# RichExplor/VIL_Fusion

Hardware: AMD Instinct MI355X
Metric: sliding-window solve iters/sec (10 KF, ~5.5k factors) @1/2/4/8 GPU vs CPU (higher is better)
Workload: dtype f64

## Files before the change

vil_fusion_amd/csrc/vilf_api.hip:

```cpp
#include <hip/hip_runtime.h>
#include <string>
#include <vector>
#include <cstring>
#include <cstdio>
#include <cmath>
#include <algorithm>
#include <chrono>
#include <cstdlib>
#include <thread>
#include <atomic>
#include <type_traits>
#include "vilf_internal.hpp"
#include "vilf_kernels.hpp"
#include "vilf_sort.hpp"

namespace {

int class_plan(const vilf_window_in &in, int *cls, int *cstart, int *ccount) {
    int pcount[VB_NPAIR] = {0};
    for (int f = 0; f < in.n_features; f++) {
        const int s = in.feature_start_frame[f], n = in.feature_obs_offset[f + 1] - in.feature_obs_offset[f];
        for (int k = 1; k < n; k++) { const int j = s + k; pcount[j * (j - 1) / 2 + s]++; }
    }
    int order[VB_NPAIR], load[4] = {0, 0, 0, 0};
// ... 1075 lines not shown
    if (!h || !counts || !h->resident || !h->marg.info || !h->marg.qlInfo) return VILF_ERR_INVALID_ARGUMENT;
    HIPCHECK(h, hipSetDevice(h->device));
    const size_t sB = h->B;
    std::vector<int> info(sB * MG_INFO), qi(sB * 4);
    HIPCHECK(h, hipMemcpyAsync(info.data(), h->marg.info, info.size() * 4, hipMemcpyDeviceToHost, h->stream));
    HIPCHECK(h, hipMemcpyAsync(qi.data(), h->marg.qlInfo, qi.size() * 4, hipMemcpyDeviceToHost, h->stream));
    HIPCHECK(h, hipStreamSynchronize(h->stream));
    counts[0] = counts[1] = counts[2] = counts[3] = 0;
    for (size_t w = 0; w < sB; w++) {
        if (info[w * MG_INFO] != 0) { counts[3]++; continue; }
        counts[0]++;
        if (info[w * MG_INFO + 7] == 0) counts[1]++;
        if (qi[w * 4 + 3] == 1) counts[2]++;
    }
    return VILF_OK;
}

static int hook_buf(vilf_handle *h, size_t doubles) { return h->d[D_HOOK].ensure(doubles * 8) ? VILF_OK : VILF_ERR_DEVICE; }

extern "C" int vilf_eval_projection(vilf_handle *h, const double *const *p, const double pts_i[3], const double pts_j[3], double *residuals, double **jac) {
    if (!h || !p || !residuals) return VILF_ERR_INVALID_ARGUMENT;
    if (hook_buf(h, 256) != VILF_OK) return VILF_ERR_DEVICE;
    double in[32];
    std::memcpy(in, p[0], 56); std::memcpy(in + 7, p[1], 56); std::memcpy(in + 14, p[2], 56);
    std::memcpy(in + 21, pts_i, 24); std::memcpy(in + 24, pts_j, 24);
    double *d = h->d[D_HOOK].as<double>();
    HIPCHECK(h, hipMemcpyAsync(d, in, sizeof(in), hipMemcpyHostToDevice, h->stream));
    hipLaunchKernelGGL(k_hook_projection, dim3(1), dim3(HOOK_NT), 0, h->stream, d, d + 7, d + 14, p[3][0], d + 21, d + 24, h->opts.focal_length / 1.5, d + 32);
    double out[28];
    HIPCHECK(h, hipMemcpyAsync(out, d + 32, sizeof(out), hipMemcpyDeviceToHost, h->stream));
    HIPCHECK(h, hipStreamSynchronize(h->stream));
    residuals[0] = out[0]; residuals[1] = out[1];
    if (jac) {
        for (int blk = 0; blk < 2; blk++)
            if (jac[blk]) for (int r = 0; r < 2; r++) { for (int c = 0; c < 6; c++) jac[blk][7 * r + c] = out[2 + 12 * blk + 6 * r + c]; jac[blk][7 * r + 6] = 0; }
        if (jac[2]) {
            double in2[40] = {0};
            std::memcpy(in2, in, 27 * 8);
            in2[31] = p[3][0]; in2[37] = 0.0; in2[38] = h->opts.focal_length / 1.5;
            HIPCHECK(h, hipMemcpyAsync(d + 64, in2, sizeof(in2), hipMemcpyHostToDevice, h->stream));
            hipLaunchKernelGGL(k_hook_projection_td, dim3(1), dim3(HOOK_NT), 0, h->stream, d + 64, d + 64 + 40);
            double out2[42];
            HIPCHECK(h, hipMemcpyAsync(out2, d + 64 + 40, sizeof(out2), hipMemcpyDeviceToHost, h->stream));
            HIPCHECK(h, hipStreamSynchronize(h->stream));
            for (int r = 0; r < 2; r++) { for (int c = 0; c < 6; c++) jac[2][7 * r + c] = out2[26 + 6 * r + c]; jac[2][7 * r + 6] = 0; }
        }
        if (jac[3]) { jac[3][0] = out[26]; jac[3][1] = out[27]; }
    }
    return VILF_OK;
}

extern "C" int vilf_eval_projection_td(vilf_handle *h, const double *const *p, const double pts_i[3], const double pts_j[3], const double vel_i[2], const double vel_j[2],
                                       double td_i, double td_j, double row_i, double row_j, double *residuals, double **jac) {
    if (!h || !p || !residuals || !pts_i || !pts_j || !vel_i || !vel_j) return VILF_ERR_INVALID_ARGUMENT;
    if (hook_buf(h, 128) != VILF_OK) return VILF_ERR_DEVICE;
    double in[40];
    std::memcpy(in, p[0], 56); std::memcpy(in + 7, p[1], 56); std::memcpy(in + 14, p[2], 56);
    std::memcpy(in + 21, pts_i, 24); std::memcpy(in + 24, pts_j, 24); std::memcpy(in + 27, vel_i, 16); std::memcpy(in + 29, vel_j, 16);
    const double ROW = h->opts.ROW;
    in[31] = p[3][0]; in[32] = p[4][0]; in[33] = td_i; in[34] = td_j; in[35] = row_i - ROW / 2; in[36] = row_j - ROW / 2;
    in[37] = h->opts.TR / ROW; in[38] = h->opts.focal_length / 1.5;
    double *d = h->d[D_HOOK].as<double>();
    HIPCHECK(h, hipMemcpyAsync(d, in, sizeof(in), hipMemcpyHostToDevice, h->stream));
    hipLaunchKernelGGL(k_hook_projection_td, dim3(1), dim3(HOOK_NT), 0, h->stream, d, d + 40);
    double out[42];
    HIPCHECK(h, hipMemcpyAsync(out, d + 40, sizeof(out), hipMemcpyDeviceToHost, h->stream));
    HIPCHECK(h, hipStreamSynchronize(h->stream));
    residuals[0] = out[0]; residuals[1] = out[1];
    if (jac) {
        const int off[3] = {2, 14, 26};
        for (int blk = 0; blk < 3; blk++)
            if (jac[blk]) for (int r = 0; r < 2; r++) { for (int c = 0; c < 6; c++) jac[blk][7 * r + c] = out[off[blk] + 6 * r + c]; jac[blk][7 * r + 6] = 0; }
        if (jac[3]) { jac[3][0] = out[38]; jac[3][1] = out[39]; }
        if (jac[4]) { jac[4][0] = out[40]; jac[4][1] = out[41]; }
    }
    return VILF_OK;
}

static void pack_imu_rec(const vilf_imu_preint *p, double *rec) {
    std::memset(rec, 0, IMU_REC * 8);
    fill_imu_rec(*p, rec);
    rec[287] = 1.0;
}

static int run_imu_hook(vilf_handle *h, const double *const *p, const vilf_imu_preint *pre, double **d_out) {
    if (hook_buf(h, 4096) != VILF_OK) return VILF_ERR_DEVICE;
    double *d = *d_out = h->d[D_HOOK].as<double>();
    std::vector<double> in(40 + IMU_REC + 225, 0.0);
    std::memcpy(&in[0], p[0], 56); std::memcpy(&in[7], p[1], 72); std::memcpy(&in[16], p[2], 56); std::memcpy(&in[23], p[3], 72);
    for (int i = 0; i < 3; i++) in[32 + i] = h->opts.G[i];
    pack_imu_rec(pre, &in[40]);
    std::memcpy(&in[40 + IMU_REC], pre->covariance, 225 * 8);
    HIPCHECK(h, vilf_copy_sync(h, d, in.data(), in.size() * 8, hipMemcpyHostToDevice));
    hipLaunchKernelGGL(k_imu_prep, dim3(1), dim3(IMU_PREP_NT), 0, h->stream, 1, d + 40 + IMU_REC, d + 1024, d + 40);
    hipLaunchKernelGGL(k_hook_imu, dim3(1), dim3(HOOK_NT), 0, h->stream, d, d + 7, d + 16, d + 23, d + 40, d + 32, d + 2048, d + 3072);
    return VILF_OK;
}
extern "C" int vilf_eval_imu(vilf_handle *h, const double *const *p, const vilf_imu_preint *pre, double *residuals, double **jac) {
    if (!h || !p || !pre || !residuals) return VILF_ERR_INVALID_ARGUMENT;
    double *d;
    { const int rc = run_imu_hook(h, p, pre, &d); if (rc != VILF_OK) return rc; }
    std::vector<double> out(15 + 450);
    HIPCHECK(h, hipMemcpyAsync(out.data(), d + 2048, out.size() * 8, hipMemcpyDeviceToHost, h->stream));
    HIPCHECK(h, hipStreamSynchronize(h->stream));
    for (int i = 0; i < 15; i++) residuals[i] = out[i];
    if (jac) {
        const int off[4] = {0, 6, 15, 21}, loc[4] = {6, 9, 6, 9}, glob[4] = {7, 9, 7, 9};
        for (int blk = 0; blk < 4; blk++)
            if (jac[blk]) for (int r = 0; r < 15; r++) { for (int c = 0; c < glob[blk]; c++) jac[blk][glob[blk] * r + c] = (c < loc[blk]) ? out[15 + 30 * r + off[blk] + c] : 0.0; }
    }
    return VILF_OK;
}

extern "C" int vilf_eval_imu_raw(vilf_handle *h, const double *const *p, const vilf_imu_preint *pre, double *residuals, double **jac, double *sqrt_info_out) {
    if (!h || !p || !pre || !residuals) return VILF_ERR_INVALID_ARGUMENT;
    double *d;
    { const int rc = run_imu_hook(h, p, pre, &d); if (rc != VILF_OK) return rc; }
    std::vector<double> raw(450 + 15), S(225);
    HIPCHECK(h, hipMemcpyAsync(raw.data(), d + 3072, raw.size() * 8, hipMemcpyDeviceToHost, h->stream));
    HIPCHECK(h, hipMemcpyAsync(S.data(), d + 40 + IMU_SQRT, 225 * 8, hipMemcpyDeviceToHost, h->stream));
    HIPCHECK(h, hipStreamSynchronize(h->stream));
    for (int i = 0; i < 15; i++) residuals[i] = raw[450 + i];
    if (jac) {
        const int off[4] = {0, 6, 15, 21}, loc[4] = {6, 9, 6, 9}, glob[4] = {7, 9, 7, 9};
        for (int blk = 0; blk < 4; blk++)
            if (jac[blk]) for (int r = 0; r < 15; r++) { for (int c = 0; c < glob[blk]; c++) jac[blk][glob[blk] * r + c] = (c < loc[blk]) ? raw[30 * r + off[blk] + c] : 0.0; }
    }
    if (sqrt_info_out) std::memcpy(sqrt_info_out, S.data(), 225 * 8);
    return VILF_OK;
}

extern "C" int vilf_eval_lidar_between(vilf_handle *h, const double *const *p, const vilf_lidar_constraint *c, double *residuals, double **jac) {
    if (!h || !p || !c || !residuals) return VILF_ERR_INVALID_ARGUMENT;
    if (hook_buf(h, 256) != VILF_OK) return VILF_ERR_DEVICE;
    if (!h->resident) lidar_extrinsic(h->opts, h->batch);
    double in[32];
    std::memcpy(in, p[0], 56); std::memcpy(in + 7, p[1], 56);
    std::memcpy(in + 14, h->batch.qil, 32); std::memcpy(in + 18, h->batch.til, 24);
    for (int i = 0; i < 4; i++) in[21 + i] = c->q[i];
    for (int i = 0; i < 3; i++) in[25 + i] = c->t[i];
    double *d = h->d[D_HOOK].as<double>();
    HIPCHECK(h, hipMemcpyAsync(d, in, sizeof(in), hipMemcpyHostToDevice, h->stream));
    hipLaunchKernelGGL(k_hook_lidar, dim3(1), dim3(HOOK_NT), 0, h->stream, d, d + 7, d + 14, d + 18, d + 21, d + 32);
    double out[78];
    HIPCHECK(h, hipMemcpyAsync(out, d + 32, sizeof(out), hipMemcpyDeviceToHost, h->stream));
    HIPCHECK(h, hipStreamSynchronize(h->stream));
    for (int i = 0; i < 6; i++) residuals[i] = out[i];
    if (jac)
        for (int blk = 0; blk < 2; blk++)
            if (jac[blk]) for (int r = 0; r < 6; r++) { for (int cc = 0; cc < 6; cc++) jac[blk][7 * r + cc] = out[6 + 36 * blk + 6 * r + cc]; jac[blk][7 * r + 6] = 0; }
    return VILF_OK;
}

extern "C" int vilf_eval_edge(vilf_handle *h, const double pose[7], const double cp[3], const double a[3], const double bb[3], double r[3], double *J) {
    if (!h) return VILF_ERR_INVALID_ARGUMENT;
    if (hook_buf(h, 128) != VILF_OK) return VILF_ERR_DEVICE;
    double in[16];
    std::memcpy(in, pose, 56); std::memcpy(in + 7, cp, 24); std::memcpy(in + 10, a, 24); std::memcpy(in + 13, bb, 24);
    double *d = h->d[D_HOOK].as<double>();
    HIPCHECK(h, hipMemcpyAsync(d, in, sizeof(in), hipMemcpyHostToDevice, h->stream));
    hipLaunchKernelGGL(k_hook_edge, dim3(1), dim3(HOOK_NT), 0, h->stream, d, d + 7, d + 10, d + 13, d + 16);
    double out[21];
    HIPCHECK(h, hipMemcpyAsync(out, d + 16, sizeof(out), hipMemcpyDeviceToHost, h->stream));
    HIPCHECK(h, hipStreamSynchronize(h->stream));
    for (int i = 0; i < 3; i++) r[i] = out[i];
    if (J) for (int i = 0; i < 3; i++) { for (int c = 0; c < 6; c++) J[7 * i + c] = out[3 + 6 * i + c]; J[7 * i + 6] = 0; }
    return VILF_OK;
}

extern "C" int vilf_eval_surf(vilf_handle *h, const double pose[7], const double cp[3], const double n[3], double dd, double r[1], double *J) {
    if (!h) return VILF_ERR_INVALID_ARGUMENT;
    if (hook_buf(h, 128) != VILF_OK) return VILF_ERR_DEVICE;
    double in[16];
    std::memcpy(in, pose, 56); std::memcpy(in + 7, cp, 24); std::memcpy(in + 10, n, 24);
    double *d = h->d[D_HOOK].as<double>();
    HIPCHECK(h, hipMemcpyAsync(d, in, sizeof(in), hipMemcpyHostToDevice, h->stream));
    hipLaunchKernelGGL(k_hook_surf, dim3(1), dim3(HOOK_NT), 0, h->stream, d, d + 7, d + 10, dd, d + 16);
    double out[7];
    HIPCHECK(h, hipMemcpyAsync(out, d + 16, sizeof(out), hipMemcpyDeviceToHost, h->stream));
    HIPCHECK(h, hipStreamSynchronize(h->stream));
    r[0] = out[0];
    if (J) { for (int c = 0; c < 6; c++) J[c] = out[1 + c]; J[6] = 0; }
    return VILF_OK;
}

static int plus_hook(vilf_handle *h, const double x[7], const double dl[6], double xp[7], int kind) {
    if (!h) return VILF_ERR_INVALID_ARGUMENT;
    if (hook_buf(h, 64) != VILF_OK) return VILF_ERR_DEVICE;
    double in[13];
    std::memcpy(in, x, 56); std::memcpy(in + 7, dl, 48);
    double *d = h->d[D_HOOK].as<double>();
    HIPCHECK(h, hipMemcpyAsync(d, in, sizeof(in), hipMemcpyHostToDevice, h->stream));
    hipLaunchKernelGGL(k_hook_plus, dim3(1), dim3(HOOK_NT), 0, h->stream, d, d + 7, kind, d + 16);
    HIPCHECK(h, hipMemcpyAsync(xp, d + 16, 56, hipMemcpyDeviceToHost, h->stream));
    HIPCHECK(h, hipStreamSynchronize(h->stream));
    return VILF_OK;
}
extern "C" int vilf_pose_plus(vilf_handle *h, const double x[7], const double d[6], double xp[7]) { return plus_hook(h, x, d, xp, 0); }
extern "C" int vilf_se3_plus(vilf_handle *h, const double x[7], const double d[6], double xp[7]) { return plus_hook(h, x, d, xp, 1); }

extern "C" int vilf_eval_prior(vilf_handle *h, const vilf_prior *p, const double *const *params, double *residuals, double **jac) {
    if (!h || !p || !params || !residuals || !p->valid || p->n < 1 || p->n > VILF_PRIOR_MAX_DIM || p->n_blocks < 1 || p->n_blocks > VILF_PRIOR_MAX_BLOCKS) return VILF_ERR_INVALID_ARGUMENT;
    const int n = p->n, nb = p->n_blocks;
    const size_t doubles = 32 + 2 * 24 * 9 + (size_t)n * n + 2 * (size_t)n + 16;
    if (hook_buf(h, doubles) != VILF_OK) return VILF_ERR_DEVICE;
    std::vector<double> in(32 + 2 * 24 * 9 + (size_t)n * n + n, 0.0);
    int *hdr = reinterpret_cast<int *>(in.data());
    hdr[0] = n; hdr[1] = nb;
    for (int i = 0; i < nb; i++) {
        hdr[2 + i] = p->block_size[i]; hdr[26 + i] = p->block_idx[i];
        if (!params[i]) return VILF_ERR_INVALID_ARGUMENT;
        for (int k = 0; k < p->block_size[i] && k < 9; k++) { in[32 + 9 * i + k] = p->block_x0[i][k]; in[32 + 216 + 9 * i + k] = params[i][k]; }
    }
    std::memcpy(&in[32 + 432], p->linearized_jacobians, sizeof(double) * n * n);
    std::memcpy(&in[32 + 432 + (size_t)n * n], p->linearized_residuals, sizeof(double) * n);
    double *d = h->d[D_HOOK].as<double>();
    HIPCHECK(h, hipMemcpyAsync(d, in.data(), in.size() * 8, hipMemcpyHostToDevice, h->stream));
    double *d_out = d + in.size();
    hipLaunchKernelGGL(k_hook_prior, dim3(1), dim3(HOOK_PRIOR_NT), 0, h->stream, reinterpret_cast<const int *>(d), d + 32, d + 32 + 216, d + 32 + 432, d + 32 + 432 + (size_t)n * n, d_out);
    HIPCHECK(h, hipMemcpyAsync(residuals, d_out, sizeof(double) * n, hipMemcpyDeviceToHost, h->stream));
    HIPCHECK(h, hipStreamSynchronize(h->stream));
    if (jac)
        for (int i = 0; i < nb; i++) {
            if (!jac[i]) continue;
            const int gs = p->block_size[i], ls = gs == 7 ? 6 : gs, idx = p->block_idx[i];
            for (int r = 0; r < n; r++) for (int c = 0; c < gs; c++) jac[i][(size_t)r * gs + c] = c < ls ? p->linearized_jacobians[(size_t)r * n + idx + c] : 0.0;
        }
    return VILF_OK;
}
```

vil_fusion_amd/csrc/vilf_device.hpp:

```cpp
#pragma once
#include <hip/hip_runtime.h>
#include <math.h>

#define VD __device__ __forceinline__

VD double vilf_dot3(double a0, double b0, double a1, double b1, double a2, double b2) { return __dadd_rn(__dadd_rn(__dmul_rn(a0, b0), __dmul_rn(a1, b1)), __dmul_rn(a2, b2)); }

__device__ __forceinline__ void lds_barrier() { asm volatile("s_waitcnt lgkmcnt(0)\n\ts_barrier" ::: "memory"); }
template <int CTRL>
VD double vilf_dpp_f64(double v) {
    const int lo = __builtin_amdgcn_update_dpp(0, __double2loint(v), CTRL, 0xF, 0xF, false), hi = __builtin_amdgcn_update_dpp(0, __double2hiint(v), CTRL, 0xF, 0xF, false);
    return __hiloint2double(hi, lo);
}
VD double vilf_wave_sum64(double v) {
    v += vilf_dpp_f64<0xB1>(v);
    v += vilf_dpp_f64<0x4E>(v);
    v += vilf_dpp_f64<0x141>(v);
    v += vilf_dpp_f64<0x140>(v);
    const double r0 = __hiloint2double(__builtin_amdgcn_readlane(__double2hiint(v), 0), __builtin_amdgcn_readlane(__double2loint(v), 0));
    const double r1 = __hiloint2double(__builtin_amdgcn_readlane(__double2hiint(v), 16), __builtin_amdgcn_readlane(__double2loint(v), 16));
    const double r2 = __hiloint2double(__builtin_amdgcn_readlane(__double2hiint(v), 32), __builtin_amdgcn_readlane(__double2loint(v), 32));
    const double r3 = __hiloint2double(__builtin_amdgcn_readlane(__double2hiint(v), 48), __builtin_amdgcn_readlane(__double2loint(v), 48));
    return (r0 + r1) + (r2 + r3);
}
// ... 260 lines not shown
    u[0] += tji[0] - tic[0]; u[1] += tji[1] - tic[1]; u[2] += tji[2] - tic[2];
    m3T_vec(ric, u, tc);
#pragma unroll
    for (int k = 0; k < 9; k++) { pt[k] = A[k]; pt[9 + k] = ARi[k]; pt[18 + k] = Rji[k]; pt[30 + k] = Rc[k]; }
#pragma unroll
    for (int k = 0; k < 3; k++) { pt[27 + k] = tji[k]; pt[39 + k] = tc[k]; }
}
template <bool JAC>
VD void projection_eval_pair(const double *pt, const double *ric, const double *tic, const double *pts_i, const double *pts_j, double inv_dep,
                             double sqrt_info, double *r, double *Ji, double *Jj, double *Jf) {
    const double il = 1.0 / inv_dep;
    const double pc_i[3] = {pts_i[0] * il, pts_i[1] * il, pts_i[2] * il};
    double pc_j[3];
    m3_vec(pt + 30, pc_i, pc_j);
    pc_j[0] += pt[39]; pc_j[1] += pt[40]; pc_j[2] += pt[41];
    const double inv_z = 1.0 / pc_j[2];
    r[0] = sqrt_info * (pc_j[0] * inv_z - pts_j[0]);
    r[1] = sqrt_info * (pc_j[1] * inv_z - pts_j[1]);
    if (JAC) {
        const double r00 = sqrt_info * inv_z, r02 = -sqrt_info * pc_j[0] * inv_z * inv_z, r12 = -sqrt_info * pc_j[1] * inv_z * inv_z;
        const double *A = pt, *ARi = pt + 9, *Rji = pt + 18;
        double p_imu_i[3], p_imu_j[3];
        m3_vec(ric, pc_i, p_imu_i);
        p_imu_i[0] += tic[0]; p_imu_i[1] += tic[1]; p_imu_i[2] += tic[2];
        m3_vec(Rji, p_imu_i, p_imu_j);
        p_imu_j[0] += pt[27]; p_imu_j[1] += pt[28]; p_imu_j[2] += pt[29];
        double M[6], M2[6], N[6];
#pragma unroll
        for (int j = 0; j < 3; j++) {
            M[j] = r00 * A[j] + r02 * A[6 + j]; M[3 + j] = r00 * A[3 + j] + r12 * A[6 + j];
            M2[j] = r00 * ARi[j] + r02 * ARi[6 + j]; M2[3 + j] = r00 * ARi[3 + j] + r12 * ARi[6 + j];
            N[j] = r00 * ric[3 * j] + r02 * ric[3 * j + 2]; N[3 + j] = r00 * ric[3 * j + 1] + r12 * ric[3 * j + 2];
        }
#pragma unroll
        for (int rr = 0; rr < 2; rr++) {
            const double *m = M + 3 * rr, *m2 = M2 + 3 * rr, *n = N + 3 * rr;
            double *ji = Ji + 6 * rr, *jj = Jj + 6 * rr;
            ji[0] = m[0]; ji[1] = m[1]; ji[2] = m[2];
            ji[3] = -(m2[1] * p_imu_i[2] - m2[2] * p_imu_i[1]);
            ji[4] = -(-m2[0] * p_imu_i[2] + m2[2] * p_imu_i[0]);
            ji[5] = -(m2[0] * p_imu_i[1] - m2[1] * p_imu_i[0]);
            jj[0] = -m[0]; jj[1] = -m[1]; jj[2] = -m[2];
            jj[3] = n[1] * p_imu_j[2] - n[2] * p_imu_j[1];
            jj[4] = -n[0] * p_imu_j[2] + n[2] * p_imu_j[0];
            jj[5] = n[0] * p_imu_j[1] - n[1] * p_imu_j[0];
        }
        double rp[3];
        m3_vec(pt + 30, pts_i, rp);
        const double s = -il * il;
        Jf[0] = (r00 * rp[0] + r02 * rp[2]) * s;
        Jf[1] = (r00 * rp[1] + r12 * rp[2]) * s;
    }
}

template <bool JAC>
VD void lidar_between_eval(const double *posei, const double *posej, const Q &qil, const double *til, const Q &lq, const double *lt,
                           double *r, double *Ji, double *Jj) {
    Q Qi = q_load(posei + 3), Qj = q_load(posej + 3);
    Q Qi_inv = q_inv(Qi), qli = q_inv(qil);
    double dP[3] = {posej[0] - posei[0], posej[1] - posei[1], posej[2] - posei[2]};
    double a[3], tli[3], b[3], c[3], rp[3];
    q_rot(Qi_inv, dP, a);
    q_rot(qli, til, tli); tli[0] = -tli[0]; tli[1] = -tli[1]; tli[2] = -tli[2];
    Q qm = q_mul(qil, lq);
    q_rot(qm, tli, b);
    c[0] = a[0] - til[0] - b[0]; c[1] = a[1] - til[1] - b[1]; c[2] = a[2] - til[2] - b[2];
    q_rot(qli, c, rp);
    Q cdq = q_mul(qm, qli);
    Q rq = q_mul(q_inv(cdq), q_mul(Qi_inv, Qj));
    r[0] = 10.0 * (rp[0] - lt[0]); r[1] = 10.0 * (rp[1] - lt[1]); r[2] = 10.0 * (rp[2] - lt[2]);
    r[3] = 100.0 * 2.0 * rq.x; r[4] = 100.0 * 2.0 * rq.y; r[5] = 100.0 * 2.0 * rq.z;
    if (JAC) {
#pragma unroll
        for (int k = 0; k < 36; k++) { Ji[k] = 0; Jj[k] = 0; }
        double Rm[9], Rl[9], S[9], T[9];
        q_toR(q_mul(qli, Qi_inv), Rm);
        q_toR(qli, Rl);
        skew3(a, S);
        m3_mul(Rl, S, T);
        double B[9], Cm[9];
        qleft_qright_br(q_mul(q_inv(Qj), Qi), cdq, B);
        qleft_br(q_mul(q_inv(cdq), q_mul(Qi_inv, Qj)), Cm);
#pragma unroll
        for (int i = 0; i < 3; i++)
#pragma unroll
            for (int j = 0; j < 3; j++) {
                Ji[6 * i + j] = -Rm[3 * i + j];
                Ji[6 * i + 3 + j] = T[3 * i + j];
                Ji[6 * (3 + i) + 3 + j] = -B[3 * i + j];
                Jj[6 * i + j] = Rm[3 * i + j];
                Jj[6 * (3 + i) + 3 + j] = Cm[3 * i + j];
            }
    }
}

template <bool JAC, int LD = 30, bool ZERO = true>
VD void imu_raw_eval(const double *posei, const double *sbi, const double *posej, const double *sbj, const double *rec, const double *G,
                     double *r, double *Jraw) {
    const double dt = rec[0];
    const double *dp = rec + 1, *dv = rec + 8, *lba = rec + 11, *lbg = rec + 14;
    const double *dp_dba = rec + 17, *dp_dbg = rec + 26, *dq_dbg = rec + 35, *dv_dba = rec + 44, *dv_dbg = rec + 53;
    Q Qi = q_load(posei + 3), Qj = q_load(posej + 3), delta_q = q_load(rec + 4);
    Q Qi_inv = q_inv(Qi);
    double dba[3] = {sbi[3] - lba[0], sbi[4] - lba[1], sbi[5] - lba[2]};
    double dbg[3] = {sbi[6] - lbg[0], sbi[7] - lbg[1], sbi[8] - lbg[2]};
    double th[3];
    m3_vec(dq_dbg, dbg, th);
    Q cdq = q_mul(delta_q, q_delta(th[0], th[1], th[2]));
    double t1[3], t2[3], cdv[3], cdp[3];
    m3_vec(dv_dba, dba, t1); m3_vec(dv_dbg, dbg, t2);
    for (int k = 0; k < 3; k++) cdv[k] = dv[k] + t1[k] + t2[k];
    m3_vec(dp_dba, dba, t1); m3_vec(dp_dbg, dbg, t2);
    for (int k = 0; k < 3; k++) cdp[k] = dp[k] + t1[k] + t2[k];
    double a[3], b[3], ra[3], rb[3];
    for (int k = 0; k < 3; k++) {
        a[k] = 0.5 * G[k] * dt * dt + posej[k] - posei[k] - sbi[k] * dt;
        b[k] = G[k] * dt + sbj[k] - sbi[k];
    }
    q_rot(Qi_inv, a, ra);
    q_rot(Qi_inv, b, rb);
    Q QiQj = q_mul(Qi_inv, Qj);
    Q rq = q_mul(q_inv(cdq), QiQj);
    r[0] = ra[0] - cdp[0]; r[1] = ra[1] - cdp[1]; r[2] = ra[2] - cdp[2];
    r[3] = 2 * rq.x; r[4] = 2 * rq.y; r[5] = 2 * rq.z;
    r[6] = rb[0] - cdv[0]; r[7] = rb[1] - cdv[1]; r[8] = rb[2] - cdv[2];
    for (int k = 0; k < 3; k++) { r[9 + k] = sbj[3 + k] - sbi[3 + k]; r[12 + k] = sbj[6 + k] - sbi[6 + k]; }
    if (JAC) {
        if (ZERO) for (int k = 0; k < 450; k++) Jraw[k] = 0;
        double RiT[9], S[9], B[9];
        q_toR(Qi_inv, RiT);
        auto put = [&](int r0, int c0, const double *m, double s) {
            for (int i = 0; i < 3; i++) for (int j = 0; j < 3; j++) Jraw[(r0 + i) * LD + c0 + j] = s * m[3 * i + j];
        };
        const double I3[9] = {1, 0, 0, 0, 1, 0, 0, 0, 1};
        put(0, 0, RiT, -1.0);
        skew3(ra, S); put(0, 3, S, 1.0);
        qleft_qright_br(q_mul(q_inv(Qj), Qi), cdq, B); put(3, 3, B, -1.0);
        skew3(rb, S); put(6, 3, S, 1.0);
        put(0, 6, RiT, -dt); put(0, 9, dp_dba, -1.0); put(0, 12, dp_dbg, -1.0);
        {
            double L[9], T[9];
            qleft_br(q_mul(q_mul(q_inv(Qj), Qi), delta_q), L);
            m3_mul(L, dq_dbg, T);
            put(3, 12, T, -1.0);
        }
        put(6, 6, RiT, -1.0); put(6, 9, dv_dba, -1.0); put(6, 12, dv_dbg, -1.0);
        put(9, 9, I3, -1.0); put(12, 12, I3, -1.0);
        put(0, 15, RiT, 1.0);
        qleft_br(q_mul(q_inv(cdq), QiQj), B); put(3, 18, B, 1.0);
        put(6, 21, RiT, 1.0); put(9, 24, I3, 1.0); put(12, 27, I3, 1.0);
    }
}

template <bool JAC>
VD void edge_eval(const double *pose, const double *cp, const double *pa, const double *pb, double *r, double *J) {
    Q q = q_load(pose);
    double lp[3];
    q_rot(q, cp, lp);
    lp[0] += pose[4]; lp[1] += pose[5]; lp[2] += pose[6];
    double u[3] = {lp[0] - pa[0], lp[1] - pa[1], lp[2] - pa[2]}, v[3] = {lp[0] - pb[0], lp[1] - pb[1], lp[2] - pb[2]};
    double ab[3] = {pa[0] - pb[0], pa[1] - pb[1], pa[2] - pb[2]};
    double inv = 1.0 / sqrt(ab[0] * ab[0] + ab[1] * ab[1] + ab[2] * ab[2]);
    r[0] = (u[1] * v[2] - u[2] * v[1]) * inv;
    r[1] = (u[2] * v[0] - u[0] * v[2]) * inv;
    r[2] = (u[0] * v[1] - u[1] * v[0]) * inv;
    if (JAC) {
        double Sab[9], Slp[9], T[9];
        skew3(ab, Sab); skew3(lp, Slp);
        m3_mul(Sab, Slp, T);
        for (int i = 0; i < 3; i++)
            for (int j = 0; j < 3; j++) { J[6 * i + j] = T[3 * i + j] * inv; J[6 * i + 3 + j] = -Sab[3 * i + j] * inv; }
    }
}
template <bool JAC>
VD void surf_eval(const double *pose, const double *cp, const double *n, double d, double *r, double *J) {
    Q q = q_load(pose);
    double pw[3];
    q_rot(q, cp, pw);
    pw[0] += pose[4]; pw[1] += pose[5]; pw[2] += pose[6];
    r[0] = n[0] * pw[0] + n[1] * pw[1] + n[2] * pw[2] + d;
    if (JAC) {
        J[0] = -(n[1] * pw[2] - n[2] * pw[1]);
        J[1] = -(-n[0] * pw[2] + n[2] * pw[0]);
        J[2] = -(n[0] * pw[1] - n[1] * pw[0]);
        J[3] = n[0]; J[4] = n[1]; J[5] = n[2];
    }
}
VD void se3_plus(const double *x, const double *d, double *o) {
    double th = sqrt(d[0] * d[0] + d[1] * d[1] + d[2] * d[2]);
    double half = 0.5 * th, imag, real = cos(half);
    if (th < 1e-10) { double t2 = th * th, t4 = t2 * t2; imag = 0.5 - 0.0208333 * t2 + 0.000260417 * t4; }
    else imag = sin(half) / th;
    Q dq{imag * d[0], imag * d[1], imag * d[2], real};
    double Jm[9];
    if (th < 1e-10) q_toR(dq, Jm);
    else {
        double O[9], O2[9];
        skew3(d, O); m3_mul(O, O, O2);
        double a = (1 - cos(th)) / (th * th), b = (th - sin(th)) / (th * th * th);
        for (int k = 0; k < 9; k++) Jm[k] = a * O[k] + b * O2[k];
        Jm[0] += 1; Jm[4] += 1; Jm[8] += 1;
    }
    double dt[3], rt[3];
    m3_vec(Jm, d + 3, dt);
    Q qn = q_mul(dq, q_load(x));
    q_rot(dq, x + 4, rt);
    q_store(o, qn);
    o[4] = rt[0] + dt[0]; o[5] = rt[1] + dt[1]; o[6] = rt[2] + dt[2];
}


template <bool JAC>
VD void projection_td_eval(const double *Pi, const double *Ri, const double *Pj, const double *Rj, const double *ric, const double *tic,
                           const double *pts_i, const double *pts_j, const double *vel_i, const double *vel_j, double td, double td_i, double td_j,
                           double row_i_c, double row_j_c, double tr_over_row, double inv_dep, double sqrt_info,
                           double *r, double *Ji, double *Jj, double *Jf, double *Jex, double *Jtd) {
    const double si = td - td_i + tr_over_row * row_i_c, sj = td - td_j + tr_over_row * row_j_c;
    const double pi_td[3] = {pts_i[0] - si * vel_i[0], pts_i[1] - si * vel_i[1], pts_i[2]};
    const double pj_td[3] = {pts_j[0] - sj * vel_j[0], pts_j[1] - sj * vel_j[1], pts_j[2]};
    double M2[6];
    projection_eval<JAC>(Pi, Ri, Pj, Rj, ric, tic, pi_td, pj_td, inv_dep, sqrt_info, r, Ji, Jj, Jf, Jex, M2);
    if (JAC) {
        const double v3[3] = {vel_i[0], vel_i[1], 0.0};
        double rv[3];
        m3_vec(ric, v3, rv);
        Jtd[0] = (M2[0] * rv[0] + M2[1] * rv[1] + M2[2] * rv[2]) / inv_dep * -1.0 + sqrt_info * vel_j[0];
        Jtd[1] = (M2[3] * rv[0] + M2[4] * rv[1] + M2[5] * rv[2]) / inv_dep * -1.0 + sqrt_info * vel_j[1];
    }
}
}
```

vil_fusion_amd/csrc/vilf_kernels.hip:

```cpp
#include "vilf_device.hpp"
#include "vilf_kernels.hpp"

using namespace vd;

typedef double double4_t __attribute__((ext_vector_type(4)));
typedef double double2_t __attribute__((ext_vector_type(2)));

#define NT VB_NT
#ifdef VILF_STAMPS
#define STAMP(kid, i) do { if (b.dbg && blockIdx.x == 0 && threadIdx.x == 0) b.dbg[(kid) * 32 + (i)] = __builtin_readcyclecounter(); } while (0)
#define TICK() __builtin_readcyclecounter()
#else
#define STAMP(kid, i) do { } while (0)
#define TICK() 0LL
#endif
#define LSTAMP(i) do { if (JAC) STAMP(0, i); } while (0)
__device__ __forceinline__ int pair_index(int i, int j) { return j * (j - 1) / 2 + i; }
__device__ __forceinline__ int perm_index(int a, int l) { return l < 6 ? 6 * a + l : 66 + 9 * a + (l - 6); }
__device__ __forceinline__ void unperm(int p, int &a, int &l) {
    if (p < 66) { a = p / 6; l = p - 6 * a; } else { int q = p - 66; a = q / 9; l = 6 + q - 9 * a; }
}
__device__ __forceinline__ int tile_index(int ta, int tb) { return ta * (ta + 1) / 2 + tb; }
#define TIX(r, c) (16 * (r) + ((c) ^ (r)))

__device__ __forceinline__ double block_sum(double v, double *s_red) {
    const int tid = threadIdx.x;
    v = vilf_wave_sum64(v);
    lds_barrier();
    if ((tid & 63) == 0) s_red[tid >> 6] = v;
    lds_barrier();
    double r = 0;
#pragma unroll
    for (int k = 0; k < NT / 64; k++) r += s_red[k];
    lds_barrier();
    return r;
}
__device__ __forceinline__ double block_max(double v, double *s_red) {
    const int tid = threadIdx.x;
    v = vilf_wave_max64(v);
    lds_barrier();
    if ((tid & 63) == 0) s_red[tid >> 6] = v;
    lds_barrier();
    double r = s_red[0];
#pragma unroll
    for (int k = 1; k < NT / 64; k++) r = fmax(r, s_red[k]);
    lds_barrier();
    return r;
}

extern "C" __global__ __launch_bounds__(IMU_PREP_NT) void k_imu_prep(int n, const double *cov, double *work, double *imu_rec) {
    __shared__ double sA[4][15][16], sI[4][15][16], s_piv[4];
    const int grp = threadIdx.x >> 4, r = threadIdx.x & 15, id = blockIdx.x * 4 + grp;
    const bool row = id < n && r < 15;
    (void)work;
    if (row) for (int j = 0; j < 15; j++) { sA[grp][r][j] = cov[(size_t)id * 225 + 15 * r + j]; sI[grp][r][j] = (j == r) ? 1.0 : 0.0; }
    __syncthreads();
    for (int k = 0; k < 15; k++) {
        if (id < n && r == 0) {
            int p = k; double best = fabs(sA[grp][k][k]);
            for (int i = k + 1; i < 15; i++) { const double v = fabs(sA[grp][i][k]); if (v > best) { best = v; p = i; } }
            if (p != k) for (int j = 0; j < 15; j++) { double t = sA[grp][k][j]; sA[grp][k][j] = sA[grp][p][j]; sA[grp][p][j] = t; t = sI[grp][k][j]; sI[grp][k][j] = sI[grp][p][j]; sI[grp][p][j] = t; }
            s_piv[grp] = sA[grp][k][k];
        }
        __syncthreads();
        if (row && r > k) {
            const double f = sA[grp][r][k] / s_piv[grp];
            for (int j = k; j < 15; j++) sA[grp][r][j] -= f * sA[grp][k][j];
            for (int j = 0; j < 15; j++) sI[grp][r][j] -= f * sI[grp][k][j];
        }
        __syncthreads();
    }
    for (int k = 14; k >= 0; k--) {
        if (row && r == k) { const double piv = sA[grp][k][k]; for (int j = 0; j < 15; j++) sI[grp][k][j] /= piv; }
        __syncthreads();
        if (row && r < k) { const double f = sA[grp][r][k]; for (int j = 0; j < 15; j++) sI[grp][r][j] -= f * sI[grp][k][j]; }
        __syncthreads();
    }
    for (int j = 0; j < 15; j++) {
        if (row && r == j) { double sacc = sI[grp][j][j]; for (int k = 0; k < j; k++) sacc -= sI[grp][j][k] * sI[grp][j][k]; sI[grp][j][j] = sqrt(sacc); }
        __syncthreads();
        if (row && r > j) { double t = sI[grp][r][j]; for (int k = 0; k < j; k++) t -= sI[grp][r][k] * sI[grp][j][k]; sI[grp][r][j] = t / sI[grp][j][j]; }
        __syncthreads();
    }
    if (row) { double *S = imu_rec + (size_t)id * IMU_REC + IMU_SQRT; for (int j = 0; j < 15; j++) S[15 * r + j] = (j >= r) ? sI[grp][j][r] : 0.0; }
}

extern "C" __global__ __launch_bounds__(NT) void k_prior_prep(VbBatch b, double *prior_H, double *prior_g, unsigned lds_bytes, const int *done4) {
    const int w = blockIdx.x, tid = threadIdx.x;
    const int *hdr = b.prior_hdr + (size_t)w * VB_PRIOR_HDR;
    if (!hdr[0] || (done4 && done4[4 * (size_t)w + 3])) return;
    const int n = hdr[1];
    const double *J = b.prior_J + (size_t)w * VB_PRIOR_LD * VB_PRIOR_LD;
    const double *r = b.prior_r + (size_t)w * VB_PRIOR_LD;
    double *H = prior_H + (size_t)w * VB_PRIOR_LD * VB_PRIOR_LD;
    double *g = prior_g + (size_t)w * VB_PRIOR_LD;
    extern __shared__ double s_J[];
    const int ld = n | 1;
    if ((size_t)n * ld * sizeof(double) <= lds_bytes) {
        for (int e = tid; e < n * n; e += NT) { const int k = e / n, i = e - k * n; s_J[k * ld + i] = J[e]; }
        __syncthreads();
        for (int e = tid; e < n * n; e += NT) {
            int i = e / n, j = e - i * n;
            double s = 0;
            for (int k = 0; k < n; k++) s += s_J[k * ld + i] * s_J[k * ld + j];
            H[i * VB_PRIOR_LD + j] = s;
        }
        for (int i = tid; i < n; i += NT) {
            double s = 0;
            for (int k = 0; k < n; k++) s += s_J[k * ld + i] * r[k];
            g[i] = s;
        }
        return;
    }
    for (int e = tid; e < n * n; e += NT) {
        int i = e / n, j = e - i * n;
        double s = 0;
        for (int k = 0; k < n; k++) s += J[k * n + i] * J[k * n + j];
        H[i * VB_PRIOR_LD + j] = s;
    }
    for (int i = tid; i < n; i += NT) {
        double s = 0;
        for (int k = 0; k < n; k++) s += J[k * n + i] * r[k];
        g[i] = s;
    }
}

__device__ void prior_setup(const VbBatch &b, int w, const double *pose, const double *sb, int *s_pcol, double *s_dx, int tid) {
    const int *hdr = b.prior_hdr + (size_t)w * VB_PRIOR_HDR;
    for (int i = tid; i < VB_P; i += NT) s_pcol[i] = -1;
    for (int i = tid; i < VB_PRIOR_LD; i += NT) s_dx[i] = 0.0;
    __syncthreads();
    if (!hdr[0]) return;
    const int nb = hdr[2];
    if (tid < nb) {
        const int id = hdr[3 + tid], size = hdr[27 + tid], idx = hdr[51 + tid];
        const double *x0 = b.prior_x0 + ((size_t)w * 24 + tid) * 9;
        if (id < VB_NF) {
            const double *x = pose + 7 * id;
            for (int k = 0; k < 3; k++) s_dx[idx + k] = x[k] - x0[k];
            Q dq = q_mul(q_inv(q_load(x0 + 3)), q_load(x + 3));
            double sgn = (dq.w >= 0) ? 2.0 : -2.0;
            s_dx[idx + 3] = sgn * dq.x; s_dx[idx + 4] = sgn * dq.y; s_dx[idx + 5] = sgn * dq.z;
            for (int k = 0; k < 6; k++) s_pcol[15 * id + k] = idx + k;
        } else if (id < 2 * VB_NF) {
            const int a = id - VB_NF;
            const double *x = sb + 9 * a;
            for (int k = 0; k < 9; k++) { s_dx[idx + k] = x[k] - x0[k]; s_pcol[15 * a + 6 + k] = idx + k; }
        } else if (id == 2 * VB_NF) {
            const double *x = b.ex + (size_t)w * 7;
            for (int k = 0; k < 3; k++) s_dx[idx + k] = x[k] - x0[k];
            Q dq = q_mul(q_inv(q_load(x0 + 3)), q_load(x + 3));
            double sgn = (dq.w >= 0) ? 2.0 : -2.0;
            s_dx[idx + 3] = sgn * dq.x; s_dx[idx + 4] = sgn * dq.y; s_dx[idx + 5] = sgn * dq.z;
        }
        (void)size;
    }
    __syncthreads();
}

__device__ double prior_cost_partial(const VbBatch &b, int w, const double *s_dx, int tid) {
    const int *hdr = b.prior_hdr + (size_t)w * VB_PRIOR_HDR;
    if (!hdr[0]) return 0.0;
    const int n = hdr[1];
    const double *J = b.prior_J + (size_t)w * VB_PRIOR_LD * VB_PRIOR_LD;
    const double *r0 = b.prior_r + (size_t)w * VB_PRIOR_LD;
    double acc = 0;
    for (int row = tid; row < n; row += NT) {
        double s = r0[row];
        for (int k = 0; k < n; k++) s += J[row * n + k] * s_dx[k];
        acc += 0.5 * s * s;
    }
    return acc;
}

__device__ __forceinline__ double prior_cost_split(const VbBatch &b, int w, const double *s_dx, double *s_tmp, int tid) {
    const int *hdr = b.prior_hdr + (size_t)w * VB_PRIOR_HDR;
    if (!hdr[0]) return 0.0;
    const int n = hdr[1];
    if (3 * n > NT) return prior_cost_partial(b, w, s_dx, tid);
    const double *J = b.prior_J + (size_t)w * VB_PRIOR_LD * VB_PRIOR_LD;
    const int row = tid / 3, part = tid - 3 * row, per = (n + 2) / 3, c0 = part * per, c1 = min(n, c0 + per);
    const double r0v = b.prior_r[(size_t)w * VB_PRIOR_LD + min(row, n - 1)];
    double acc = 0;
    if (row < n) {
        const double *Jr = J + (size_t)row * n;
#pragma unroll 8
        for (int k = c0; k < c1; k++) acc += Jr[k] * s_dx[k];
    }
    s_tmp[tid] = acc;
    lds_barrier();
    double cost = 0;
    if (row < n && part == 0) { double t = r0v; t += s_tmp[tid]; t += s_tmp[tid + 1]; t += s_tmp[tid + 2]; cost = 0.5 * t * t; }
    lds_barrier();
    return cost;
}
__device__ __forceinline__ double prior_grad_split(const VbBatch &b, int w, const double *s_dx, const int *s_pcol, double *s_tmp, int tid) {
    const int *hdr = b.prior_hdr + (size_t)w * VB_PRIOR_HDR;
    if (!hdr[0]) return 0.0;
    const int n = hdr[1];
    const int pc = (tid < VB_P) ? s_pcol[tid] : -1;
    if (3 * n > NT) {
        if (pc < 0) return 0.0;
        double t = b.prior_g[(size_t)w * VB_PRIOR_LD + pc];
        const double *pH = b.prior_H + (size_t)w * VB_PRIOR_LD * VB_PRIOR_LD + (size_t)pc * VB_PRIOR_LD;
#pragma unroll 8
        for (int k = 0; k < n; k++) t += pH[k] * s_dx[k];
        return t;
    }
    const int col = tid / 3, part = tid - 3 * col, per = (n + 2) / 3, c0 = part * per, c1 = min(n, c0 + per);
    const double g0 = b.prior_g[(size_t)w * VB_PRIOR_LD + max(pc, 0)];
    double acc = 0;
    if (col < n) {
        const double *pH = b.prior_H + (size_t)w * VB_PRIOR_LD * VB_PRIOR_LD + (size_t)col * VB_PRIOR_LD;
#pragma unroll 8
        for (int k = c0; k < c1; k++) acc += pH[k] * s_dx[k];
    }
    s_tmp[tid] = acc;
    lds_barrier();
    double g = 0;
    if (pc >= 0) { g = g0; g += s_tmp[3 * pc]; g += s_tmp[3 * pc + 1]; g += s_tmp[3 * pc + 2]; }
    lds_barrier();
    return g;
}

template <bool GRAD>
__device__ __forceinline__ void prior_products_j(const VbBatch &b, int w, const double *s_dx, const int *s_pcol, double *s_tmp, double *s_t, int tid, double &cost, double &gprior) {
    cost = 0.0; gprior = 0.0;
    const int *hdr = b.prior_hdr + (size_t)w * VB_PRIOR_HDR;
    if (!hdr[0]) return;
    const int n = hdr[1];
    if (n > 85) {
        cost = prior_cost_split(b, w, s_dx, s_tmp, tid);
        if (GRAD) gprior = prior_grad_split(b, w, s_dx, s_pcol, s_tmp, tid);
        return;
    }
    const double *J = b.prior_J + (size_t)w * VB_PRIOR_LD * VB_PRIOR_LD, *r0 = b.prior_r + (size_t)w * VB_PRIOR_LD;
    const int lane = tid & 63, wave = __builtin_amdgcn_readfirstlane(tid >> 6);
    const int c0 = min(lane, n - 1), c1 = min(lane + 64, n - 1);
    const double dx0 = s_dx[lane], dx1 = s_dx[lane + 64];
    const double r0v = r0[min(wave + 4 * min(lane, 31), n - 1)];
    {
        double a0[6], a1[6];
#pragma unroll 1
        for (int rb = wave; rb < n; rb += 24) {
#pragma unroll
            for (int u = 0; u < 6; u++) { const double *Jr = J + (size_t)min(rb + 4 * u, n - 1) * n; a0[u] = Jr[c0]; a1[u] = Jr[c1]; }
#pragma unroll
            for (int u = 0; u < 6; u++) {
                const int r = rb + 4 * u;
                const double sum = vilf_wave_sum64(a0[u] * dx0 + a1[u] * dx1);
                const double t = readlane_f64(r0v, (r - wave) >> 2) + sum;
                if (r < n && lane == 0) { s_t[r] = t; cost += 0.5 * t * t; }
            }
        }
    }
    if (GRAD) {
        lds_barrier();
        const int pc = (tid < VB_P) ? s_pcol[tid] : -1;
        if (wave < 3) {
            const int per = (n + 2) / 3, ra = wave * per, rb = min(n, ra + per);
            double g0 = 0, g1 = 0;
#pragma unroll 8
            for (int r = ra; r < rb; r++) { const double t = s_t[r]; const double *Jr = J + (size_t)r * n; g0 += Jr[c0] * t; g1 += Jr[c1] * t; }
            s_tmp[85 * wave + c0] = g0;
            if (lane + 64 < n) s_tmp[85 * wave + lane + 64] = g1;
        }
        lds_barrier();
        if (pc >= 0) { double g = s_tmp[pc]; g += s_tmp[85 + pc]; g += s_tmp[170 + pc]; gprior = g; }
        lds_barrier();
    }
}

__device__ __forceinline__ int vb_window(const VbBatch &b) {
    const int i = b.live_it;
    if (!b.live_ctl || i < 3 || !b.live_ctl[i - 2]) return blockIdx.x + b.w0;
    if ((int)blockIdx.x >= b.live_ctl[64 + i - 1]) return -1;
    return b.live_buf[(size_t)((i - 1) & 1) * b.B + blockIdx.x];
}
#define LIN_LDS_DOUBLES VB_LIN_LDS_DOUBLES

__device__ __forceinline__ double pd_get(const double *pd, const int *s_pcn, int p, int e) { const double v = pd[p * VB_PAIRD + e]; return (s_pcn[p] > 0) ? v : 0.0; }

__device__ __forceinline__ int pair_elem(int row, int col) {
    if (row < 6) {
        if (col < 6) return 6 * row + col;
        if (col < 12) return 36 + 6 * row + (col - 6);
        if (col == 12) return 108 + row;
        return -1;
    }
    if (row < 12) {
        if (col >= 6 && col < 12) return 72 + 6 * (row - 6) + (col - 6);
        if (col == 12) return 114 + (row - 6);
    }
    return -1;
}

struct LinShared {
    double pose[77], sb[99], R[99], ric[9], tic[3];
    double lidJ[10 * 72], lidr[64], grad[176];
    double pt[VB_NPAIR * PT_LD];
    double dx[VB_PRIOR_LD];
    double red[NT];
    double def[2];
    int pcol[VB_P], pst[VB_NPAIR], pcn[VB_NPAIR];
    int last, defi[2];
};
static_assert(sizeof(LinShared) <= VB_LIN_SHARED_BYTES, "VB_LIN_SHARED_BYTES (vilf_batch.hpp) must cover LinShared");
template <bool JAC, bool SPLIT = false>
__device__ __forceinline__ int linearize_body(const VbBatch &b, int iteration_zero) {
    const int tid = threadIdx.x, lane = tid & 63, wave = __builtin_amdgcn_readfirstlane(tid >> 6);
    const int NR = SPLIT ? b.split_nr : 1, NCH = NR - 2;
    const int w = SPLIT ? (int)blockIdx.x / NR : vb_window(b);
    const int role = SPLIT ? (int)blockIdx.x - w * NR : 0;
    if (w < 0) return 2;
    const bool do_vis = !SPLIT || role < NCH, do_imu = !SPLIT || role == NCH, do_lp = !SPLIT || role == NCH + 1;
    int *sctl = SPLIT ? b.split_ctl + (size_t)w * VB_SPLIT_CTL : nullptr;
    double *sbuf = SPLIT ? b.split_buf + (size_t)w * VB_SPLIT_DBL : nullptr, *scost = SPLIT ? sbuf + VB_SPLIT_CARRY : nullptr;
    extern __shared__ double s_dyn[];
    LinShared &LS = *reinterpret_cast<LinShared *>(s_dyn + LIN_LDS_DOUBLES);
    int &s_last = LS.last;
    double *s_def = LS.def;
    int *s_defi = LS.defi;
    auto arrive = [&]() -> bool {
        __threadfence();
        __syncthreads();
        if (tid == 0) s_last = (__hip_atomic_fetch_add(sctl + VB_SPLIT_CNT + (b.split_gen & 7), 1, __ATOMIC_ACQ_REL, __HIP_MEMORY_SCOPE_AGENT) == NR - 1) ? 1 : 0;
        __syncthreads();
        if (s_last) __builtin_amdgcn_fence(__ATOMIC_ACQUIRE, "agent");
        return s_last != 0;
    };
    VbState *st = b.st + w;
    if (SPLIT && tid == 0) sctl[VB_SPLIT_CNT + ((b.split_gen + 4) & 7)] = 0;
    const int lit = b.live_it;
    const bool lists = !iteration_zero && JAC && b.live_ctl != nullptr && lit >= 1;
    const int stopped_before = lists ? b.live_ctl[lit - 1] : 0;
    if (!iteration_zero && st->done) { if (lists && tid == 0) b.live_ctl[lit] = 1; return 2; }
    auto still_live = [&]() {
        if (!lists) return;
        if (st->done || stopped_before) b.live_ctl[lit] = 1;
        if (stopped_before && !st->done) b.live_buf[(size_t)(lit & 1) * b.B + atomicAdd(b.live_ctl + 64 + lit, 1)] = w;
    };
    auto step_bookkeeping = [&]() {
        const int valid = s_defi[0];
        if (!s_defi[1]) { st->dogleg_step_norm = s_def[0]; st->model_cost_change = s_def[1]; }
        if (!valid) {
            st->num_consecutive_invalid += 1;
            st->mu *= 10.0;
            st->reuse = 0;
            st->solve_failed = 0;
            if (st->num_consecutive_invalid >= 5) { st->done = 1; st->termination = 4; }
        } else st->num_consecutive_invalid = 0;
    };
    const int wset = iteration_zero ? 0 : (st->ws ^ 1);
    const size_t ww = (size_t)wset * b.B + w;

    double *s_X = s_dyn;
    double *s_U = s_dyn;
    double *pd = b.pairD + ww * VB_NPAIR * VB_PAIRD;
    double *s_pose = LS.pose, *s_sb = LS.sb, *s_R = LS.R, *s_ric = LS.ric, *s_tic = LS.tic;
    double *s_lidJ = LS.lidJ, *s_lidr = LS.lidr, *s_grad = LS.grad;
    double *s_pt = LS.pt;
    double *s_dx = LS.dx;
    int *s_pcol = LS.pcol, *s_pst = LS.pst, *s_pcn = LS.pcn;
    double *s_red = LS.red;

    LSTAMP(0);
    const int F = b.n_feat[w], nfac = b.n_fac[w];
    const size_t FM = b.Fmax, FC = b.FACmax;
    double *pose_g = b.pose + (size_t)w * 77, *sb_g = b.sb + (size_t)w * 99;
    double *feat_x = b.feat + (size_t)w * FM, *cfeat = b.cand_feat + (size_t)w * FM;
    const double *feat = iteration_zero ? feat_x : cfeat;
    const double *ex = b.ex + (size_t)w * 7;
    const uint8_t *f_const0 = b.f_const + (size_t)w * FM;

    if (tid < 77) s_pose[tid] = pose_g[tid];
    if (tid < 99) s_sb[tid] = sb_g[tid];
    double stepsq = 0;
    if (!iteration_zero) {
        int *s_flagi = reinterpret_cast<int *>(s_red);
        if (tid == 0) {
            int valid = 1;
            double ca = 0, cb = 0;
            const int sf0 = st->solve_failed;
            double norm0 = 0, mcc0 = 0;
            if (sf0) valid = 0;
            else {
                const double radius = st->radius, alpha = st->alpha;
                const double gradient_norm = sqrt(st->grad_sqnorm), gn_norm = sqrt(st->gn_sqnorm);
                double norm;
                if (gn_norm <= radius) { ca = 0; cb = 1; norm = gn_norm; }
                else if (gradient_norm * alpha >= radius) { ca = -(radius / gradient_norm); cb = 0; norm = radius; }
                else {
                    const double b_dot_a = alpha * st->gy;
                    const double a_sq = (alpha * gradient_norm) * (alpha * gradient_norm);
                    const double bma = a_sq - 2 * b_dot_a + gn_norm * gn_norm;
                    const double c = b_dot_a - a_sq;
                    const double d = sqrt(c * c + bma * (radius * radius - a_sq));
                    const double beta = (c <= 0) ? (d - c) / bma : (radius * radius - a_sq) / (d + c);
                    ca = -alpha * (1.0 - beta); cb = beta;
                    norm = sqrt(ca * ca * st->grad_sqnorm - 2 * ca * cb * st->gy + cb * cb * st->gn_sqnorm);
                }
                norm0 = norm;
                const double mu = st->mu_used, G2 = st->grad_sqnorm;
                const double sg = ca * G2 - cb * st->gy;
                const double vHy = G2 - mu * st->gy;
                const double yHy = st->gy - mu * st->gn_sqnorm;
                const double sHs = ca * ca * st->Jg2 - 2 * ca * cb * vHy + cb * cb * yHy;
                const double mcc = -sg - 0.5 * sHs;
                mcc0 = mcc;
                if (!(mcc > 0.0)) valid = 0;
            }
            s_def[0] = norm0; s_def[1] = mcc0; s_defi[0] = valid; s_defi[1] = sf0;
            if (!SPLIT) step_bookkeeping();
            s_flagi[0] = valid;
            s_red[1] = ca; s_red[2] = cb;
            if (!SPLIT && !valid) still_live();
        }
        __syncthreads();
        if (!s_flagi[0]) {
            if (SPLIT) { if (arrive()) { if (tid == 0) step_bookkeeping(); } }
            return 1;
        }
        const double ca = s_red[1], cb = s_red[2];
        const double *scale_g = b.scale + (size_t)w * (VB_P + FM), *diag_g = b.diag + (size_t)w * (VB_P + FM);
        const double *grad_g = b.grad + (size_t)w * (VB_P + FM), *gn_g = b.gn + (size_t)w * (VB_P + FM);
        if (tid < VB_P) {
            int a, l; unperm(tid, a, l);
            s_grad[15 * a + l] = (ca * grad_g[tid] + cb * gn_g[tid]) / diag_g[tid] * scale_g[tid];
        }
        lds_barrier();
        if (tid < VB_NF) {
            double xp[7];
            pose_plus(s_pose + 7 * tid, s_grad + 15 * tid, xp);
            for (int k = 0; k < 7; k++) { const double d = s_pose[7 * tid + k] - xp[k]; stepsq += d * d; s_pose[7 * tid + k] = xp[k]; }
            for (int k = 0; k < 9; k++) { const double d = s_grad[15 * tid + 6 + k]; stepsq += d * d; s_sb[9 * tid + k] += d; }
        }
        for (int f = tid; f < F; f += NT) {
            double v = feat_x[f];
            if (!f_const0[f]) {
                const double d = (ca * grad_g[VB_P + f] + cb * gn_g[VB_P + f]) / diag_g[VB_P + f] * scale_g[VB_P + f];
                stepsq += d * d;
                v += d;
            }
            cfeat[f] = v;
        }
        __threadfence_block();
    }
    unsigned long long cls_mask;
    int my_pst, my_pcn;
    {
        const int *pt = b.pair_off + (size_t)w * VB_PTAB;
        const int pp = min(lane, VB_NPAIR - 1), v1 = pt[2 * pp + 1];
        my_pst = pt[2 * pp]; my_pcn = v1 & 0xffffff;
        if (wave == 0 && lane < VB_NPAIR) { s_pst[lane] = my_pst; s_pcn[lane] = my_pcn; }
        const bool mine = lane < VB_NPAIR && (v1 >> 24) == wave && my_pcn > 0;
        cls_mask = __ballot(mine);
    }
    if (JAC && do_imu) for (int i = tid; i < 10 * 512; i += NT) s_U[i] = 0.0;
    __syncthreads();
    if (tid < VB_NF) q_toR(q_load(s_pose + 7 * tid + 3), s_R + 9 * tid);
    if (tid == 32) { q_toR(q_load(ex + 3), s_ric); s_tic[0] = ex[0]; s_tic[1] = ex[1]; s_tic[2] = ex[2]; }
    prior_setup(b, w, s_pose, s_sb, s_pcol, s_dx, tid);
    if (tid >= 128 && tid < 128 + VB_NPAIR) {
        const int p = tid - 128;
        int j = 1; while (j * (j + 1) / 2 <= p) j++;
        const int i = p - j * (j - 1) / 2;
        pair_table(s_pose + 7 * i, s_R + 9 * i, s_pose + 7 * j, s_R + 9 * j, s_ric, s_tic, s_pt + PT_LD * p);
    }
    LSTAMP(1);

    double cost_local = 0;
    if (do_imu && tid >= 192 && tid < 202) {
        const int k = tid - 192;
        const double *rec = b.imu + ((size_t)w * 10 + k) * IMU_REC;
        if (rec[287] != 0.0) {
            double r[15];
            if (JAC) {
                imu_raw_eval<true, 32, false>(s_pose + 7 * k, s_sb + 9 * k, s_pose + 7 * (k + 1), s_sb + 9 * (k + 1), rec, b.G, r, s_U + 512 * k);
                for (int m = 0; m < 15; m++) s_U[512 * k + 32 * m + 30] = r[m];
            } else {
                imu_raw_eval<false>(s_pose + 7 * k, s_sb + 9 * k, s_pose + 7 * (k + 1), s_sb + 9 * (k + 1), rec, b.G, r, nullptr);
                double acc = 0;
                for (int i = 0; i < 15; i++) { double sq = 0; for (int m = i; m < 15; m++) sq += rec[IMU_SQRT + 15 * i + m] * r[m]; acc += sq * sq; }
                cost_local += 0.5 * acc;
            }
        }
    }
    if (do_lp && tid >= 64 && tid < 74) {
        const int k = tid - 64;
        if (b.use_lidar) {
            const double *lc = b.lidar + ((size_t)w * 10 + k) * 7;
            if (JAC) {
                double Ji[36], Jj[36];
                lidar_between_eval<true>(s_pose + 7 * k, s_pose + 7 * (k + 1), q_load(b.qil), b.til, q_load(lc), lc + 4, s_lidr + 6 * k, Ji, Jj);
                for (int rr = 0; rr < 6; rr++) for (int c = 0; c < 6; c++) { s_lidJ[72 * k + 12 * rr + c] = Ji[6 * rr + c]; s_lidJ[72 * k + 12 * rr + 6 + c] = Jj[6 * rr + c]; }
            } else lidar_between_eval<false>(s_pose + 7 * k, s_pose + 7 * (k + 1), q_load(b.qil), b.til, q_load(lc), lc + 4, s_lidr + 6 * k, nullptr, nullptr);
        } else {
            if (JAC) for (int e = 0; e < 72; e++) s_lidJ[72 * k + e] = 0;
            for (int e = 0; e < 6; e++) s_lidr[6 * k + e] = 0;
        }
    }
    lds_barrier();
    LSTAMP(2);
    if (JAC && do_imu) for (int task = wave; task < 20; task += 4) {
        const int k = task >> 1, ct = task & 1;
        double *Xk = s_U + 512 * k;
        const double *S = b.imu + ((size_t)w * 10 + k) * IMU_REC + IMU_SQRT;
        double av[4], bv[4];
#pragma unroll
        for (int s4 = 0; s4 < 4; s4++) {
            const int i = lane & 15, kk = 4 * s4 + (lane >> 4);
            av[s4] = (i < 15 && kk < 15) ? S[15 * i + kk] : 0.0;
            bv[s4] = Xk[32 * kk + 16 * ct + (lane & 15)];
        }
        double4_t acc = {0, 0, 0, 0};
#pragma unroll
        for (int s4 = 0; s4 < 4; s4++) acc = __builtin_amdgcn_mfma_f64_16x16x4f64(av[s4], bv[s4], acc, 0, 0, 0);
#pragma unroll
        for (int q = 0; q < 4; q++) Xk[32 * ((lane >> 4) + 4 * q) + 16 * ct + (lane & 15)] = acc[q];
    }
    lds_barrier();
    LSTAMP(3);
    if (JAC) {
        double *imuH = b.imuH + ww * 9000, *imug = b.imug + ww * 300;
        if (do_imu)
        for (int task = wave; task < 30; task += 4) {
            const int k = task / 3, tt = task - 3 * k;
            const int ti = (tt == 0) ? 0 : 1, tj = (tt == 2) ? 1 : 0;
            const double *Xk = s_U + 512 * k;
            double4_t acc = {0, 0, 0, 0};
#pragma unroll
            for (int s4 = 0; s4 < 4; s4++) {
                const int row = 4 * s4 + (lane >> 4);
                acc = __builtin_amdgcn_mfma_f64_16x16x4f64(Xk[32 * row + 16 * ti + (lane & 15)], Xk[32 * row + 16 * tj + (lane & 15)], acc, 0, 0, 0);
            }
#pragma unroll
            for (int q = 0; q < 4; q++) {
                const int p = 16 * ti + (lane >> 4) + 4 * q, c = 16 * tj + (lane & 15);
                if (p < 30 && c < 30) { imuH[900 * k + 30 * p + c] = acc[q]; if (ti != tj) imuH[900 * k + 30 * c + p] = acc[q]; }
                if (p == 30 && c < 30) imug[30 * k + c] = acc[q];
                if (p == 30 && c == 30) cost_local += 0.5 * acc[q];
            }
        }
        LSTAMP(10);
        double *lidH = b.lidH + ww * 1440, *lidg = b.lidg + ww * 120;
        if (do_lp) {
        for (int idx = tid; idx < 1440; idx += NT) {
            const int k = idx / 144, e = idx - 144 * k, p = e / 12, q = e - 12 * p;
            double s = 0;
            for (int row = 0; row < 6; row++) s += s_lidJ[72 * k + 12 * row + p] * s_lidJ[72 * k + 12 * row + q];
            lidH[idx] = s;
        }
        for (int idx = tid; idx < 120; idx += NT) {
            const int k = idx / 12, p = idx - 12 * k;
            double s = 0;
            for (int row = 0; row < 6; row++) s += s_lidJ[72 * k + 12 * row + p] * s_lidr[6 * k + row];
            lidg[idx] = s;
        }
        }
    }
    if (SPLIT && do_imu) scost[tid] = cost_local;
    if (SPLIT) cost_local = 0;
    if (do_lp && tid >= 64 && tid < 74) { const int k = tid - 64; double s = 0; for (int m = 0; m < 6; m++) s += s_lidr[6 * k + m] * s_lidr[6 * k + m]; cost_local += 0.5 * s; }
    LSTAMP(11);
    if (SPLIT && do_lp) { scost[256 + tid] = cost_local; cost_local = 0; }
    double gprior = 0;
    if (!SPLIT || do_lp) {
        double pcost;
        prior_products_j<(JAC && !SPLIT)>(b, w, s_dx, s_pcol, s_red, s_grad, tid, pcost, gprior);
        if (SPLIT) scost[512 + tid] = pcost; else cost_local += pcost;
    }
    LSTAMP(13);
    lds_barrier();
    if (tid == 0) s_X[2 * VB_CHUNK * VB_XLD] = 0.0;
    LSTAMP(4);
    const int *f_start = b.f_start + (size_t)w * FM;
    const uint8_t *f_const = b.f_const + (size_t)w * FM;
    const double *facrec = b.facrec + (size_t)w * FC * 8;
    double *facw = b.facw + (size_t)w * VB_FACW * FC;
    double *W = b.W + ww * FM * VB_WLD;
    long long t_eval = 0, t_sync1 = 0, t_mfma = 0, t_sync2 = 0, t_a = 0;
    int pe[4];
#pragma unroll
    for (int q4 = 0; q4 < 4; q4++) pe[q4] = pair_elem((lane >> 4) + 4 * q4, lane & 15);
    double4_t cacc = {0, 0, 0, 0}, cacc1 = {0, 0, 0, 0};
    unsigned long long mrem = cls_mask;
    if (!JAC) {
        for (int fac = tid; fac < nfac; fac += NT) {
            const double4_t *rp = reinterpret_cast<const double4_t *>(facrec + (size_t)fac * 8);
            const double4_t ra = rp[0], rb = rp[1];
            const double pts_i[3] = {ra[0], ra[1], ra[2]}, pts_j[3] = {ra[3], rb[0], rb[1]};
            const unsigned long long ia = __double_as_longlong(rb[2]), ib = __double_as_longlong(rb[3]);
            if ((ib >> 17) & 1) continue;
            const int f = (int)(ia & 0xffffffffu), fi = (int)(ib & 0xff), fj = (int)((ib >> 8) & 0xff);
            double r[2];
            projection_eval_pair<false>(s_pt + PT_LD * pair_index(fi, fj), s_ric, s_tic, pts_i, pts_j, feat[f], b.sqrt_info, r, nullptr, nullptr, nullptr);
            double rho0, sw;
            cauchy(r[0] * r[0] + r[1] * r[1], b.cauchy_b, rho0, sw);
            cost_local += 0.5 * rho0;
        }
    } else {
    const int c_begin = SPLIT ? role * VB_CHUNK : 0, c_end = SPLIT ? (do_vis ? min(nfac, (role + 1) * VB_CHUNK) : 0) : nfac;
    double4_t ra_n = {0, 0, 0, 0}, rb_n = {0, 0, 0, 0};
    double fv_n = 0;
    if (c_begin < c_end) {
        const double4_t *rp = reinterpret_cast<const double4_t *>(facrec + (size_t)min(c_begin + tid, nfac - 1) * 8);
        ra_n = rp[0]; rb_n = rp[1];
        fv_n = feat[(int)(__double_as_longlong(rb_n[2]) & 0xffffffffu)];
    }
    for (int c0 = c_begin; c0 < c_end; c0 += VB_CHUNK) {
        t_a = TICK();
        const int q = c0 + tid;
        double *x0 = s_X + (2 * min(tid, VB_CHUNK - 1)) * VB_XLD, *x1 = x0 + VB_XLD;
        const double4_t ra = ra_n, rb = rb_n;
        const double fv = fv_n;
        const unsigned long long ia = __double_as_longlong(rb[2]), ib = __double_as_longlong(rb[3]);
        if (tid >= VB_CHUNK) {
        } else if (q < nfac && !((ib >> 17) & 1)) {
            const double pts_i[3] = {ra[0], ra[1], ra[2]}, pts_j[3] = {ra[3], rb[0], rb[1]};
            const int slot = (int)(ia >> 32), fi = (int)(ib & 0xff), fj = (int)((ib >> 8) & 0xff);
            const bool fc = ((ib >> 16) & 1) != 0;
            double r[2], Ji[12], Jj[12], Jf[2];
            projection_eval_pair<true>(s_pt + PT_LD * pair_index(fi, fj), s_ric, s_tic, pts_i, pts_j, fv, b.sqrt_info, r, Ji, Jj, Jf);
            double rho0, sw;
            cauchy(r[0] * r[0] + r[1] * r[1], b.cauchy_b, rho0, sw);
            cost_local += 0.5 * rho0;
#pragma unroll
            for (int c = 0; c < 6; c++) { x0[c] = sw * Jj[c]; x0[6 + c] = sw * Ji[c]; x1[c] = sw * Jj[6 + c]; x1[6 + c] = sw * Ji[6 + c]; }
            x0[12] = sw * r[0]; x1[12] = sw * r[1];
            if (!fc) {
                const double jf0 = sw * Jf[0], jf1 = sw * Jf[1];
                double2_t *Wr = reinterpret_cast<double2_t *>(W + (size_t)(ib >> 18) * VB_WLD + 6 * fj);
                double2_t *fw = reinterpret_cast<double2_t *>(facw + (size_t)slot * VB_FACW);
#pragma unroll
                for (int c = 0; c < 6; c += 2) {
                    Wr[c >> 1] = double2_t{x0[c] * jf0 + x1[c] * jf1, x0[c + 1] * jf0 + x1[c + 1] * jf1};
                    fw[c >> 1] = double2_t{x0[6 + c] * jf0 + x1[6 + c] * jf1, x0[7 + c] * jf0 + x1[7 + c] * jf1};
                }
                fw[3] = double2_t{jf0 * jf0 + jf1 * jf1, jf0 * x0[12] + jf1 * x1[12]};
            }
        } else {
#pragma unroll
            for (int c = 0; c < VB_XLD; c++) { x0[c] = 0; x1[c] = 0; }
        }
        { long long t_b = TICK(); t_eval += t_b - t_a; t_a = t_b; }
        lds_barrier();
        { long long t_b = TICK(); t_sync1 += t_b - t_a; t_a = t_b; }
        if (c0 + VB_CHUNK < c_end) {
            const double4_t *rp = reinterpret_cast<const double4_t *>(facrec + (size_t)min(c0 + VB_CHUNK + tid, nfac - 1) * 8);
            ra_n = rp[0]; rb_n = rp[1];
        }
        const int x0c = VB_CLS * (c0 / VB_CHUNK);
        if constexpr (SPLIT) {
            double *carry_out = sbuf + ((size_t)(role * 4 + wave) * 64 + lane) * 8;
            const double *carry_in = sbuf + ((size_t)(max(role, 1) * 4 - 4 + wave) * 64 + lane) * 8;
            int *flag_out = sctl + 1 + 4 * role + wave, *flag_in = sctl + 1 + 4 * max(role - 1, 0) + wave;
#pragma unroll 1
            for (int pass = 0; pass < 3; pass++) {
                unsigned long long m = cls_mask;
                while (m) {
                    const int p = __builtin_amdgcn_readfirstlane(__builtin_ctzll(m));
                    m &= m - 1;
                    const int pst = __builtin_amdgcn_readlane(my_pst, p), pcn_ = __builtin_amdgcn_readlane(my_pcn, p);
                    if (pst + pcn_ <= x0c) continue;
                    if (pst >= x0c + VB_CLS) break;
                    const bool in = pst < x0c, out = pst + pcn_ > x0c + VB_CLS;
                    if ((in ? 2 : (out ? 0 : 1)) != pass) continue;
                    double4_t acc = {0, 0, 0, 0}, acc1 = {0, 0, 0, 0};
                    if (in) {
                        int spins = 0;
                        bool got = false;
                        for (; spins < VB_SPLIT_SPIN_MAX; spins++) {
                            if (__hip_atomic_load(flag_in, __ATOMIC_ACQUIRE, __HIP_MEMORY_SCOPE_AGENT) == b.split_gen) { got = true; break; }
                            __builtin_amdgcn_s_sleep(1);
                        }
                        if (got) {
                            const double2_t *ci = reinterpret_cast<const double2_t *>(carry_in);
                            const double2_t c0_ = ci[0], c1_ = ci[1], c2_ = ci[2], c3_ = ci[3];
                            acc = double4_t{c0_[0], c0_[1], c1_[0], c1_[1]}; acc1 = double4_t{c2_[0], c2_[1], c3_[0], c3_[1]};
                        } else if (lane == 0) __hip_atomic_store(&st->dev_error, 1, __ATOMIC_RELAXED, __HIP_MEMORY_SCOPE_AGENT);
                    }
                    const int lo = max(pst, x0c), hi = min(pst + pcn_, x0c + VB_CLS);
                    const int r_lo = 2 * (VB_CLS * wave + lo - x0c), r_hi = 2 * (VB_CLS * wave + hi - x0c);
                    auto ld4 = [&](int r0, double *a) {
#pragma unroll
                        for (int u = 0; u < 4; u++) {
                            const int row = r0 + 4 * u + (lane >> 4);
                            a[u] = s_X[(row < r_hi && (lane & 15) < VB_XLD) ? row * VB_XLD + (lane & 15) : 2 * VB_CHUNK * VB_XLD];
                        }
                    };
                    double a[4], an[4];
                    ld4(r_lo, a);
// ... 356 lines not shown
        const double *Wr_ = W + (size_t)min((F0) + g, NR - 1) * VB_WLD + c16;                                                    \
        asm volatile("global_load_dwordx2 %0, %5, off\n\tglobal_load_dwordx2 %1, %5, off offset:128\n\t"                           \
                     "global_load_dwordx2 %2, %5, off offset:256\n\tglobal_load_dwordx2 %3, %5, off offset:384\n\t"                \
                     "global_load_dwordx2 %4, %5, off offset:512"                                                                  \
                     : "=&v"(R[0]), "=&v"(R[1]), "=&v"(R[2]), "=&v"(R[3]), "=&v"(R[4]) : "v"(Wr_) : "memory");                      \
    }
#define FD_WAIT(N, R) asm volatile("s_waitcnt vmcnt(" #N ")" : "+v"(R[0]), "+v"(R[1]), "+v"(R[2]), "+v"(R[3]), "+v"(R[4]) : : "memory");
#define FD_STEP(F0, R)                                                                                                             \
    {                                                                                                                              \
        const int k = (F0) + g;                                                                                                    \
        double acc = 0;                                                                                                            \
        _Pragma("unroll") for (int t5 = 0; t5 < 5; t5++) acc += R[t5] * sv[t5];                                                    \
        _Pragma("unroll") for (int o = 8; o > 0; o >>= 1) acc += __shfl_xor(acc, o, 64);                                           \
        if (c16 == 0 && k < NR) out[k] = acc;                                                                                       \
    }
    constexpr int RS = 4 * SNW;
    asm volatile("s_waitcnt vmcnt(0)" ::: "memory");
    FD_ISSUE(4 * wave, ra) FD_ISSUE(4 * wave + RS, rb)
    for (int f0 = 4 * wave; f0 < NR; f0 += 3 * RS) {
        FD_ISSUE(f0 + 2 * RS, rc) FD_WAIT(10, ra) FD_STEP(f0, ra)
        if (f0 + RS < NR) { FD_ISSUE(f0 + 3 * RS, ra) FD_WAIT(10, rb) FD_STEP(f0 + RS, rb) }
        if (f0 + 2 * RS < NR) { FD_ISSUE(f0 + 4 * RS, rb) FD_WAIT(10, rc) FD_STEP(f0 + 2 * RS, rc) }
    }
    asm volatile("s_waitcnt vmcnt(0)" : "+v"(ra[0]), "+v"(ra[1]), "+v"(ra[2]), "+v"(ra[3]), "+v"(ra[4]), "+v"(rb[0]), "+v"(rb[1]), "+v"(rb[2]), "+v"(rb[3]), "+v"(rb[4]),
                                        "+v"(rc[0]), "+v"(rc[1]), "+v"(rc[2]), "+v"(rc[3]), "+v"(rc[4]) : : "memory");
#undef FD_ISSUE
#undef FD_WAIT
#undef FD_STEP
}

extern "C" __global__ __launch_bounds__(SNT) void k_solve(VbBatch b) {
    const int w = vb_window(b), tid = threadIdx.x, lane = tid & 63, wave = __builtin_amdgcn_readfirstlane(tid >> 6);
    if (w < 0) return;
    VbState *st = b.st + w;
    extern __shared__ double s_dyn[];
    double *s_T = s_dyn + SOLVE_OFF_T, *s_g = s_dyn + SOLVE_OFF_G, *s_diag = s_dyn + SOLVE_OFF_DIAG, *s_scale = s_dyn + SOLVE_OFF_SCALE;
    double *s_y = s_dyn + SOLVE_OFF_Y, *s_invd = s_dyn + SOLVE_OFF_INVD, *s_v = s_dyn + SOLVE_OFF_V, *s_red = s_dyn + SOLVE_OFF_RED;
    double *s_cf = s_dyn + SOLVE_OFF_CF;
    int *s_rng = (int *)(s_dyn + SOLVE_OFF_RNG);
    __shared__ int s_pcol[VB_P], s_pinv[VB_PRIOR_LD];
    __shared__ double s_dx[VB_PRIOR_LD];
    __shared__ int s_flag[4];

    if (tid == 0) {
        const int done = st->done, iteration = st->iteration, reuse = st->reuse;
        const double gmn = st->gradient_max_norm, radius = st->radius;
        int go = 1;
        if (done) go = 0;
        else if (iteration >= b.max_iterations) { st->done = 1; st->termination = 0; go = 0; }
        else if (gmn <= b.gradient_tolerance) { st->done = 1; st->termination = 3; go = 0; }
        else if (radius <= b.min_radius) { st->done = 1; st->termination = 4; go = 0; }
        if (go) st->iteration = iteration + 1;
        s_flag[0] = go;
        s_flag[1] = go ? reuse : 1;
    }
    __syncthreads();
    if (!s_flag[0] || s_flag[1]) return;

    STAMP(1, 0);
    const int F = b.n_feat[w];
    const size_t FM = b.Fmax;
    const size_t ww = (size_t)st->ws * b.B + w;
    const double *Hpp = b.Hpp + ww * 66 * 36;
    const double *imuH = b.imuH + ww * 9000, *lidH = b.lidH + ww * 1440;
    const double *priorH = b.prior_H + (size_t)w * VB_PRIOR_LD * VB_PRIOR_LD;
    double *W = b.W + ww * FM * VB_WLD;
    const double *hf = b.hf + ww * FM, *gf = b.gf + ww * FM;
    const uint8_t *f_const = b.f_const + (size_t)w * FM;
    const int *f_start = b.f_start + (size_t)w * FM, *f_nobs = b.f_nobs + (size_t)w * FM;
    const int *f_wrow = b.f_wrow + (size_t)w * FM, *row_feat = b.row_feat + (size_t)w * FM;
    const int NR = b.n_rows[w];
    double *scale_g = b.scale + (size_t)w * (VB_P + FM), *diag_g = b.diag + (size_t)w * (VB_P + FM);
    double *grad_g = b.grad + (size_t)w * (VB_P + FM), *gn_g = b.gn + (size_t)w * (VB_P + FM);
    const double *g_in = b.g + ww * VB_P;
    const int *phdr = b.prior_hdr + (size_t)w * VB_PRIOR_HDR;
    const int pn = phdr[0] ? phdr[1] : 0;

    prior_setup(b, w, b.pose + (size_t)w * 77, b.sb + (size_t)w * 99, s_pcol, s_dx, tid);
    if (tid < VB_PRIOR_LD) s_pinv[tid] = -1;
    __syncthreads();
    if (tid < VB_P) { const int pc = s_pcol[tid]; if (pc >= 0) { const int a = tid / 15, l = tid - 15 * a; s_pinv[pc] = perm_index(a, l); } }
    const int scaling_ready = st->scaling_ready;
    double mu = st->mu;
    int tries = 0;
    bool solved = false;
    double Jg2 = 0, G2 = 0;
    double g2 = 0;
    if (tid < VB_NPAD) {
        double sc = 1.0, d = 1.0, gs = 0.0, vv = 0.0;
        if (tid < VB_P) {
            int a, l; unperm(tid, a, l);
            const double dh = b.diagH[ww * VB_P + 15 * a + l];
            if (scaling_ready) sc = scale_g[tid]; else { sc = 1.0 / (1.0 + sqrt(dh)); scale_g[tid] = sc; }
            d = sqrt(fmin(fmax(sc * sc * dh, b.min_lm_diagonal), b.max_lm_diagonal));
            gs = g_in[15 * a + l] * sc;
            diag_g[tid] = d;
            const double gr = gs / d;
            grad_g[tid] = gr;
            g2 = gr * gr;
            vv = gr / d;
        }
        s_scale[tid] = sc; s_diag[tid] = d; s_g[tid] = gs; s_v[tid] = vv;
    }
#pragma unroll
    for (int u = 0; u < 2; u++) {
        const int f = tid + u * SNT;
        if (f < F) {
            s_rng[f] = (6 * f_start[f]) | ((6 * (f_start[f] + f_nobs[f])) << 16);
            if (!f_const[f]) {
                const double hfv = hf[f], gfv = gf[f];
                double sf;
                if (scaling_ready) sf = scale_g[VB_P + f]; else { sf = 1.0 / (1.0 + sqrt(hfv)); scale_g[VB_P + f] = sf; }
                const double d = sqrt(fmin(fmax(sf * sf * hfv, b.min_lm_diagonal), b.max_lm_diagonal));
                diag_g[VB_P + f] = d;
                const double gr = sf * gfv / d;
                grad_g[VB_P + f] = gr;
                g2 += gr * gr;
            }
        }
    }
    __syncthreads();
    STAMP(1, 1);
    for (;;) {
        double part = 0;
        for (int i = tid; i < 66 * 256; i += SNT) s_T[i] = 0.0;
        __syncthreads();
        if (tid < VB_NPAD - VB_P) s_T[tile_index(10, 10) * 256 + TIX(5 + tid, 5 + tid)] = 1.0;
        {
            const int2 *lv = (const int2 *)b.lut_vis;
            for (int t0 = tid; t0 < 66 * 36; t0 += 5 * SNT) {
                double v[5]; int2 o[5];
#pragma unroll
                for (int u = 0; u < 5; u++) { const int t = min(t0 + u * SNT, 66 * 36 - 1); v[u] = Hpp[t]; o[u] = lv[t]; }
#pragma unroll
                for (int u = 0; u < 5; u++) {
                    if (t0 + u * SNT >= 66 * 36) continue;
                    const int r = (o[u].x >> 15) & 255, c = (o[u].x >> 23) & 255;
                    const double val = v[u] * s_scale[r] * s_scale[c];
                    const int off = (o[u].x & 0x7fff) - 1;
                    if (off >= 0) lds_add(&s_T[off], val);
                    if (o[u].y > 0) lds_add(&s_T[o[u].y - 1], val);
                    part += (((r / 6) != (c / 6)) ? 2.0 : 1.0) * s_v[r] * val * s_v[c];
                }
            }
        }
        __syncthreads();
        for (int par = 0; par < 2; par++) {
            for (int t0 = tid; t0 < 5 * 900; t0 += 5 * SNT) {
                double v[5]; int o[5];
#pragma unroll
                for (int u = 0; u < 5; u++) {
                    const int t = min(t0 + u * SNT, 5 * 900 - 1);
                    const int k2 = t / 900, src = 900 * (2 * k2 + par) + (t - 900 * k2);
                    o[u] = b.lut_imu[src]; v[u] = imuH[src];
                }
#pragma unroll
                for (int u = 0; u < 5; u++) {
                    if (t0 + u * SNT >= 5 * 900) continue;
                    const int r = (o[u] >> 15) & 255, c = (o[u] >> 23) & 255;
                    const double val = v[u] * s_scale[r] * s_scale[c];
                    const int off = (o[u] & 0x7fff) - 1;
                    if (off >= 0) lds_add(&s_T[off], val);
                    part += s_v[r] * val * s_v[c];
                }
            }
            __syncthreads();
            for (int t = tid; t < 5 * 144; t += SNT) {
                const int k2 = t / 144, src = 144 * (2 * k2 + par) + (t - 144 * k2);
                const int o0 = b.lut_lid[src];
                const int r = (o0 >> 15) & 255, c = (o0 >> 23) & 255;
                const double val = lidH[src] * s_scale[r] * s_scale[c];
                const int off = (o0 & 0x7fff) - 1;
                if (off >= 0) lds_add(&s_T[off], val);
                part += s_v[r] * val * s_v[c];
            }
            __syncthreads();
        }
        if (pn > 0) for (int t0 = tid; t0 < pn * pn; t0 += 6 * SNT) {
            double v[6]; int rr[6], cc[6];
#pragma unroll
            for (int u = 0; u < 6; u++) {
                const int t = min(t0 + u * SNT, pn * pn - 1);
                const int i = t / pn, j = t - pn * i;
                rr[u] = s_pinv[i]; cc[u] = s_pinv[j]; v[u] = priorH[i * VB_PRIOR_LD + j];
            }
#pragma unroll
            for (int u = 0; u < 6; u++) {
                const int r = rr[u], c = cc[u];
                if (t0 + u * SNT >= pn * pn || r < 0 || c < 0) continue;
                const double val = v[u] * s_scale[r] * s_scale[c];
                if ((r >> 4) >= (c >> 4)) lds_add(&s_T[tile_index(r >> 4, c >> 4) * 256 + TIX(r & 15, c & 15)], val);
                part += s_v[r] * val * s_v[c];
            }
        }
        __syncthreads();
        STAMP(1, 2);
        if (tries == 0) {
#pragma unroll
            for (int u = 0; u < 2; u++) {
                const int f = tid + u * SNT;
                if (f < F && !f_const[f]) {
                    const double sf = scale_g[VB_P + f], df = diag_g[VB_P + f], hfv = hf[f], gfv = gf[f];
                    const double vf = sf * gfv / (df * df);
                    part += sf * sf * hfv * vf * vf;
                    W[(size_t)f_wrow[f] * VB_WLD + VB_NPOSE + 1] = vf * (sf * sf * hfv + mu * df * df) / sf;
                }
            }
            __threadfence_block();
            G2 = block_sum_s(g2, s_red);
            Jg2 = block_sum_s(part, s_red);
        }
        STAMP(1, 3);
        if (tid < VB_P) { const int tt = tid >> 4, e = tid & 15; s_T[tile_index(tt, tt) * 256 + TIX(e, e)] += mu * s_diag[tid] * s_diag[tid]; }
#pragma unroll
        for (int u = 0; u < 2; u++) {
            const int f = tid + u * SNT;
            if (f < F && !f_const[f]) { const double sf = scale_g[VB_P + f], df = diag_g[VB_P + f]; s_cf[f_wrow[f]] = sf * rsqrt_nr(sf * sf * hf[f] + mu * df * df); }
        }
        if (tid < VB_NPAD) s_y[tid] = s_g[tid];
        __syncthreads();
        STAMP(1, 4);
        for (int k = tid; k < NR; k += SNT) if (row_feat[k] < 0) s_cf[k] = 0.0;
        if (tid < 80) s_red[tid] = 0.0;
        __syncthreads();
        __threadfence_block();
        if (wave & 1) schur_mfma<1>(W, NR, s_cf, s_scale, s_T, s_y, lane, wave); else schur_mfma<0>(W, NR, s_cf, s_scale, s_T, s_y, lane, wave);
        if (tries == 0) {
            double cr = ((lane < VB_NPOSE) ? s_v[lane] * s_red[lane] : 0.0) + ((lane + 64 < VB_NPOSE) ? s_v[lane + 64] * s_red[lane + 64] : 0.0);
            cr = vilf_wave_sum64(cr);
            Jg2 -= 2.0 * cr;
            __syncthreads();
        }
        STAMP(1, 5);
        if (tid < VB_P) s_T[tile_index(10, tid >> 4) * 256 + TIX(5, tid & 15)] = s_y[tid];
        if (tid == 0) s_T[tile_index(10, 10) * 256 + TIX(5, 5)] = 1e250;
        __syncthreads();
        bool ok = true;
        long long tc_a = TICK(), tc_trsm = 0, tc_p1 = 0, tc_p2 = 0, tc_potrf0 = 0;
        if (wave == 0) { bool o = potrf_tile_wave(s_T + tile_index(0, 0) * 256, s_invd, lane); if (lane == 0) s_flag[2] = o ? 1 : 0; }
        __syncthreads();
        { long long t = TICK(); tc_potrf0 = t - tc_a; tc_a = t; }
        for (int k = 0; k < VB_NTILE; k++) {
            if (!s_flag[2]) { ok = false; break; }
            const double *Tkk = s_T + tile_index(k, k) * 256;
            const int nrows = (VB_NTILE - 1 - k) * 16;
            if (tid < nrows) {
                const int ti = k + 1 + (tid >> 4), rr = tid & 15;
                double *Tik = s_T + tile_index(ti, k) * 256;
                double x[16];
#pragma unroll
                for (int c = 0; c < 16; c++) x[c] = Tik[TIX(rr, c)];
#pragma unroll
                for (int c = 0; c < 16; c++) {
                    double s = x[c];
#pragma unroll
                    for (int p = 0; p < c; p++) s -= x[p] * Tkk[TIX(c, p)];
                    x[c] = s * s_invd[16 * k + c];
                }
#pragma unroll
                for (int c = 0; c < 16; c++) Tik[TIX(rr, c)] = x[c];
            }
            __syncthreads();
            { long long t = TICK(); tc_trsm += t - tc_a; tc_a = t; }
            if (k == VB_NTILE - 1) break;
            const int nt = VB_NTILE - 1 - k;
            auto update_tile = [&](int ti, int tj) {
                double *C = s_T + tile_index(ti, tj) * 256;
                const double *A = s_T + tile_index(ti, k) * 256, *Bm = s_T + tile_index(tj, k) * 256;
                double4_t acc;
                double av[4], bv[4];
#pragma unroll
                for (int q = 0; q < 4; q++) acc[q] = C[TIX((lane >> 4) + 4 * q, lane & 15)];
#pragma unroll
                for (int s4 = 0; s4 < 4; s4++) { av[s4] = -A[TIX(lane & 15, 4 * s4 + (lane >> 4))]; bv[s4] = Bm[TIX(lane & 15, 4 * s4 + (lane >> 4))]; }
#pragma unroll
                for (int s4 = 0; s4 < 4; s4++) acc = __builtin_amdgcn_mfma_f64_16x16x4f64(av[s4], bv[s4], acc, 0, 0, 0);
#pragma unroll
                for (int q = 0; q < 4; q++) C[TIX((lane >> 4) + 4 * q, lane & 15)] = acc[q];
            };
            for (int ii = wave; ii < nt; ii += SNW) update_tile(k + 1 + ii, k + 1);
            __syncthreads();
            { long long t = TICK(); tc_p1 += t - tc_a; tc_a = t; }
            if (wave == 0) {
                bool o = potrf_tile_wave(s_T + tile_index(k + 1, k + 1) * 256, s_invd + 16 * (k + 1), lane);
                if (lane == 0) s_flag[2] = o ? 1 : 0;
            } else {
                const int nrest = (nt - 1) * nt / 2;
                for (int tt = wave - 1; tt < nrest; tt += SNW - 1) {
                    int ii = 0; while ((ii + 1) * (ii + 2) / 2 <= tt) ii++;
                    const int jj = tt - ii * (ii + 1) / 2;
                    update_tile(k + 2 + ii, k + 2 + jj);
                }
            }
            __syncthreads();
            { long long t = TICK(); tc_p2 += t - tc_a; tc_a = t; }
        }
        if (b.dbg && blockIdx.x == 0 && tid == 0) { b.dbg[64 + 20] = tc_potrf0; b.dbg[64 + 21] = tc_trsm; b.dbg[64 + 22] = tc_p1; b.dbg[64 + 23] = tc_p2; }
        STAMP(1, 6);
        tries++;
        if (ok) { solved = true; break; }
        mu *= 10.0;
        if (!(mu < 1.0)) break;
        __syncthreads();
    }
    if (!solved) {
        if (tid == 0) { st->solve_failed = 1; st->mu = mu; st->num_linear_solves += tries; st->scaling_ready = 1; st->grad_sqnorm = G2; st->Jg2 = Jg2; }
        return;
// ... 105 lines not shown
    return (c == SB_ND) ? SB_BRHS(a) : -1;
}

__device__ __forceinline__ constexpr int sb_t15_a(int i) { constexpr int T[15] = {0, 1, 1, 2, 2, 2, 3, 3, 3, 3, 4, 4, 4, 4, 4}; return T[i]; }
__device__ __forceinline__ constexpr int sb_t15_b(int i) { constexpr int T[15] = {0, 0, 1, 0, 1, 2, 0, 1, 2, 3, 0, 1, 2, 3, 4}; return T[i]; }
__device__ __forceinline__ constexpr int sb_y_ntl(int wv) { return wv == 3 ? 3 : 4; }
__device__ __forceinline__ constexpr int sb_y_ct(int wv, int k) { constexpr int T[4][3] = {{0, 1, 2}, {1, 2, 3}, {0, 3, 4}, {1, 2, 4}}; return T[wv][k]; }
__device__ __forceinline__ constexpr int sb_y_pa(int wv, int i) { constexpr int T[4][4] = {{0, 1, 1, 2}, {1, 1, 2, 2}, {1, 1, 2, 2}, {2, 2, 2, 2}}; return T[wv][i]; }
__device__ __forceinline__ constexpr int sb_y_pb(int wv, int i) { constexpr int T[4][4] = {{0, 0, 1, 0}, {0, 1, 0, 1}, {0, 1, 0, 1}, {0, 1, 2, 2}}; return T[wv][i]; }

__device__ __forceinline__ void sb_feature_reduce(const double *W, const double *cf, int NR, int wv, const double *s_scale, double4_t (&acc)[15], int lane) {
    const int c16 = lane & 15, g4 = lane >> 4;
    const int nsteps = NR / 4;
    if (wv >= nsteps) return;
    double sc5[5];
#pragma unroll
    for (int t5 = 0; t5 < 4; t5++) sc5[t5] = s_scale[16 * t5 + c16];
    sc5[4] = (c16 < 2) ? s_scale[64 + c16] : ((c16 == 11 || c16 == 12) ? 1.0 : 0.0);
    const int col4 = (c16 < 2) ? 64 + c16 : (c16 == 11 ? VB_NPOSE : (c16 == 12 ? VB_NPOSE + 1 : VB_NPOSE + 2));
    double r0[5], r1[5], r2[5], r3[5], r4[5], c0, c1, c2, c3, c4;
#define SBF_ISSUE(ST, R, C)                                                                                                        \
    {                                                                                                                              \
        const int row_ = 4 * min((ST), nsteps - 1) + g4;                                                                           \
        const double *p0_ = W + (size_t)row_ * VB_WLD + c16, *p4_ = W + (size_t)row_ * VB_WLD + col4, *pc_ = cf + row_;             \
        asm volatile("global_load_dwordx2 %0, %6, off\n\tglobal_load_dwordx2 %1, %6, off offset:128\n\t"                           \
                     "global_load_dwordx2 %2, %6, off offset:256\n\tglobal_load_dwordx2 %3, %6, off offset:384\n\t"                \
                     "global_load_dwordx2 %4, %7, off\n\tglobal_load_dwordx2 %5, %8, off"                                          \
                     : "=&v"(R[0]), "=&v"(R[1]), "=&v"(R[2]), "=&v"(R[3]), "=&v"(R[4]), "=&v"(C) : "v"(p0_), "v"(p4_), "v"(pc_) : "memory"); \
    }
#define SBF_WAIT(N, R, C) asm volatile("s_waitcnt vmcnt(" #N ")" : "+v"(R[0]), "+v"(R[1]), "+v"(R[2]), "+v"(R[3]), "+v"(R[4]), "+v"(C) : : "memory");
#define SBF_STEP(R, C)                                                                                                             \
    {                                                                                                                              \
        double u[5];                                                                                                               \
        _Pragma("unroll") for (int t5 = 0; t5 < 5; t5++) u[t5] = R[t5] * C * sc5[t5];                                              \
        _Pragma("unroll") for (int i = 0; i < 15; i++) acc[i] = __builtin_amdgcn_mfma_f64_16x16x4f64(u[sb_t15_a(i)], u[sb_t15_b(i)], acc[i], 0, 0, 0); \
    }
    asm volatile("s_waitcnt vmcnt(0)" ::: "memory");
    SBF_ISSUE(wv, r0, c0) SBF_ISSUE(wv + 3, r1, c1) SBF_ISSUE(wv + 6, r2, c2) SBF_ISSUE(wv + 9, r3, c3)
    for (int st = wv; st < nsteps; st += 15) {
        SBF_ISSUE(st + 12, r4, c4) SBF_WAIT(24, r0, c0) SBF_STEP(r0, c0)
        if (st + 3 < nsteps) { SBF_ISSUE(st + 15, r0, c0) SBF_WAIT(24, r1, c1) SBF_STEP(r1, c1) }
        if (st + 6 < nsteps) { SBF_ISSUE(st + 18, r1, c1) SBF_WAIT(24, r2, c2) SBF_STEP(r2, c2) }
        if (st + 9 < nsteps) { SBF_ISSUE(st + 21, r2, c2) SBF_WAIT(24, r3, c3) SBF_STEP(r3, c3) }
        if (st + 12 < nsteps) { SBF_ISSUE(st + 24, r3, c3) SBF_WAIT(24, r4, c4) SBF_STEP(r4, c4) }
    }
    asm volatile("s_waitcnt vmcnt(0)" : "+v"(r0[0]), "+v"(r0[1]), "+v"(r0[2]), "+v"(r0[3]), "+v"(r0[4]), "+v"(r1[0]), "+v"(r1[1]), "+v"(r1[2]), "+v"(r1[3]), "+v"(r1[4]),
                                        "+v"(r2[0]), "+v"(r2[1]), "+v"(r2[2]), "+v"(r2[3]), "+v"(r2[4]), "+v"(r3[0]), "+v"(r3[1]), "+v"(r3[2]), "+v"(r3[3]), "+v"(r3[4]),
                                        "+v"(r4[0]), "+v"(r4[1]), "+v"(r4[2]), "+v"(r4[3]), "+v"(r4[4]), "+v"(c0), "+v"(c1), "+v"(c2), "+v"(c3), "+v"(c4) : : "memory");
#undef SBF_ISSUE
#undef SBF_WAIT
#undef SBF_STEP
}
template <int NTL, int PA, int PB>
__device__ __forceinline__ void sb_acc_sub(double *s_P, double *s_t, const double4_t *a, int lane, bool cauchy, double *s_dump) {
    const int c16 = lane & 15, g4 = lane >> 4;
    double v[NTL][4]; int off[NTL][4];
#pragma unroll
    for (int i = 0; i < NTL; i++)
#pragma unroll
        for (int q = 0; q < 4; q++) {
            const int r = 16 * ((PA >> (4 * i)) & 15) + g4 + 4 * q, c = 16 * ((PB >> (4 * i)) & 15) + c16;
            int o = (int)(s_dump - s_P) + lane;
            if (r < SB_NR && c <= r && c < SB_ND) o = sb_prow(r) + c;
            else if (cauchy && r == SB_NR && c < SB_ND) o = (int)(s_t - s_P) + c;
            off[i][q] = o;
            v[i][q] = s_P[o];
        }
#pragma unroll
    for (int i = 0; i < NTL; i++)
#pragma unroll
        for (int q = 0; q < 4; q++) s_P[off[i][q]] = v[i][q] - a[i][q];
}
template <int WV>
__device__ __forceinline__ void sb_y_chain(const double *s_band, const double *s_E, const double *s_zero, double4_t (&acc)[4], int lane) {
    const int c16 = lane & 15, g4 = lane >> 4;
    double4_t t[3];
#pragma unroll
    for (int ct = 0; ct < 3; ct++) t[ct] = double4_t{0, 0, 0, 0};
#pragma unroll 1
    for (int a = SB_NCH; a >= 1; a--) {
        const double *Ba = s_band + SB_BOFF(a);
        const int str = SB_BSTR(a);
        double yo[3][3];
#pragma unroll
        for (int ct = 0; ct < 3; ct++) {
            const int p = sb_band_pos(a, 16 * sb_y_ct(WV, ct) + c16);
#pragma unroll
            for (int ks = 0; ks < 3; ks++) {
                const int r = 4 * ks + g4;
                const double v = *((r < 9 && p >= 0) ? Ba + r * str + p : s_zero);
                yo[ks][ct] = v - t[ct][ks];
            }
        }
        if (a > 1) {
            const double *Na = s_E + 81 * (a - 2);
            double av[3];
#pragma unroll
            for (int ks = 0; ks < 3; ks++) { const int k = 4 * ks + g4; av[ks] = *((c16 < 9 && k < 9) ? Na + 9 * c16 + k : s_zero); }
#pragma unroll
            for (int ct = 0; ct < 3; ct++) t[ct] = double4_t{0, 0, 0, 0};
#pragma unroll
            for (int ks = 0; ks < 3; ks++)
#pragma unroll
                for (int ct = 0; ct < 3; ct++) t[ct] = __builtin_amdgcn_mfma_f64_16x16x4f64(av[ks], yo[ks][ct], t[ct], 0, 0, 0);
        }
#pragma unroll
        for (int ks = 0; ks < 3; ks++)
#pragma unroll
            for (int i = 0; i < sb_y_ntl(WV); i++) acc[i] = __builtin_amdgcn_mfma_f64_16x16x4f64(yo[ks][sb_y_pa(WV, i)], yo[ks][sb_y_pb(WV, i)], acc[i], 0, 0, 0);
    }
}
template <int WV>
__device__ __forceinline__ void sb_y_store(const double4_t (&acc)[4], double *s_P, double *s_t, int lane, double *s_dump) {
    constexpr int PA = sb_y_ct(WV, sb_y_pa(WV, 0)) | (sb_y_ct(WV, sb_y_pa(WV, 1)) << 4) | (sb_y_ct(WV, sb_y_pa(WV, 2)) << 8) | (sb_y_ct(WV, sb_y_pa(WV, 3)) << 12);
    constexpr int PB = sb_y_ct(WV, sb_y_pb(WV, 0)) | (sb_y_ct(WV, sb_y_pb(WV, 1)) << 4) | (sb_y_ct(WV, sb_y_pb(WV, 2)) << 8) | (sb_y_ct(WV, sb_y_pb(WV, 3)) << 12);
    sb_acc_sub<sb_y_ntl(WV), PA, PB>(s_P, s_t, &acc[0], lane, false, s_dump);
}

__device__ __forceinline__ bool sb_potrf9(double *Dp, double *linv, int lane) {
    const int r = min(lane, 8);
    double v[9];
#pragma unroll
    for (int c = 0; c < 9; c++) v[c] = Dp[9 * r + c];
    bool ok = true;
    double myinv = 1.0;
#pragma unroll
    for (int j = 0; j < 9; j++) {
        const double djj = readlane_f64(v[j], j);
        if (!(djj > 0.0)) ok = false;
        const double inv = rsqrt_h3(djj);
        const double lrj = v[j] * inv;
        v[j] = lrj;
        if (r == j) myinv = inv;
#pragma unroll
        for (int c = j + 1; c < 9; c++) v[c] -= lrj * readlane_f64(lrj, c);
    }
    if (lane < 9) {
#pragma unroll
        for (int c = 0; c < 9; c++) if (c <= r) Dp[9 * r + c] = v[c];
        linv[r] = myinv;
    }
    return ok;
}
#define SB_META(off, r, c, on) (((off) & 0x3fff) | ((r) << 14) | ((c) << 22) | ((on) ? 0 : (int)0x80000000))
extern "C" __global__ __launch_bounds__(SBT) void k_sb_table(int *tab) {
    const int tid = threadIdx.x, td = tid, ln = tid & 63;
    int t[SB_TAB_ROWS * 4];
    for (int k = 0; k < SB_TAB_ROWS * 4; k++) t[k] = -1;
    if (tid >= 192) {
        for (int u = 0; u < 13; u++) {
            const int q = min(ln + 64 * u, 809), a1 = q / 81, rem = q - 81 * a1, i = rem / 9, j = rem - 9 * i;
            const bool on = ln + 64 * u < 810 && j <= i;
            t[3 * u] = SB_META(SB_OFF_D + q, VB_NPOSE + 9 + 9 * a1 + i, VB_NPOSE + 9 + 9 * a1 + j, on);
            t[3 * u + 1] = 900 * a1 + 30 * (21 + i) + 21 + j;
            t[3 * u + 2] = a1 + 1 <= 9 ? 900 * (a1 + 1) + 30 * (6 + i) + 6 + j : -1;
        }
        for (int u = 0; u < 12; u++) {
            const int q = min(ln + 64 * u, 728), a1 = q / 81, rem = q - 81 * a1, i = rem / 9, j = rem - 9 * i;
            t[39 + 2 * u] = SB_META(SB_OFF_E + q, VB_NPOSE + 18 + 9 * a1 + i, VB_NPOSE + 9 + 9 * a1 + j, ln + 64 * u < 729);
            t[39 + 2 * u + 1] = 900 * (a1 + 1) + 30 * (21 + i) + 6 + j;
        }
    } else {
        for (int u = 0; u < 4; u++) {
            const int q = min(td + 192 * u, 755), nb = q / 36, e = q - 36 * nb, l1 = e / 6, l2 = e - 6 * l1;
            const bool dg = nb < 11;
            const int A = dg ? nb : nb - 10, Bf = dg ? nb : nb - 11, r = 6 * A + l1, c = 6 * Bf + l2;
            const int i0 = dg ? 900 * (A - 1) + 30 * (15 + l1) + 15 + l2 : 900 * Bf + 30 * (15 + l1) + l2, i1i = 900 * A + 30 * l1 + l2;
            const int j0 = dg ? 144 * (A - 1) + 12 * (6 + l1) + 6 + l2 : 144 * Bf + 12 * (6 + l1) + l2, j1 = 144 * A + 12 * l1 + l2;
            const bool h0 = !dg || A >= 1, h1 = dg && A <= 9;
            t[6 * u] = SB_META(SB_OFF_P + sb_prow(r) + c, r, c, td + 192 * u < 756 && c <= r);
            t[6 * u + 1] = 36 * (A * (A + 1) / 2 + Bf) + e;
            t[6 * u + 2] = h0 ? i0 : -1; t[6 * u + 3] = h1 ? i1i : -1; t[6 * u + 4] = h0 ? j0 : -1; t[6 * u + 5] = h1 ? j1 : -1;
        }
        for (int u = 0; u < 9; u++) {
            const int q = min(td + 192 * u, 1619), fb = q / 36, e = q - 36 * fb, l1 = e / 6, l2 = e - 6 * l1;
            int A2 = 0; while ((A2 + 1) * (A2 + 2) / 2 <= fb) A2++;
            const int Bf = fb - A2 * (A2 + 1) / 2, A = A2 + 2, r = 6 * A + l1, c = 6 * Bf + l2;
            t[24 + 2 * u] = SB_META(SB_OFF_P + sb_prow(r) + c, r, c, td + 192 * u < 1620);
            t[24 + 2 * u + 1] = 36 * (A * (A + 1) / 2 + Bf) + e;
        }
        for (int u = 0; u < 4; u++) {
            const int q = min(td + 192 * u, 674), i = q / 75, c = q - 75 * i, r = VB_NPOSE + i, Bf = c / 6, l2 = c - 6 * Bf;
            const int src = (c < VB_NPOSE) ? 30 * (6 + i) + (Bf == 0 ? l2 : 15 + l2) : 30 * (6 + i) + 6 + (c - VB_NPOSE);
            const bool hs = c >= VB_NPOSE || Bf <= 1;
            t[44 + 2 * u] = SB_META(SB_OFF_P + sb_prow(r) + c, r, c, td + 192 * u < 675 && c <= r);
            t[44 + 2 * u + 1] = hs ? src : -1;
        }
        for (int u = 0; u < 13; u++) {
            const int q = min(td + 192 * u, 2429), a1 = q / 243, rem = q - 243 * a1, i = rem / 27, pos = rem - 27 * i, a = a1 + 1;
            const int seg = pos / 6, m = pos - 6 * seg;
            const bool on = td + 192 * u < 2430 && (seg < 2 || (seg == 2 && a <= 9) || (seg >= 3 && a == 1));
            int s0, s1 = -1, c165;
            if (seg == 0) { s0 = 900 * a1 + 30 * (21 + i) + m; c165 = 6 * a1 + m; }
            else if (seg == 1) { s0 = 900 * a1 + 30 * (21 + i) + 15 + m; s1 = (a <= 9) ? 900 * a + 30 * (6 + i) + m : -1; c165 = 6 * a + m; }
            else if (seg == 2) { s0 = 900 * min(a, 9) + 30 * (6 + i) + 15 + m; c165 = 6 * (a + 1) + m; }
            else { s0 = 30 * (21 + i) + 6 + (pos - 18); c165 = VB_NPOSE + (pos - 18); }
            t[52 + 3 * u] = SB_META(SB_OFF_BAND + SB_BOFF(a) + i * SB_BSTR(a) + pos, VB_NPOSE + 9 * a + i, c165, on);
            t[52 + 3 * u + 1] = on ? s0 : -1;
            t[52 + 3 * u + 2] = s1;
        }
    }
    for (int k = 0; k < SB_TAB_ROWS; k++) for (int j = 0; j < 4; j++) tab[((size_t)k * 256 + tid) * 4 + j] = t[4 * k + j];
}

__device__ __forceinline__ void solve_sb_body(const VbBatch &b, int w) {
    const int tid = threadIdx.x, lane = tid & 63, wave = __builtin_amdgcn_readfirstlane(tid >> 6);
    if (w < 0) return;
    VbState *st = b.st + w;
    extern __shared__ double s_dyn[];
    double *s_P = s_dyn + SB_OFF_P, *s_D = s_dyn + SB_OFF_D, *s_E = s_dyn + SB_OFF_E, *s_band = s_dyn + SB_OFF_BAND;
    double *s_g = s_dyn + SB_OFF_VEC, *s_diag = s_g + SB_VLD, *s_scale = s_diag + SB_VLD, *s_y = s_scale + SB_VLD, *s_v = s_y + SB_VLD;
    double *s_t = s_dyn + SB_OFF_T, *s_linv = s_dyn + SB_OFF_LINV, *s_dinv = s_dyn + SB_OFF_DINV, *s_pan = s_dyn + SB_OFF_PAN, *s_u = s_dyn + SB_OFF_U, *s_w = s_dyn + SB_OFF_W;
    double *s_red = s_dyn + SB_OFF_RED;
    __shared__ int s_pcp[VB_P];
    __shared__ int s_flag[4];

    if (tid == 0) {
        const int done = st->done, iteration = st->iteration, reuse = st->reuse;
        const double gmn = st->gradient_max_norm, radius = st->radius;
        int go = 1;
        if (done) go = 0;
        else if (iteration >= b.max_iterations) { st->done = 1; st->termination = 0; go = 0; }
        else if (gmn <= b.gradient_tolerance) { st->done = 1; st->termination = 3; go = 0; }
        else if (radius <= b.min_radius) { st->done = 1; st->termination = 4; go = 0; }
        if (go) st->iteration = iteration + 1;
        s_flag[0] = go;
        s_flag[1] = go ? reuse : 1;
    }
    __syncthreads();
    if (!s_flag[0] || s_flag[1]) return;

    STAMP(1, 0);
    const int F = b.n_feat[w];
    const size_t FM = b.Fmax;
    const size_t ww = (size_t)st->ws * b.B + w;
    const double *Hpp = b.Hpp + ww * 66 * 36;
    const double *imuH = b.imuH + ww * 9000, *lidH = b.lidH + ww * 1440;
    const double *priorH = b.prior_H + (size_t)w * VB_PRIOR_LD * VB_PRIOR_LD;
    double *W = b.W + ww * FM * VB_WLD;
    double *cf = b.cf + (size_t)w * FM;
    const double *hf = b.hf + ww * FM, *gf = b.gf + ww * FM;
    const uint8_t *f_const = b.f_const + (size_t)w * FM;
    const int *f_wrow = b.f_wrow + (size_t)w * FM, *row_feat = b.row_feat + (size_t)w * FM;
    const int NR = b.n_rows[w];
    double *scale_g = b.scale + (size_t)w * (VB_P + FM), *diag_g = b.diag + (size_t)w * (VB_P + FM);
    double *grad_g = b.grad + (size_t)w * (VB_P + FM), *gn_g = b.gn + (size_t)w * (VB_P + FM);
    const double *g_in = b.g + ww * VB_P;
    const int *phdr = b.prior_hdr + (size_t)w * VB_PRIOR_HDR;
    const bool has_prior = phdr[0] != 0;
    const __amdgpu_buffer_rsrc_t rHpp = sb_rsrc(Hpp, 66 * 36 * 8), rImu = sb_rsrc(imuH, 9000 * 8), rLid = sb_rsrc(lidH, 1440 * 8), rPri = sb_rsrc(priorH, VB_PRIOR_LD * VB_PRIOR_LD * 8);

    for (int i = tid; i < SB_NCH * 81; i += SBT) s_D[i] = 0.0;
    for (int i = tid; i < 252 + 180 * (SB_NCH - 1); i += SBT) s_band[i] = 0.0;
    if (tid < 80) s_t[tid] = 0.0;
    if (tid == 0) s_P[sb_prow(SB_ND) + SB_ND] = 0.0;
    if (tid < VB_P) s_pcp[tid] = -1;
    __syncthreads();
    if (has_prior && tid < phdr[2]) {
        const int id = phdr[3 + tid], idx = phdr[51 + tid];
        if (id < VB_NF) { for (int k = 0; k < 6; k++) s_pcp[6 * id + k] = idx + k; }
        else if (id == VB_NF) { for (int k = 0; k < 9; k++) s_pcp[VB_NPOSE + k] = idx + k; }
    }
    const int scaling_ready = st->scaling_ready;
    double mu = st->mu;
    int tries = 0;
    bool solved = false;
    double Jg2 = 0, G2 = 0, g2 = 0;
    if (tid < VB_P) {
        int a, l; unperm(tid, a, l);
        const double dh = b.diagH[ww * VB_P + 15 * a + l];
        double sc;
        if (scaling_ready) sc = scale_g[tid]; else { sc = 1.0 / (1.0 + sqrt(dh)); scale_g[tid] = sc; }
        const double d = sqrt(fmin(fmax(sc * sc * dh, b.min_lm_diagonal), b.max_lm_diagonal));
        const double gs = g_in[15 * a + l] * sc;
        diag_g[tid] = d;
        const double gr = gs / d;
        grad_g[tid] = gr;
        g2 = gr * gr;
        s_scale[tid] = sc; s_diag[tid] = d; s_g[tid] = gs; s_v[tid] = gr / d;
    }
    for (int f = tid; f < F; f += SBT) {
        if (f_const[f]) continue;
        const double hfv = hf[f], gfv = gf[f];
        double sf;
        if (scaling_ready) sf = scale_g[VB_P + f]; else { sf = 1.0 / (1.0 + sqrt(hfv)); scale_g[VB_P + f] = sf; }
        const double d = sqrt(fmin(fmax(sf * sf * hfv, b.min_lm_diagonal), b.max_lm_diagonal));
        diag_g[VB_P + f] = d;
        const double gr = sf * gfv / d;
        grad_g[VB_P + f] = gr;
        g2 += gr * gr;
    }
    __threadfence_block();
    __syncthreads();
    int blk_i = 0;
    while ((blk_i + 1) * (blk_i + 2) / 2 <= tid) blk_i++;
    const int blk_j = tid - blk_i * (blk_i + 1) / 2;

    STAMP(1, 1);
    for (;;) {
        int ln = lane, bi = blk_i, bjm = blk_j, td = tid;
        asm volatile("" : "+v"(ln), "+v"(bi), "+v"(bjm), "+v"(td));
        double part = 0;
        if (td == 0) s_flag[2] = 1;
        if (wave == 3) {
            {
                double sv[25][2]; int meta[25];
                int ti[64];
                {
                    const int4 *tp = reinterpret_cast<const int4 *>(b.sb_tab) + td;
#pragma unroll
                    for (int k = 0; k < 16; k++) { const int4 v = tp[k * 256]; ti[4 * k] = v.x; ti[4 * k + 1] = v.y; ti[4 * k + 2] = v.z; ti[4 * k + 3] = v.w; }
                }
#pragma unroll
                for (int u = 0; u < 13; u++) {
                    sv[u][0] = sb_bload(rImu, ti[3 * u + 1]);
                    sv[u][1] = sb_bload(rImu, ti[3 * u + 2]);
                    meta[u] = ti[3 * u];
                }
#pragma unroll
                for (int u = 0; u < 12; u++) {
                    sv[13 + u][0] = sb_bload(rImu, ti[39 + 2 * u + 1]);
                    sv[13 + u][1] = 0.0;
                    meta[13 + u] = ti[39 + 2 * u];
                }
#pragma unroll
                for (int u = 0; u < 25; u++) {
                    if (meta[u] < 0) continue;
                    const int r = (meta[u] >> 14) & 255, c = (meta[u] >> 22) & 255;
                    const double val = (sv[u][0] + sv[u][1]) * s_scale[r] * s_scale[c];
                    part += ((r != c) ? 2.0 : 1.0) * s_v[r] * val * s_v[c];
                    s_dyn[meta[u] & 0x3fff] = val + ((r == c) ? mu : 0.0) * s_diag[r] * s_diag[r];
                }
            }
            bool ok = true;
#pragma unroll 1
            for (int a = SB_NCH; a >= 1; a--) {
                double *Da = s_D + 81 * (a - 1);
                ok = sb_potrf9(Da, s_linv + 9 * (a - 1), ln) && ok;
                if (a == 1) break;
                double *Ea = s_E + 81 * (a - 2);
                const int c = min(ln, 8);
                double x[9];
#pragma unroll
                for (int i = 0; i < 9; i++) {
                    double s = Ea[9 * i + c];
#pragma unroll
                    for (int j = 0; j < i; j++) s -= Da[9 * i + j] * x[j];
                    x[i] = s * s_linv[9 * (a - 1) + i];
                }
                if (ln < 9) {
#pragma unroll
                    for (int i = 0; i < 9; i++) Ea[9 * i + c] = x[i];
// ... 404 lines not shown
        {                                                                                                                          \
            const double *Wr_ = W + (size_t)min((F0) + g, NR - 1) * VB_WLD + c16;                                                \
            asm volatile("global_load_dwordx2 %0, %5, off\n\tglobal_load_dwordx2 %1, %5, off offset:128\n\t"                       \
                         "global_load_dwordx2 %2, %5, off offset:256\n\tglobal_load_dwordx2 %3, %5, off offset:384\n\t"            \
                         "global_load_dwordx2 %4, %5, off offset:512"                                                              \
                         : "=&v"(R[0]), "=&v"(R[1]), "=&v"(R[2]), "=&v"(R[3]), "=&v"(R[4]) : "v"(Wr_) : "memory");                  \
        }
#define FD_WAIT(N, R) asm volatile("s_waitcnt vmcnt(" #N ")" : "+v"(R[0]), "+v"(R[1]), "+v"(R[2]), "+v"(R[3]), "+v"(R[4]) : : "memory");
#define FD_STEP(F0, R)                                                                                                             \
        {                                                                                                                          \
            const int k = (F0) + g;                                                                                                \
            double dacc = 0;                                                                                                       \
            _Pragma("unroll") for (int t5 = 0; t5 < 5; t5++) dacc += R[t5] * sv[t5];                                               \
            _Pragma("unroll") for (int o = 8; o > 0; o >>= 1) dacc += __shfl_xor(dacc, o, 64);                                     \
            if (c16 == 0 && k < NR) cf[k] = dacc;                                                                                   \
        }
        constexpr int RS = 4 * 3;
        asm volatile("s_waitcnt vmcnt(0)" ::: "memory");
        FD_ISSUE(4 * w3, ra) FD_ISSUE(4 * w3 + RS, rb)
        for (int f0 = 4 * w3; f0 < NR; f0 += 3 * RS) {
            FD_ISSUE(f0 + 2 * RS, rc) FD_WAIT(10, ra) FD_STEP(f0, ra)
            if (f0 + RS < NR) { FD_ISSUE(f0 + 3 * RS, ra) FD_WAIT(10, rb) FD_STEP(f0 + RS, rb) }
            if (f0 + 2 * RS < NR) { FD_ISSUE(f0 + 4 * RS, rb) FD_WAIT(10, rc) FD_STEP(f0 + 2 * RS, rc) }
        }
        asm volatile("s_waitcnt vmcnt(0)" : "+v"(ra[0]), "+v"(ra[1]), "+v"(ra[2]), "+v"(ra[3]), "+v"(ra[4]), "+v"(rb[0]), "+v"(rb[1]), "+v"(rb[2]), "+v"(rb[3]), "+v"(rb[4]),
                                            "+v"(rc[0]), "+v"(rc[1]), "+v"(rc[2]), "+v"(rc[3]), "+v"(rc[4]) : : "memory");
#undef FD_ISSUE
#undef FD_WAIT
#undef FD_STEP
        __threadfence_block();
    }
    __syncthreads();
    if (tid < 9 * SB_NCH) {
        const int a1 = tid / 9, i = tid - 9 * a1;
        double s = 0;
#pragma unroll
        for (int k = 0; k < 9; k++) s += ((k >= i) ? s_D[81 * a1 + 9 * k + i] : 0.0) * s_w[9 * a1 + k];
        s_y[VB_NPOSE + 9 + tid] = s;
    }
    __syncthreads();
    STAMP(1, 10);
    double gy = 0, gn2 = 0;
    if (tid < VB_P) {
        const double y = s_y[tid], d = s_diag[tid];
        gn_g[tid] = -d * y;
        gy += s_g[tid] * y;
        gn2 += d * d * y * y;
    }
    for (int f = tid; f < F; f += SBT) {
        const int k = f_wrow[f];
        if (k < 0) continue;
        const double sf = scale_g[VB_P + f], df = diag_g[VB_P + f];
        const double hp = sf * sf * hf[f] + mu * df * df;
        const double gt = sf * gf[f];
        const double y = (gt - sf * cf[k]) / hp;
        gn_g[VB_P + f] = -df * y;
        gy += gt * y;
        gn2 += df * df * y * y;
    }
    block_sum2_sb(gy, gn2, s_red, gy, gn2);
    STAMP(1, 11);
    if (tid == 0) {
        st->grad_sqnorm = G2; st->Jg2 = Jg2; st->alpha = G2 / Jg2;
        st->gy = gy; st->gn_sqnorm = gn2; st->mu = mu; st->mu_used = mu;
        st->num_linear_solves += tries; st->solve_failed = 0; st->reuse = 1; st->scaling_ready = 1;
    }
}
extern "C" __global__ __launch_bounds__(SBT, 2) void k_solve_sb(VbBatch b) { solve_sb_body(b, vb_window(b)); }

extern "C" __global__ void k_finalize(VbBatch b) {
    const int w = blockIdx.x + b.w0, tid = threadIdx.x;
    if (tid >= VB_NF) return;
    const double *pose = b.pose + (size_t)w * 77, *sb = b.sb + (size_t)w * 99;
    const double *R0b = b.gauge_R0 + (size_t)w * 9, *P0b = b.gauge_P0 + (size_t)w * 3;
    double R00[9], y0[3], y00[3], rot[9];
    q_toR(q_load(pose + 3), R00);
    R2ypr(R0b, y0); R2ypr(R00, y00);
    double yd[3] = {y0[0] - y00[0], 0, 0};
    ypr2R(yd, rot);
    if (fabs(fabs(y0[1]) - 90) < 1.0 || fabs(fabs(y00[1]) - 90) < 1.0) {
        for (int i = 0; i < 3; i++) for (int j = 0; j < 3; j++) rot[3 * i + j] = R0b[3 * i] * R00[3 * j] + R0b[3 * i + 1] * R00[3 * j + 1] + R0b[3 * i + 2] * R00[3 * j + 2];
    }
    double Ri[9], Ro[9], d[3], o[3];
    q_toR(q_normalized(q_load(pose + 7 * tid + 3)), Ri);
    m3_mul(rot, Ri, Ro);
    for (int k = 0; k < 9; k++) b.out_Rs[((size_t)w * VB_NF + tid) * 9 + k] = Ro[k];
    d[0] = pose[7 * tid] - pose[0]; d[1] = pose[7 * tid + 1] - pose[1]; d[2] = pose[7 * tid + 2] - pose[2];
    m3_vec(rot, d, o);
    for (int k = 0; k < 3; k++) b.out_Ps[((size_t)w * VB_NF + tid) * 3 + k] = o[k] + P0b[k];
    m3_vec(rot, sb + 9 * tid, o);
    for (int k = 0; k < 3; k++) {
        b.out_Vs[((size_t)w * VB_NF + tid) * 3 + k] = o[k];
        b.out_Bas[((size_t)w * VB_NF + tid) * 3 + k] = sb[9 * tid + 3 + k];
        b.out_Bgs[((size_t)w * VB_NF + tid) * 3 + k] = sb[9 * tid + 6 + k];
    }
}

extern "C" __global__ void k_time_limit(VbBatch b, const int *mflag, int only_margin_old) {
    const int w = blockIdx.x + b.w0;
    if (threadIdx.x) return;
    if (only_margin_old && mflag[w] != 0) return;
    VbState *st = b.st + w;
    if (!st->done) { st->done = 1; st->termination = 0; }
}

extern "C" __global__ void k_reset(VbBatch b, int rewind_state) {
    const int w = blockIdx.x + b.w0, tid = threadIdx.x;
    if (blockIdx.x == 0 && b.live_ctl && tid < 128) b.live_ctl[tid] = 0;
    if (rewind_state) {
        if (tid < 77) b.pose[(size_t)w * 77 + tid] = b.pose_init[(size_t)w * 77 + tid];
        if (tid < 99) b.sb[(size_t)w * 99 + tid] = b.sb_init[(size_t)w * 99 + tid];
        for (int f = tid; f < b.Fmax; f += blockDim.x) b.feat[(size_t)w * b.Fmax + f] = b.feat_init[(size_t)w * b.Fmax + f];
    }
    if (tid == 0) {
        VbState s;
        s.x_cost = 0; s.cand_cost = 0; s.initial_cost = 0;
        s.radius = b.initial_radius; s.mu = 1e-8; s.alpha = 0; s.dogleg_step_norm = 0;
        s.x_norm = 0; s.gradient_max_norm = 1e300; s.grad_sqnorm = 0; s.Jg2 = 0; s.gy = 0; s.gn_sqnorm = 0; s.mu_used = 1e-8;
        s.model_cost_change = 0; s.relative_decrease = 0;
        s.iteration = 0; s.num_successful = 0; s.num_linear_solves = 0; s.num_consecutive_invalid = 0;
        s.termination = 0; s.done = 0; s.reuse = 0; s.need_linearize = 1; s.solve_failed = 0; s.scaling_ready = 0; s.started = 1; s.ws = 0; s.dev_error = 0;
        b.st[w] = s;
    }
}

extern "C" __global__ void k_hook_projection(const double *p0, const double *p1, const double *p2, double lam, const double *pi, const double *pj,
                                             double sqrt_info, double *out ) {
    if (threadIdx.x) return;
    double Ri[9], Rj[9], ric[9], pt[PT_LD];
    q_toR(q_load(p0 + 3), Ri); q_toR(q_load(p1 + 3), Rj); q_toR(q_load(p2 + 3), ric);
    pair_table(p0, Ri, p1, Rj, ric, p2, pt);
    projection_eval_pair<true>(pt, ric, p2, pi, pj, lam, sqrt_info, out, out + 2, out + 14, out + 26);
}
extern "C" __global__ void k_hook_projection_td(const double *in, double *out) {
    if (threadIdx.x) return;
    const double *p0 = in, *p1 = in + 7, *p2 = in + 14, *pi = in + 21, *pj = in + 24, *vi = in + 27, *vj = in + 29, *sc = in + 31;
    double Ri[9], Rj[9], ric[9];
    q_toR(q_load(p0 + 3), Ri); q_toR(q_load(p1 + 3), Rj); q_toR(q_load(p2 + 3), ric);
    projection_td_eval<true>(p0, Ri, p1, Rj, ric, p2, pi, pj, vi, vj, sc[1], sc[2], sc[3], sc[4], sc[5], sc[6], sc[0], sc[7], out, out + 2, out + 14, out + 38, out + 26, out + 40);
}
extern "C" __global__ void k_hook_imu(const double *p0, const double *p1, const double *p2, const double *p3, const double *rec, const double *G,
                                      double *out , double *scratch ) {
    if (threadIdx.x) return;
    double *Jr = scratch, *rr = scratch + 450;
    imu_raw_eval<true>(p0, p1, p2, p3, rec, G, rr, Jr);
    const double *S = rec + IMU_SQRT;
    for (int i = 0; i < 15; i++) { double s = 0; for (int m = 0; m < 15; m++) s += S[15 * i + m] * rr[m]; out[i] = s; }
    for (int i = 0; i < 15; i++) for (int c = 0; c < 30; c++) { double s = 0; for (int m = 0; m < 15; m++) s += S[15 * i + m] * Jr[30 * m + c]; out[15 + 30 * i + c] = s; }
}
extern "C" __global__ void k_hook_lidar(const double *p0, const double *p1, const double *qil, const double *til, const double *lc, double *out ) {
    if (threadIdx.x) return;
    lidar_between_eval<true>(p0, p1, q_load(qil), til, q_load(lc), lc + 4, out, out + 6, out + 42);
}
extern "C" __global__ void k_hook_prior(const int *hdr, const double *x0, const double *x, const double *J0, const double *r0, double *out) {
    __shared__ double s_dx[VB_PRIOR_LD];
    const int tid = threadIdx.x, n = hdr[0], nb = hdr[1];
    if (tid < VB_PRIOR_LD) s_dx[tid] = 0.0;
    __syncthreads();
    if (tid < nb) {
        const int size = hdr[2 + tid], idx = hdr[26 + tid];
        const double *a0 = x0 + 9 * tid, *a = x + 9 * tid;
        if (size == 7) {
            for (int k = 0; k < 3; k++) s_dx[idx + k] = a[k] - a0[k];
            Q dq = q_mul(q_inv(q_load(a0 + 3)), q_load(a + 3));
            const double sgn = (dq.w >= 0) ? 2.0 : -2.0;
            s_dx[idx + 3] = sgn * dq.x; s_dx[idx + 4] = sgn * dq.y; s_dx[idx + 5] = sgn * dq.z;
        } else {
            for (int k = 0; k < size; k++) s_dx[idx + k] = a[k] - a0[k];
        }
    }
    __syncthreads();
    for (int r = tid; r < n; r += blockDim.x) {
        double acc = r0[r];
        for (int c = 0; c < n; c++) acc += J0[(size_t)r * n + c] * s_dx[c];
        out[r] = acc;
    }
}
extern "C" __global__ void k_hook_edge(const double *pose, const double *cp, const double *pa, const double *pb, double *out ) {
    if (threadIdx.x) return;
    edge_eval<true>(pose, cp, pa, pb, out, out + 3);
}
extern "C" __global__ void k_hook_surf(const double *pose, const double *cp, const double *n, double d, double *out ) {
    if (threadIdx.x) return;
    surf_eval<true>(pose, cp, n, d, out, out + 1);
}
extern "C" __global__ void k_hook_plus(const double *x, const double *d, int kind, double *out) {
    if (threadIdx.x) return;
    if (kind == 0) pose_plus(x, d, out); else se3_plus(x, d, out);
}
```

vil_fusion_amd/csrc/vilf_kernels.hpp:

```cpp
#pragma once
#include <hip/hip_runtime.h>
#include "../../include/vilfusion.h"
#include "vilf_batch.hpp"

#define VILF_MAX_FEATURES_DEV 1000
static_assert(VILF_MAX_FEATURES_DEV == VILF_MAX_FEATURES, "the kernels' per-feature LDS arrays hold what the ABI admits");
#define VILF_LDS_CU_BYTES (160 * 1024)

#define SNT 512
#define SBT 256
#define IMU_PREP_NT 64
#define WIN1_NT 64
#define QL_NT 64
#define HOOK_NT 64
#define HOOK_PRIOR_NT 256
#define PREINT_NT 64

static_assert(VB_LIN_LDS_DOUBLES >= 10 * 512, "the IMU staging area precedes the chunk loop in the same region");
static_assert(VB_LIN_LDS_BYTES <= VILF_LDS_CU_BYTES / 2, "k_linearize: two workgroups per CU");

#define SOLVE_OFF_T 0
#define SOLVE_OFF_G (SOLVE_OFF_T + 66 * 256)
#define SOLVE_OFF_DIAG (SOLVE_OFF_G + VB_NPAD)
#define SOLVE_OFF_SCALE (SOLVE_OFF_DIAG + VB_NPAD)
#define SOLVE_OFF_Y (SOLVE_OFF_SCALE + VB_NPAD)
#define SOLVE_OFF_INVD (SOLVE_OFF_Y + VB_NPAD)
#define SOLVE_OFF_V (SOLVE_OFF_INVD + VB_NPAD)
#define SOLVE_OFF_RED (SOLVE_OFF_V + VB_NPAD)
#define SOLVE_OFF_CF (SOLVE_OFF_RED + SNT)
#define SOLVE_OFF_RNG (SOLVE_OFF_CF + VILF_MAX_FEATURES_DEV)
#define SOLVE_LDS_BYTES (SOLVE_OFF_RNG * 8 + VILF_MAX_FEATURES_DEV * 4)
static_assert(SOLVE_LDS_BYTES <= VILF_LDS_CU_BYTES, "k_solve");

#define SB_LDS_BYTES (SB_LDS_DOUBLES * 8)
#define SB_TAB_ROWS 23
static_assert(SB_LDS_BYTES <= VILF_LDS_CU_BYTES / 2, "k_solve_sb: two workgroups per CU");

#define PRIOR_PREP_LDS_BYTES ((MG_NK + 1) * (MG_NK + 1) * 8)
static_assert(MG_NK * (MG_NK | 1) * 8 <= PRIOR_PREP_LDS_BYTES && PRIOR_PREP_LDS_BYTES <= VILF_LDS_CU_BYTES / 2, "k_prior_prep");

#define MGS_OFF_S 0
#define MGS_OFF_Y (MGS_OFF_S + MG_MD * MG_MD)
#define MGS_OFF_IH (MGS_OFF_Y + MG_MD * (MG_NK + 1))
#define MGS_OFF_RED (MGS_OFF_IH + VILF_MAX_FEATURES_DEV)
#define MGS_OFF_W (MGS_OFF_RED + VB_NT)
#define MGS_FAST_LDS_BYTES ((MGS_OFF_W + MG_FCH * MG_RWP) * 8)
#define MGS_EXACT_LDS_DOUBLES (MG_MLDS * MG_MLDS)
#define MGS_EXACT_LDS_BYTES (MGS_EXACT_LDS_DOUBLES * 8)
static_assert(MGS_FAST_LDS_BYTES <= VILF_LDS_CU_BYTES / 3, "k_marg_schur, fast path: three workgroups per CU");
static_assert(MGS_EXACT_LDS_BYTES <= VILF_LDS_CU_BYTES && MGS_FAST_LDS_BYTES <= MGS_EXACT_LDS_BYTES, "k_marg_schur, exact path (its total is the kernel's attribute)");

#define MFT_ROWS 160
#define MFT_OFF_P 0
#define MFT_OFF_PAN (MFT_OFF_P + SB_NR * (SB_NR + 1) / 2)
#define MFT_OFF_LP (MFT_OFF_PAN + 4 * MFT_ROWS)
#define MFT_LDS_DOUBLES (MFT_OFF_LP + 4 * MFT_ROWS + 16)
#define MFT_LDS_BYTES (MFT_LDS_DOUBLES * 8)
static_assert(MFT_LDS_BYTES <= VILF_LDS_CU_BYTES / 2, "k_mf_chol_tiles");

#define QL_OFF_D 0
#define QL_OFF_E (QL_OFF_D + (MG_NK + 2) * QL_LPW)
#define QL_LDS_BYTES ((QL_OFF_E + (MG_NK + 2) * QL_LPW) * 8)
static_assert(QL_LPW <= QL_NT && QL_LDS_BYTES <= VILF_LDS_CU_BYTES, "k_mf_ql");

#define MGF_SMALL_N 78
#define MGF_SMALL_LDS_BYTES ((MGF_SMALL_N - 1) * (MGF_SMALL_N - 1) * 8)
#define MGF_LDS_BYTES ((MG_NK + 2) * (MG_NK + 2) * 8)
#define MFA_CH 64
#define MFA_LDS_EXTRA_BYTES (4 * MFA_CH * 8 + QL_ICAP * 2)
static_assert((MGF_SMALL_N - 1) * ((MGF_SMALL_N - 1) | 1) * 8 <= MGF_SMALL_LDS_BYTES && MG_NK * (MG_NK | 1) * 8 <= MGF_LDS_BYTES, "V fits its class");
static_assert(MGF_SMALL_LDS_BYTES + MFA_LDS_EXTRA_BYTES <= VILF_LDS_CU_BYTES / 3 && MGF_LDS_BYTES + MFA_LDS_EXTRA_BYTES <= VILF_LDS_CU_BYTES, "kept-block kernels");

extern "C" {
__global__ __launch_bounds__(IMU_PREP_NT) void k_imu_prep(int n, const double *cov, double *work, double *imu_rec);
__global__ __launch_bounds__(VB_NT) void k_prior_prep(VbBatch b, double *prior_H, double *prior_g, unsigned lds_bytes, const int *done4);
__global__ __launch_bounds__(VB_NT) void k_linearize(VbBatch b, int iteration_zero);
__global__ __launch_bounds__(VB_NT) void k_linearize_last(VbBatch b);
__global__ __launch_bounds__(VB_NT) void k_linearize_split(VbBatch b, int iteration_zero);
__global__ __launch_bounds__(SNT) void k_solve(VbBatch b);
__global__ __launch_bounds__(SBT) void k_sb_table(int *tab);
__global__ __launch_bounds__(SBT, 2) void k_solve_sb(VbBatch b);
__global__ void k_finalize(VbBatch b);
__global__ void k_time_limit(VbBatch b, const int *mflag, int only_margin_old);
__global__ void k_reset(VbBatch b, int rewind_state);
__global__ void k_hook_projection(const double *p0, const double *p1, const double *p2, double lam, const double *pi, const double *pj, double sqrt_info, double *out);
__global__ void k_hook_projection_td(const double *in, double *out);
__global__ void k_hook_imu(const double *p0, const double *p1, const double *p2, const double *p3, const double *rec, const double *G, double *out, double *scratch);
__global__ void k_hook_lidar(const double *p0, const double *p1, const double *qil, const double *til, const double *lc, double *out);
__global__ void k_hook_prior(const int *hdr, const double *x0, const double *x, const double *J0, const double *r0, double *out);
__global__ void k_hook_edge(const double *pose, const double *cp, const double *pa, const double *pb, double *out);
__global__ void k_hook_surf(const double *pose, const double *cp, const double *n, double d, double *out);
__global__ void k_hook_plus(const double *x, const double *d, int kind, double *out);
__global__ __launch_bounds__(VB_NT, 2) void k_marg_prepare(VbBatch b, VbMarg g);
__global__ __launch_bounds__(VB_NT) void k_marg_prepare_td(VbBatch b, VbMarg g);
__global__ __launch_bounds__(VB_NT, 3) void k_marg_schur(VbBatch b, VbMarg g, int exact);
__global__ __launch_bounds__(VB_NT) void k_mf_chol(VbBatch b, VbMarg g, int n_lo, int n_hi, int disable);
__global__ __launch_bounds__(VB_NT, 2) void k_mf_chol_tiles(VbBatch b, VbMarg g, int disable);
__global__ __launch_bounds__(VB_NT) void k_mf_tridiag(VbBatch b, VbMarg g, int n_lo, int n_hi);
__global__ __launch_bounds__(QL_NT) void k_mf_ql(VbBatch b, VbMarg g, int force_overflow);
__global__ __launch_bounds__(VB_NT) void k_mf_apply(VbBatch b, VbMarg g, int n_lo, int n_hi);
__global__ __launch_bounds__(VB_NT) void k_marg_finish(VbBatch b, VbMarg g, int n_lo, int n_hi, int only_flagged);
__global__ __launch_bounds__(VB_NT) void k_prior_keep(VbBatch b, VbMarg g);
}
__global__ void k_preintegrate(int n, vilf_imu_noise nz, const double *acc0, const double *gyr0, const double *ba, const double *bg, const int *n_samples, int max_samples,
                               const double *dt, const double *acc, const double *gyr, vilf_imu_preint *out);
```

vil_fusion_amd/csrc/vilf_marg.hip:

```cpp
#include "vilf_device.hpp"
#include "vilf_kernels.hpp"

using namespace vd;
#define NT VB_NT
__device__ __forceinline__ int pair_index_c(int i, int j) { return j * (j - 1) / 2 + i; }

__device__ __forceinline__ void rr_pair(int round, int k, int M, int &p, int &q) {
    int a = (k == 0) ? (M - 1) : (round + k) % (M - 1);
    int c = (round - k + (M - 1)) % (M - 1);
    p = min(a, c); q = max(a, c);
}

#ifdef VILF_STAMPS
__device__ long long mg_dbg[4 * 32];
#define MG_STAMP_WG 1500
#define MG_STAMP(kid, i) do { if (blockIdx.x == MG_STAMP_WG && threadIdx.x == 0) mg_dbg[(kid) * 32 + (i)] = __builtin_readcyclecounter(); } while (0)
extern "C" int vilf_debug_stamps_marg(long long *out128) { return hipMemcpyFromSymbol(out128, HIP_SYMBOL(mg_dbg), sizeof(long long) * 4 * 32) == hipSuccess ? 0 : -1; }
#define MG_ACC_DECL long long macc[6] = {0, 0, 0, 0, 0, 0}; long long macc_last = __builtin_readcyclecounter();
#define MG_ACC(i) do { const long long now_ = __builtin_readcyclecounter(); macc[i] += now_ - macc_last; macc_last = now_; } while (0)
#define MG_ACC_OUT(kid) do { if (blockIdx.x == MG_STAMP_WG && threadIdx.x == 0) for (int i_ = 0; i_ < 6; i_++) mg_dbg[(kid) * 32 + 24 + i_] = macc[i_]; } while (0)
#else
#define MG_STAMP(kid, i) do { } while (0)
#define MG_ACC_DECL
#define MG_ACC(i) do { } while (0)
// ... 59 lines not shown
    __shared__ double s_pm[10 * MG_PAIRM];
    __shared__ int s_off_pose[VB_NF], s_off_sb[2], s_off_ex, s_off_td, s_pmap[VB_PRIOR_LD], s_hdr[8], s_pst[VB_NPAIR], s_pcn[VB_NPAIR], s_pcl[VB_NPAIR];
    __shared__ double s_td;
    __shared__ double s_zero;
    __shared__ double s_part[4 * MG_PTRI];
    __shared__ __attribute__((aligned(16))) double s_rows[MG_GCH * MG_MROW];
    __shared__ int s_slots[MG_SLOTS], s_pend[10];
    int *info = g.info + (size_t)w * MG_INFO;
    const int F = b.n_feat[w];
    const size_t FM = b.Fmax, FC = b.FACmax;
    const int *phdr = b.prior_hdr + (size_t)w * VB_PRIOR_HDR;
    const int mode = g.mflag[w];
    const int have_prior = phdr[0];
    const int *f_start = b.f_start + (size_t)w * FM, *f_nobs = b.f_nobs + (size_t)w * FM, *f_fac0 = b.f_fac0 + (size_t)w * FM;
    int *f0rank = g.f0rank + (size_t)w * FM;
    double *st_feat = g.st_feat + (size_t)w * FM;

    if (tid < VB_NF) {
        const double *P = b.out_Ps + ((size_t)w * VB_NF + tid) * 3, *R = b.out_Rs + ((size_t)w * VB_NF + tid) * 9;
        for (int k = 0; k < 3; k++) s_pose[7 * tid + k] = P[k];
        q_store(s_pose + 7 * tid + 3, q_fromR(R));
        for (int k = 0; k < 9; k++) s_R[9 * tid + k] = R[k];
        for (int k = 0; k < 3; k++) { s_sb[9 * tid + k] = b.out_Vs[((size_t)w * VB_NF + tid) * 3 + k]; s_sb[9 * tid + 3 + k] = b.out_Bas[((size_t)w * VB_NF + tid) * 3 + k]; s_sb[9 * tid + 6 + k] = b.out_Bgs[((size_t)w * VB_NF + tid) * 3 + k]; }
    }
    if (tid == 33) s_td = b.td[w];
    if (tid == 32) {
        const double *ex = b.ex + (size_t)w * 7;
        q_toR(q_load(ex + 3), s_ric);
        for (int k = 0; k < 3; k++) s_ex[k] = ex[k];
        q_store(s_ex + 3, q_fromR(s_ric));
    }
    for (int f = tid; f < F; f += NT) {
        const double est = 1.0 / b.feat[(size_t)w * FM + f];
        const double v = est > 0 ? 1.0 / est : 1.0 / g.init_depth;
        st_feat[f] = v;
        if (f < MG_GCH * MG_MROW) s_rows[f] = v;
    }
    if (tid < VB_NPAIR) { const int *pt = b.pair_off + (size_t)w * VB_PTAB; const int v1 = pt[2 * tid + 1]; s_pst[tid] = pt[2 * tid]; s_pcn[tid] = v1 & 0xffffff; s_pcl[tid] = v1 >> 24; }
    __syncthreads();
    MG_STAMP(0, 1);
    if (tid < 77) g.st_pose[(size_t)w * 77 + tid] = s_pose[tid];
    if (tid < 99) g.st_sb[(size_t)w * 99 + tid] = s_sb[tid];
    if (tid < 7) g.st_ex[(size_t)w * 7 + tid] = s_ex[tid];

    __shared__ int s_fw[NT / 64], s_mf, s_maxobs;
    if (tid == 0) { s_mf = 0; s_maxobs = 0; s_zero = 0.0; }
    __syncthreads();
    MG_STAMP(0, 2);
    if (mode == 0) {
        for (int f0 = 0; f0 < F; f0 += NT) {
            const int f = f0 + tid;
            const int flag = (f < F && f_start[f] == 0) ? 1 : 0;
            const int nob = flag ? f_nobs[f] : 0;
            int incl = flag, mx = nob;
#pragma unroll
            for (int o = 1; o < 64; o <<= 1) { const int u = __shfl_up(incl, o, 64); if ((tid & 63) >= o) incl += u; }
#pragma unroll
            for (int o = 32; o > 0; o >>= 1) mx = max(mx, __shfl_xor(mx, o, 64));
            if ((tid & 63) == 63) s_fw[tid >> 6] = incl;
            if ((tid & 63) == 0 && mx > 0) atomicMax(&s_maxobs, mx);
            __syncthreads();
    MG_STAMP(0, 3);
            int off = s_mf;
            for (int k = 0; k < (tid >> 6); k++) off += s_fw[k];
            if (f < F) f0rank[f] = flag ? off + incl - 1 : -1;
            __syncthreads();
    MG_STAMP(0, 4);
            if (tid == 0) { int t = 0; for (int k = 0; k < NT / 64; k++) t += s_fw[k]; s_mf += t; }
            __syncthreads();
    MG_STAMP(0, 5);
        }
    } else for (int f = tid; f < F; f += NT) f0rank[f] = -1;
    if (tid == 0) {
        int status = 0, md = 0, mf = 0, n = 0, nb = 0;
        unsigned present = 0, drop = 0;
#define MG_SET(m, i) ((m) |= 1u << (i))
#define MG_HAS(m, i) (((m) >> (i)) & 1u)
        if (have_prior) for (int i = 0; i < phdr[2]; i++) MG_SET(present, phdr[3 + i]);
        if (mode == 0) {
            MG_SET(present, 0); MG_SET(present, 1); MG_SET(drop, 0);
            MG_SET(present, VB_NF); MG_SET(drop, VB_NF);
            if (b.use_lidar) MG_SET(drop, 1);
            const double *rec = b.imu + ((size_t)w * 10) * IMU_REC;
            if (rec[0] < 10.0) MG_SET(present, VB_NF + 1);
            mf = s_mf;
            for (int j = 1; j < s_maxobs && j < VB_NF; j++) MG_SET(present, j);
            if (mf > 0) MG_SET(present, 2 * VB_NF);
            if (mf > 0 && TD) MG_SET(present, 2 * VB_NF + 1);
        } else {
            if (!have_prior || !MG_HAS(present, VB_NF - 2)) status = 2;
            MG_SET(drop, VB_NF - 2);
        }
        int off = 0;
        for (int a = 0; a < VB_NF; a++) s_off_pose[a] = -1;
        s_off_sb[0] = s_off_sb[1] = -1; s_off_ex = -1; s_off_td = -1;
        for (int id = 0; id < 2 * VB_NF + 1 && status == 0; id++) if (MG_HAS(present, id) && MG_HAS(drop, id)) {
            if (id < VB_NF) { s_off_pose[id] = off; off += 6; } else if (id < 2 * VB_NF) { if (id - VB_NF < 2) s_off_sb[id - VB_NF] = off; else status = 3; off += 9; }
        }
        md = off;
        for (int id = 0; id < 2 * VB_NF + 2 && status == 0; id++) if (MG_HAS(present, id) && !MG_HAS(drop, id)) {
            int size = 7, loc = 6, sid;
            if (id < VB_NF) { s_off_pose[id] = off; }
            else if (id < 2 * VB_NF) { if (id - VB_NF < 2) s_off_sb[id - VB_NF] = off; else status = 3; size = 9; loc = 9; }
            else if (id == 2 * VB_NF) s_off_ex = off;
            else { s_off_td = off; size = 1; loc = 1; }
            if (id >= 2 * VB_NF) sid = id;
            else if (mode == 0) sid = id - 1;
            else { const int fr = id < VB_NF ? id : id - VB_NF; sid = (fr == VB_NF - 1) ? id - 1 : id; }
            if (nb >= 24) { status = 3; break; }
            info[8 + nb] = sid; info[32 + nb] = size; info[56 + nb] = off - md; info[80 + nb] = id;
            nb++;
            off += loc;
        }
        n = off - md;
        if (n > MG_NK || md > MG_MD) status = 3;
        int M = md + mf; M += (M & 1);
        if (M > g.Mcap) status = 3;
        info[0] = status; info[1] = md; info[2] = mf; info[3] = n; info[4] = md + mf; info[5] = nb; info[6] = M;
        s_hdr[0] = status; s_hdr[1] = md; s_hdr[2] = mf; s_hdr[3] = n;
    }
    __syncthreads();
    MG_STAMP(0, 6);
    if (s_hdr[0] != 0) return;
    const int md = s_hdr[1], n = s_hdr[3], nd = md + n;
    double *Hd = g.Hd + (size_t)w * MG_ND * MG_ND, *gd = g.gd + (size_t)w * MG_ND;
    for (int i = tid; i < MG_ND; i += NT) gd[i] = 0.0;
    if (tid < VB_PRIOR_LD) { s_dx[tid] = 0.0; s_pmap[tid] = -1; }
    __syncthreads();
    MG_STAMP(0, 7);
    if (have_prior && tid < phdr[2]) {
        const int id = phdr[3 + tid], size = phdr[27 + tid], idx = phdr[51 + tid];
        const double *x0 = b.prior_x0 + ((size_t)w * 24 + tid) * 9;
        const double *x = id < VB_NF ? s_pose + 7 * id : (id < 2 * VB_NF ? s_sb + 9 * (id - VB_NF) : (id == 2 * VB_NF ? s_ex : &s_td));
        const int doff = id < VB_NF ? s_off_pose[id] : (id < 2 * VB_NF ? s_off_sb[id - VB_NF] : (id == 2 * VB_NF ? s_off_ex : s_off_td));
        if (size == 7) {
            for (int k = 0; k < 3; k++) s_dx[idx + k] = x[k] - x0[k];
            Q dq = q_mul(q_inv(q_load(x0 + 3)), q_load(x + 3));
            const double sgn = (dq.w >= 0) ? 2.0 : -2.0;
            s_dx[idx + 3] = sgn * dq.x; s_dx[idx + 4] = sgn * dq.y; s_dx[idx + 5] = sgn * dq.z;
            for (int k = 0; k < 6; k++) s_pmap[idx + k] = doff + k;
        } else for (int k = 0; k < size; k++) { s_dx[idx + k] = x[k] - x0[k]; s_pmap[idx + k] = doff + k; }
    }
    for (int i = tid; i < 15 * 32; i += NT) s_J[i] = 0.0;
    if (tid < 72) s_lJ[tid] = 0.0;
    if (tid < 16) s_r[tid] = 0.0;
    if (tid < 8) s_lr[tid] = 0.0;
    __syncthreads();
    MG_STAMP(0, 8);
    __shared__ int s_pinv[MG_ND];
    if (tid < MG_ND) s_pinv[tid] = -1;
    __syncthreads();
    if (have_prior && tid < phdr[1] && s_pmap[tid] >= 0) s_pinv[s_pmap[tid]] = tid;
    if (mode == 0) {
        if (tid == 0) {
            const double *rec = b.imu + ((size_t)w * 10) * IMU_REC;
            if (rec[0] < 10.0) {
                double r[15];
                imu_raw_eval<true, 32, false>(s_pose, s_sb, s_pose + 7, s_sb + 9, rec, b.G, r, s_J);
                for (int k = 0; k < 15; k++) s_J[32 * k + 30] = r[k];
            }
        }
        if (tid == 64 && b.use_lidar) {
            const double *lc = b.lidar + ((size_t)w * 10) * 7;
            double Ji[36], Jj[36];
            lidar_between_eval<true>(s_pose, s_pose + 7, q_load(b.qil), b.til, q_load(lc), lc + 4, s_lr, Ji, Jj);
            for (int rr = 0; rr < 6; rr++) for (int c = 0; c < 6; c++) { s_lJ[12 * rr + c] = Ji[6 * rr + c]; s_lJ[12 * rr + 6 + c] = Jj[6 * rr + c]; }
        }
    }
    __syncthreads();
    MG_STAMP(0, 9);
    {
        const double *__restrict__ pH0 = b.prior_H + (size_t)w * VB_PRIOR_LD * VB_PRIOR_LD;
        double *__restrict__ Hd0 = Hd;
        for (int e0 = tid; e0 < MG_ND * MG_ND; e0 += 18 * NT) {
            double v6[18];
#pragma unroll
            for (int k = 0; k < 18; k++) {
                const int e = min(e0 + k * NT, MG_ND * MG_ND - 1), di = e / MG_ND, dj = e - MG_ND * di;
                const int pi = s_pinv[di], pj = s_pinv[dj];
                v6[k] = (pi >= 0 && pj >= 0) ? pH0[pi * VB_PRIOR_LD + pj] : 0.0;
            }
#pragma unroll
            for (int k = 0; k < 18; k++) { const int e = e0 + k * NT; if (e < MG_ND * MG_ND) Hd0[e] = v6[k]; }
        }
    }
    __syncthreads();
    {
        const double *S = b.imu + ((size_t)w * 10) * IMU_REC + IMU_SQRT;
        double acc[2] = {0, 0};
        int e0 = tid, e1 = tid + NT;
        for (int t = 0; t < 2; t++) {
            const int e = t ? e1 : e0;
            if (e < 15 * 31) { const int row = e / 31, col = e - 31 * row; double s = 0; for (int m2 = row; m2 < 15; m2++) s += S[15 * row + m2] * s_J[32 * m2 + col]; acc[t] = s; }
        }
        __syncthreads();
    MG_STAMP(0, 10);
        if (e0 < 15 * 31) s_J[32 * (e0 / 31) + (e0 % 31)] = acc[0];
        if (e1 < 15 * 31) s_J[32 * (e1 / 31) + (e1 % 31)] = acc[1];
    }
    __syncthreads();
    MG_STAMP(0, 11);
    double *Mb = g.Mbuf + (size_t)w * MG_MROW * FC;
    if (mode == 0) {
        int ntot = 0;
#pragma unroll
        for (int jj = 0; jj < 10; jj++) ntot += s_pcn[pair_index_c(0, jj + 1)];
        for (int t = tid; t < ntot; t += NT) {
            int rem = t, q = -1;
#pragma unroll
            for (int jj = 0; jj < 10; jj++) {
                const int pj = pair_index_c(0, jj + 1), nseg = s_pcn[pj];
                if (q < 0) { if (rem < nseg) q = VB_SLOT(s_pcl[pj], s_pst[pj] + rem); else rem -= nseg; }
            }
            const double *rec = b.facrec + ((size_t)w * FC + q) * 8;
            double pts_i[3], pts_j[3];
#pragma unroll
            for (int k = 0; k < 3; k++) { pts_i[k] = rec[k]; pts_j[k] = rec[3 + k]; }
            const long long ra = __double_as_longlong(rec[6]), rb = __double_as_longlong(rec[7]);
            const int f = (int)(ra & 0xffffffffll), slot = (int)(ra >> 32), fj = (int)((rb >> 8) & 255);
            if (t < MG_SLOTS) s_slots[t] = slot;
            double r[2], Ji[12], Jj[12], Jf[2], Jex[12], Jtd[2] = {0.0, 0.0};
            if (TD) {
                const int oj = b.ps_obs[(size_t)w * FC + q], oi = b.f_obs0[(size_t)w * FM + f];
                const double *vi = b.obs_vel + ((size_t)w * b.Omax + oi) * 2, *vj = b.obs_vel + ((size_t)w * b.Omax + oj) * 2;
                projection_td_eval<true>(s_pose, s_R, s_pose + 7 * fj, s_R + 9 * fj, s_ric, s_ex, pts_i, pts_j, vi, vj, s_td, b.obs_ctd[(size_t)w * b.Omax + oi], b.obs_ctd[(size_t)w * b.Omax + oj],
                                         b.obs_row[(size_t)w * b.Omax + oi] - b.row_half, b.obs_row[(size_t)w * b.Omax + oj] - b.row_half, b.tr_over_row, st_feat[f], b.sqrt_info, r, Ji, Jj, Jf, Jex, Jtd);
            } else
            projection_eval<true>(s_pose, s_R, s_pose + 7 * fj, s_R + 9 * fj, s_ric, s_ex, pts_i, pts_j, f < MG_GCH * MG_MROW ? s_rows[f] : st_feat[f], b.sqrt_info, r, Ji, Jj, Jf, Jex);
            double rho0, sw;
            cauchy(r[0] * r[0] + r[1] * r[1], b.cauchy_b, rho0, sw);
            {
                typedef double mg_double2 __attribute__((ext_vector_type(2)));
                mg_double2 *row2 = reinterpret_cast<mg_double2 *>(Mb + (size_t)slot * MG_MROW);
#pragma unroll
                for (int k = 0; k < 12; k += 2) { row2[k >> 1] = mg_double2{sw * Ji[k], sw * Ji[k + 1]}; row2[6 + (k >> 1)] = mg_double2{sw * Jj[k], sw * Jj[k + 1]}; row2[12 + (k >> 1)] = mg_double2{sw * Jex[k], sw * Jex[k + 1]}; }
                row2[18] = mg_double2{sw * Jf[0], sw * Jf[1]};
                row2[19] = mg_double2{sw * r[0], sw * r[1]};
                row2[20] = mg_double2{sw * Jtd[0], sw * Jtd[1]};
            }
        }
    }
    __syncthreads();
    MG_STAMP(0, 12);
    if (mode == 0) {
        const int *ps_slot = b.ps_slot + (size_t)w * FC;
        if (tid < 10) { int c = 0; for (int k = 0; k <= tid; k++) c += s_pcn[pair_index_c(0, k + 1)]; s_pend[tid] = c; }
        __syncthreads();
        const int ntot = s_pend[9];
        const int wave = tid >> 6, lane = tid & 63, l16 = lane & 15, l4 = lane >> 4;
        const int sub = l4 & 1;
        auto comp_of = [&](int c) -> int { return c < 18 ? 12 * (c / 6) + (c % 6) + 6 * sub : (c == 18 ? 40 + sub : (c == 19 ? 38 + sub : -1)); };
        const int comp0 = comp_of(l16), comp1 = comp_of(16 + l16);
        mgp_double4 T00 = {0.0, 0.0, 0.0, 0.0}, T10 = {0.0, 0.0, 0.0, 0.0}, T11 = {0.0, 0.0, 0.0, 0.0};
        int jj = 0;
        int pu = 0;
        while ((pu + 1) * (pu + 2) / 2 <= min(tid, MG_PTRI - 1)) pu++;
        const int pv = min(tid, MG_PTRI - 1) - pu * (pu + 1) / 2;
        auto flush = [&]() {
            double *mine = s_part + wave * MG_PTRI;
#pragma unroll
            for (int q = 0; q < 4; q++) {
                const int u0 = l4 + 4 * q, u1 = 16 + l4 + 4 * q, v0 = l16, v1 = 16 + l16;
                if (v0 <= u0) mine[u0 * (u0 + 1) / 2 + v0] = T00[q];
                if (u1 < 20) mine[u1 * (u1 + 1) / 2 + v0] = T10[q];
                if (u1 < 20 && v1 <= u1) mine[u1 * (u1 + 1) / 2 + v1] = T11[q];
            }
            T00 = mgp_double4{0.0, 0.0, 0.0, 0.0}; T10 = T00; T11 = T00;
            lds_barrier();
            if (tid < MG_PTRI) s_pm[jj * MG_PAIRM + 20 * pv + pu] = ((s_part[tid] + s_part[MG_PTRI + tid]) + s_part[2 * MG_PTRI + tid]) + s_part[3 * MG_PTRI + tid];
            lds_barrier();
            jj++;
        };
        typedef double mg_double2 __attribute__((ext_vector_type(2)));
        constexpr int RW2 = MG_MROW / 2, NLD = (MG_GCH * RW2 + NT - 1) / NT;
        static_assert(MG_MROW % 2 == 0, "rows as 16-byte pieces");
        mg_double2 vals[NLD];
        auto request = [&](int t0) {
            const int nr = min(MG_GCH, ntot - t0);
            int off[NLD];
            if (t0 + nr <= MG_SLOTS) {
#pragma unroll
                for (int k = 0; k < NLD; k++) { const int idx = min(tid + NT * k, nr * RW2 - 1), r = idx / RW2; off[k] = s_slots[t0 + r] * RW2 + (idx - RW2 * r); }
            } else {
#pragma unroll 1
                for (int k = 0; k < NLD; k++) {
                    const int idx = min(tid + NT * k, nr * RW2 - 1), r = idx / RW2;
                    int rem = t0 + r, q = 0;
                    for (int kk = 0; kk < 10; kk++) { const int pj = pair_index_c(0, kk + 1), nseg = s_pcn[pj]; if (rem >= 0) { if (rem < nseg) { q = VB_SLOT(s_pcl[pj], s_pst[pj] + rem); rem = -1; } else rem -= nseg; } }
                    const int o = ps_slot[q] * RW2 + (idx - RW2 * r);
#pragma unroll
                    for (int k2 = 0; k2 < NLD; k2++) if (k2 == k) off[k2] = o;
                }
            }
            const mg_double2 *Mb2 = reinterpret_cast<const mg_double2 *>(Mb);
#pragma unroll
            for (int k = 0; k < NLD; k++) vals[k] = Mb2[(size_t)off[k]];
        };
        MG_ACC_DECL
        if (ntot > 0) request(0);
        for (int t0 = 0; t0 < ntot; t0 += MG_GCH) {
            const int nr = min(MG_GCH, ntot - t0);
            MG_ACC(0);
            {
                mg_double2 *s_rows2 = reinterpret_cast<mg_double2 *>(s_rows);
#pragma unroll
                for (int k = 0; k < NLD; k++) { const int idx = tid + NT * k; if (idx < nr * RW2) s_rows2[idx] = vals[k]; }
            }
            MG_ACC(1);
            lds_barrier();
            if (t0 + MG_GCH < ntot) request(t0 + MG_GCH);
            MG_ACC(2);
            while (jj < 10) {
                const int ps = jj ? s_pend[jj - 1] : 0, pe = s_pend[jj];
                if (pe > ps && ps >= t0 + nr) break;
                const int lo = max(ps, t0) - t0, hi = min(pe, t0 + nr) - t0;
                for (int fr0 = lo + 8 * wave; fr0 < hi; fr0 += 32) {
                    double a0[4], a1[4];
#pragma unroll
                    for (int k4 = 0; k4 < 4; k4++) {
// ... 1123 lines not shown
```

Baseline: 1.088 million.

## Split IMU and lidar factor evaluation into per-wave roles with LDS-staged records

The IMU and lidar Jacobian evaluation, previously done by a few threads in one wave each, is split into role subsets (residual, rotation blocks, bias blocks) assigned to different waves so the serial per-factor work runs concurrently. IMU records and lidar constraints are prefetched into LDS before the barrier, the sqrt-information loads are hoisted earlier, and table indices are mapped to the lower triangle. The aim is to shorten the critical serial linearization stage. In exchange the code grows more complex, uses extra LDS, and adds a debug hook kernel for validation.

```diff
diff --git a/vil_fusion_amd/csrc/vilf_api.hip b/vil_fusion_amd/csrc/vilf_api.hip
--- a/vil_fusion_amd/csrc/vilf_api.hip
+++ b/vil_fusion_amd/csrc/vilf_api.hip
@@ -1251,6 +1251,43 @@
     return VILF_OK;
 }
 
+extern "C" int vilf_debug_imu_stage_lanes(vilf_handle *h, int n, int layout, const double *states, const vilf_imu_preint *pre, const int *valid,
+                                          const vilf_lidar_constraint *lc, double *out, double *sqrt_info_out) {
+    if (!h || n <= 0 || (layout != 0 && layout != 1) || !states || !pre || !valid || !lc || !out) return VILF_ERR_INVALID_ARGUMENT;
+    HIPCHECK(h, hipSetDevice(h->device));
+    if (!h->resident) lidar_extrinsic(h->opts, h->batch);
+    const size_t sn = (size_t)n, o_rec = 32 * sn, o_cov = o_rec + IMU_REC * sn, o_lc = o_cov + 225 * sn, o_c = o_lc + 7 * sn, n_in = o_c + 16;
+    std::vector<double> in(n_in, 0.0);
+    std::memcpy(in.data(), states, 32 * sn * 8);
+    for (size_t i = 0; i < sn; i++) {
+        pack_imu_rec(pre + i, &in[o_rec + IMU_REC * i]);
+        in[o_rec + IMU_REC * i + 287] = valid[i] ? 1.0 : 0.0;
+        std::memcpy(&in[o_cov + 225 * i], pre[i].covariance, 225 * 8);
+        for (int k = 0; k < 4; k++) in[o_lc + 7 * i + k] = lc[i].q[k];
+        for (int k = 0; k < 3; k++) in[o_lc + 7 * i + 4 + k] = lc[i].t[k];
+    }
+    for (int k = 0; k < 3; k++) { in[o_c + k] = h->opts.G[k]; in[o_c + 8 + k] = h->batch.til[k]; }
+    for (int k = 0; k < 4; k++) in[o_c + 4 + k] = h->batch.qil[k];
+    double *d = nullptr;
+    int rc = VILF_OK;
+    if (hipMalloc(&d, (n_in + HOOK_STAGE_LD * sn) * 8) != hipSuccess) rc = VILF_ERR_DEVICE;
+    double *d_out = d + n_in;
+    if (rc == VILF_OK && (hipMemcpyAsync(d, in.data(), n_in * 8, hipMemcpyHostToDevice, h->stream) != hipSuccess ||
+                          hipMemsetAsync(d_out, 0, HOOK_STAGE_LD * sn * 8, h->stream) != hipSuccess)) rc = VILF_ERR_DEVICE;
+    if (rc == VILF_OK) {
+        hipLaunchKernelGGL(k_imu_prep, dim3((unsigned)((n + 3) / 4)), dim3(IMU_PREP_NT), 0, h->stream, n, d + o_cov, (double *)nullptr, d + o_rec);
+        hipLaunchKernelGGL(k_hook_stage_lanes, dim3(1), dim3(VB_NT), 0, h->stream, n, layout, d, d + o_rec, d + o_lc, d + o_c, d + o_c + 4, d + o_c + 8, d_out);
+        if (hipGetLastError() != hipSuccess) rc = VILF_ERR_DEVICE;
+    }
+    std::vector<double> rec(sqrt_info_out ? IMU_REC * sn : 0);
+    if (rc == VILF_OK && hipMemcpyAsync(out, d_out, HOOK_STAGE_LD * sn * 8, hipMemcpyDeviceToHost, h->stream) != hipSuccess) rc = VILF_ERR_DEVICE;
+    if (rc == VILF_OK && sqrt_info_out && hipMemcpyAsync(rec.data(), d + o_rec, IMU_REC * sn * 8, hipMemcpyDeviceToHost, h->stream) != hipSuccess) rc = VILF_ERR_DEVICE;
+    if (rc == VILF_OK && hipStreamSynchronize(h->stream) != hipSuccess) rc = VILF_ERR_DEVICE;
+    if (rc == VILF_OK && sqrt_info_out) for (size_t i = 0; i < sn; i++) std::memcpy(sqrt_info_out + 225 * i, &rec[IMU_REC * i + IMU_SQRT], 225 * 8);
+    if (d) hipFree(d);
+    return rc;
+}
+
 extern "C" int vilf_eval_edge(vilf_handle *h, const double pose[7], const double cp[3], const double a[3], const double bb[3], double r[3], double *J) {
     if (!h) return VILF_ERR_INVALID_ARGUMENT;
     if (hook_buf(h, 128) != VILF_OK) return VILF_ERR_DEVICE;
diff --git a/vil_fusion_amd/csrc/vilf_device.hpp b/vil_fusion_amd/csrc/vilf_device.hpp
--- a/vil_fusion_amd/csrc/vilf_device.hpp
+++ b/vil_fusion_amd/csrc/vilf_device.hpp
@@ -436,6 +436,152 @@
     }
 }
 
+enum : unsigned {
+    IMU_ROLE_RES = 1,
+    IMU_ROLE_QLR = 2,
+    IMU_ROLE_DBG = 4,
+    IMU_ROLE_RJ = 8,
+    IMU_ROLE_SBI = 16,
+    IMU_ROLE_J = 32,
+    IMU_ROLE_ALL = 63,
+    LID_ROLE_RES = 1, LID_ROLE_JI = 2, LID_ROLE_JJ = 4, LID_ROLE_ALL = 7
+};
+VD unsigned imu_wave_roles(int wave) {
+    return wave == 3 ? (IMU_ROLE_RES | IMU_ROLE_QLR) : wave == 0 ? (IMU_ROLE_DBG | IMU_ROLE_RJ | IMU_ROLE_J) : wave == 2 ? IMU_ROLE_SBI : 0u;
+}
+VD unsigned lidar_wave_roles(int wave) { return wave == 1 ? (unsigned)LID_ROLE_ALL : 0u; }
+
+template <bool JAC, int LD>
+VD void imu_raw_roles(unsigned roles, const double *posei, const double *sbi, const double *posej, const double *sbj, const double *rec, const double *G,
+                      double *r, double *Jraw) {
+    const double dt = rec[0];
+    const double *dp = rec + 1, *dv = rec + 8, *lba = rec + 11, *lbg = rec + 14;
+    const double *dp_dba = rec + 17, *dp_dbg = rec + 26, *dq_dbg = rec + 35, *dv_dba = rec + 44, *dv_dbg = rec + 53;
+    Q Qi = q_load(posei + 3), Qj = q_load(posej + 3), delta_q = q_load(rec + 4);
+    Q Qi_inv = q_inv(Qi);
+    Q cdq{0, 0, 0, 1}, QiQj{0, 0, 0, 1};
+    double dbg[3] = {sbi[6] - lbg[0], sbi[7] - lbg[1], sbi[8] - lbg[2]};
+    if (roles & (IMU_ROLE_RES | IMU_ROLE_QLR | IMU_ROLE_RJ)) {
+        double th[3];
+        m3_vec(dq_dbg, dbg, th);
+        cdq = q_mul(delta_q, q_delta(th[0], th[1], th[2]));
+    }
+    if (roles & (IMU_ROLE_RES | IMU_ROLE_RJ)) QiQj = q_mul(Qi_inv, Qj);
+    auto put = [&](int r0, int c0, const double *m, double s) {
+        for (int i = 0; i < 3; i++) for (int j = 0; j < 3; j++) Jraw[(r0 + i) * LD + c0 + j] = s * m[3 * i + j];
+    };
+    if (roles & IMU_ROLE_RES) {
+        double dba[3] = {sbi[3] - lba[0], sbi[4] - lba[1], sbi[5] - lba[2]};
+        double t1[3], t2[3], cdv[3], cdp[3];
+        m3_vec(dv_dba, dba, t1); m3_vec(dv_dbg, dbg, t2);
+        for (int k = 0; k < 3; k++) cdv[k] = dv[k] + t1[k] + t2[k];
+        m3_vec(dp_dba, dba, t1); m3_vec(dp_dbg, dbg, t2);
+        for (int k = 0; k < 3; k++) cdp[k] = dp[k] + t1[k] + t2[k];
+        double a[3], b[3], ra[3], rb[3];
+        for (int k = 0; k < 3; k++) {
+            a[k] = 0.5 * G[k] * dt * dt + posej[k] - posei[k] - sbi[k] * dt;
+            b[k] = G[k] * dt + sbj[k] - sbi[k];
+        }
+        q_rot(Qi_inv, a, ra);
+        q_rot(Qi_inv, b, rb);
+        Q rq = q_mul(q_inv(cdq), QiQj);
+        r[0] = ra[0] - cdp[0]; r[1] = ra[1] - cdp[1]; r[2] = ra[2] - cdp[2];
+        r[3] = 2 * rq.x; r[4] = 2 * rq.y; r[5] = 2 * rq.z;
+        r[6] = rb[0] - cdv[0]; r[7] = rb[1] - cdv[1]; r[8] = rb[2] - cdv[2];
+        for (int k = 0; k < 3; k++) { r[9 + k] = sbj[3 + k] - sbi[3 + k]; r[12 + k] = sbj[6 + k] - sbi[6 + k]; }
+        if (JAC) {
+            double S[9];
+            skew3(ra, S); put(0, 3, S, 1.0);
+            skew3(rb, S); put(6, 3, S, 1.0);
+        }
+    }
+    if (!JAC) return;
+    if (roles & IMU_ROLE_QLR) {
+        double B[9];
+        qleft_qright_br(q_mul(q_inv(Qj), Qi), cdq, B); put(3, 3, B, -1.0);
+    }
+    if (roles & IMU_ROLE_DBG) {
+        double L[9], T[9];
+        qleft_br(q_mul(q_mul(q_inv(Qj), Qi), delta_q), L);
+        m3_mul(L, dq_dbg, T);
+        put(3, 12, T, -1.0);
+    }
+    if (roles & IMU_ROLE_RJ) {
+        double B[9];
+        qleft_br(q_mul(q_inv(cdq), QiQj), B); put(3, 18, B, 1.0);
+    }
+    if (roles & (IMU_ROLE_SBI | IMU_ROLE_J)) {
+        double RiT[9];
+        q_toR(Qi_inv, RiT);
+        const double I3[9] = {1, 0, 0, 0, 1, 0, 0, 0, 1};
+        if (roles & IMU_ROLE_SBI) {
+            put(0, 0, RiT, -1.0);
+            put(0, 6, RiT, -dt); put(0, 9, dp_dba, -1.0); put(0, 12, dp_dbg, -1.0);
+            put(6, 6, RiT, -1.0); put(6, 9, dv_dba, -1.0); put(6, 12, dv_dbg, -1.0);
+            put(9, 9, I3, -1.0); put(12, 12, I3, -1.0);
+        }
+        if (roles & IMU_ROLE_J) {
+            put(0, 15, RiT, 1.0);
+            put(6, 21, RiT, 1.0); put(9, 24, I3, 1.0); put(12, 27, I3, 1.0);
+        }
+    }
+}
+
+template <bool JAC>
+VD void lidar_between_roles(unsigned roles, const double *posei, const double *posej, const Q &qil, const double *til, const Q &lq, const double *lt,
+                            double *r, double *Ji, double *Jj) {
+    Q Qi = q_load(posei + 3), Qj = q_load(posej + 3);
+    Q Qi_inv = q_inv(Qi), qli = q_inv(qil);
+    double dP[3] = {posej[0] - posei[0], posej[1] - posei[1], posej[2] - posei[2]};
+    double a[3];
+    q_rot(Qi_inv, dP, a);
+    Q qm = q_mul(qil, lq);
+    Q cdq = q_mul(qm, qli);
+    if (roles & LID_ROLE_RES) {
+        double tli[3], b[3], c[3], rp[3];
+        q_rot(qli, til, tli); tli[0] = -tli[0]; tli[1] = -tli[1]; tli[2] = -tli[2];
+        q_rot(qm, tli, b);
+        c[0] = a[0] - til[0] - b[0]; c[1] = a[1] - til[1] - b[1]; c[2] = a[2] - til[2] - b[2];
+        q_rot(qli, c, rp);
+        Q rq = q_mul(q_inv(cdq), q_mul(Qi_inv, Qj));
+        r[0] = 10.0 * (rp[0] - lt[0]); r[1] = 10.0 * (rp[1] - lt[1]); r[2] = 10.0 * (rp[2] - lt[2]);
+        r[3] = 100.0 * 2.0 * rq.x; r[4] = 100.0 * 2.0 * rq.y; r[5] = 100.0 * 2.0 * rq.z;
+    }
+    if (!JAC) return;
+    double Rm[9];
+    if (roles & (LID_ROLE_JI | LID_ROLE_JJ)) q_toR(q_mul(qli, Qi_inv), Rm);
+    if (roles & LID_ROLE_JI) {
+#pragma unroll
+        for (int k = 0; k < 36; k++) Ji[k] = 0;
+        double Rl[9], S[9], T[9], B[9];
+        q_toR(qli, Rl);
+        skew3(a, S);
+        m3_mul(Rl, S, T);
+        qleft_qright_br(q_mul(q_inv(Qj), Qi), cdq, B);
+#pragma unroll
+        for (int i = 0; i < 3; i++)
+#pragma unroll
+            for (int j = 0; j < 3; j++) {
+                Ji[6 * i + j] = -Rm[3 * i + j];
+                Ji[6 * i + 3 + j] = T[3 * i + j];
+                Ji[6 * (3 + i) + 3 + j] = -B[3 * i + j];
+            }
+    }
+    if (roles & LID_ROLE_JJ) {
+#pragma unroll
+        for (int k = 0; k < 36; k++) Jj[k] = 0;
+        double Cm[9];
+        qleft_br(q_mul(q_inv(cdq), q_mul(Qi_inv, Qj)), Cm);
+#pragma unroll
+        for (int i = 0; i < 3; i++)
+#pragma unroll
+            for (int j = 0; j < 3; j++) {
+                Jj[6 * i + j] = Rm[3 * i + j];
+                Jj[6 * (3 + i) + 3 + j] = Cm[3 * i + j];
+            }
+    }
+}
+
 template <bool JAC>
 VD void edge_eval(const double *pose, const double *cp, const double *pa, const double *pb, double *r, double *J) {
     Q q = q_load(pose);
diff --git a/vil_fusion_amd/csrc/vilf_kernels.hip b/vil_fusion_amd/csrc/vilf_kernels.hip
--- a/vil_fusion_amd/csrc/vilf_kernels.hip
+++ b/vil_fusion_amd/csrc/vilf_kernels.hip
@@ -10,7 +10,9 @@
 #ifdef VILF_STAMPS
 #define STAMP(kid, i) do { if (b.dbg && blockIdx.x == 0 && threadIdx.x == 0) b.dbg[(kid) * 32 + (i)] = __builtin_readcyclecounter(); } while (0)
 #define TICK() __builtin_readcyclecounter()
+#define WSTAMP(i) do { if (JAC && b.dbg && blockIdx.x == 0 && (threadIdx.x & 63) == 0) b.dbg[(i)] = __builtin_readcyclecounter(); } while (0)
 #else
+#define WSTAMP(i) do { } while (0)
 #define STAMP(kid, i) do { } while (0)
 #define TICK() 0LL
 #endif
@@ -278,8 +280,20 @@
     return b.live_buf[(size_t)((i - 1) & 1) * b.B + blockIdx.x];
 }
 #define LIN_LDS_DOUBLES VB_LIN_LDS_DOUBLES
+#define LIN_REC_LD 63
+#define LIN_U_LD 513
+#define LIN_REC_OFF (10 * LIN_U_LD)
+#define LIN_LIDC_OFF (LIN_REC_OFF + 10 * LIN_REC_LD)
+#define LIN_STAGED (10 * LIN_REC_LD + 10 * 7)
+static_assert(LIN_REC_OFF + LIN_STAGED <= LIN_LDS_DOUBLES && LIN_STAGED <= 3 * NT, "the staged records fit behind s_U in the chunk's region (its zero slot is written when they are dead); three entries per thread");
 
 __device__ __forceinline__ double pd_get(const double *pd, const int *s_pcn, int p, int e) { const double v = pd[p * VB_PAIRD + e]; return (s_pcn[p] > 0) ? v : 0.0; }
+
+__device__ __forceinline__ int imu_lower(int idx) {
+    if (idx < 0) return idx;
+    const int a = idx / 900, e = idx - 900 * a, p = e / 30, c = e - 30 * p;
+    return 900 * a + 30 * max(p, c) + min(p, c);
+}
 
 __device__ __forceinline__ int pair_elem(int row, int col) {
     if (row < 6) {
@@ -446,6 +460,16 @@
         }
         __threadfence_block();
     }
+    double *s_rec = s_dyn + LIN_REC_OFF, *s_lidc = s_dyn + LIN_LIDC_OFF;
+    const bool stage_lid = do_lp && b.use_lidar;
+    double staged[3];
+#pragma unroll
+    for (int q = 0; q < 3; q++) {
+        const int i = tid + NT * q, ir = min(i, 10 * LIN_REC_LD - 1), k = ir / LIN_REC_LD, e = ir - LIN_REC_LD * k;
+        const double *src = b.imu + ((size_t)w * 10 + k) * IMU_REC + (e < IMU_SQRT ? e : 287);
+        if (stage_lid && i >= 10 * LIN_REC_LD) src = b.lidar + (size_t)w * 70 + min(i - 10 * LIN_REC_LD, 69);
+        staged[q] = *src;
+    }
     unsigned long long cls_mask;
     int my_pst, my_pcn;
     {
@@ -456,78 +480,109 @@
         const bool mine = lane < VB_NPAIR && (v1 >> 24) == wave && my_pcn > 0;
         cls_mask = __ballot(mine);
     }
-    if (JAC && do_imu) for (int i = tid; i < 10 * 512; i += NT) s_U[i] = 0.0;
+    if (JAC && do_imu) for (int i = tid; i < 10 * LIN_U_LD; i += NT) s_U[i] = 0.0;
+#pragma unroll
+    for (int q = 0; q < 3; q++) if (tid + NT * q < LIN_STAGED) s_rec[tid + NT * q] = staged[q];
     __syncthreads();
     if (tid < VB_NF) q_toR(q_load(s_pose + 7 * tid + 3), s_R + 9 * tid);
     if (tid == 32) { q_toR(q_load(ex + 3), s_ric); s_tic[0] = ex[0]; s_tic[1] = ex[1]; s_tic[2] = ex[2]; }
     prior_setup(b, w, s_pose, s_sb, s_pcol, s_dx, tid);
+    double avS[5][4], Srow[15];
+    if (JAC) {
+        if (do_imu)
+#pragma unroll
+        for (int t5 = 0; t5 < 5; t5++) {
+            const double *S = b.imu + ((size_t)w * 10 + ((wave + 4 * t5) >> 1)) * IMU_REC + IMU_SQRT;
+#pragma unroll
+            for (int s4 = 0; s4 < 4; s4++) {
+                const int i = lane & 15, kk = 4 * s4 + (lane >> 4);
+                const double v = S[15 * min(i, 14) + min(kk, 14)];
+                avS[t5][s4] = (i < 15 && kk < 15) ? v : 0.0;
+            }
+        }
+    } else if (do_imu && tid < 150) {
+        const double *S = b.imu + ((size_t)w * 10 + tid / 15) * IMU_REC + IMU_SQRT + 15 * (tid % 15);
+#pragma unroll
+        for (int m = 0; m < 15; m++) Srow[m] = S[m];
+    }
     if (tid >= 128 && tid < 128 + VB_NPAIR) {
         const int p = tid - 128;
         int j = 1; while (j * (j + 1) / 2 <= p) j++;
         const int i = p - j * (j - 1) / 2;
         pair_table(s_pose + 7 * i, s_R + 9 * i, s_pose + 7 * j, s_R + 9 * j, s_ric, s_tic, s_pt + PT_LD * p);
+        WSTAMP(24);
     }
     LSTAMP(1);
+    WSTAMP(16 + wave);
 
     double cost_local = 0;
-    if (do_imu && tid >= 192 && tid < 202) {
-        const int k = tid - 192;
-        const double *rec = b.imu + ((size_t)w * 10 + k) * IMU_REC;
-        if (rec[287] != 0.0) {
+    if (do_imu && lane < 10) {
+        const int k = lane;
+        const unsigned roles = JAC ? imu_wave_roles(wave) : (wave == 3 ? (unsigned)IMU_ROLE_RES : 0u);
+        const double *rec = s_rec + LIN_REC_LD * k;
+        if (roles && rec[LIN_REC_LD - 1] != 0.0) {
             double r[15];
-            if (JAC) {
-                imu_raw_eval<true, 32, false>(s_pose + 7 * k, s_sb + 9 * k, s_pose + 7 * (k + 1), s_sb + 9 * (k + 1), rec, b.G, r, s_U + 512 * k);
-                for (int m = 0; m < 15; m++) s_U[512 * k + 32 * m + 30] = r[m];
-            } else {
-                imu_raw_eval<false>(s_pose + 7 * k, s_sb + 9 * k, s_pose + 7 * (k + 1), s_sb + 9 * (k + 1), rec, b.G, r, nullptr);
-                double acc = 0;
-                for (int i = 0; i < 15; i++) { double sq = 0; for (int m = i; m < 15; m++) sq += rec[IMU_SQRT + 15 * i + m] * r[m]; acc += sq * sq; }
-                cost_local += 0.5 * acc;
-            }
-        }
-    }
-    if (do_lp && tid >= 64 && tid < 74) {
-        const int k = tid - 64;
+            imu_raw_roles<JAC, 32>(roles, s_pose + 7 * k, s_sb + 9 * k, s_pose + 7 * (k + 1), s_sb + 9 * (k + 1), rec, b.G, r, s_U + LIN_U_LD * k);
+            if (roles & IMU_ROLE_RES) for (int m = 0; m < 15; m++) s_U[LIN_U_LD * k + 32 * m + 30] = r[m];
+        }
+    }
+    if (do_lp && lane < 10) {
+        const int k = lane;
+        const unsigned roles = JAC ? lidar_wave_roles(wave) : (wave == 1 ? (unsigned)LID_ROLE_RES : 0u);
         if (b.use_lidar) {
-            const double *lc = b.lidar + ((size_t)w * 10 + k) * 7;
-            if (JAC) {
+            if (roles) {
+                const double *lc = s_lidc + 7 * k;
                 double Ji[36], Jj[36];
-                lidar_between_eval<true>(s_pose + 7 * k, s_pose + 7 * (k + 1), q_load(b.qil), b.til, q_load(lc), lc + 4, s_lidr + 6 * k, Ji, Jj);
-                for (int rr = 0; rr < 6; rr++) for (int c = 0; c < 6; c++) { s_lidJ[72 * k + 12 * rr + c] = Ji[6 * rr + c]; s_lidJ[72 * k + 12 * rr + 6 + c] = Jj[6 * rr + c]; }
-            } else lidar_between_eval<false>(s_pose + 7 * k, s_pose + 7 * (k + 1), q_load(b.qil), b.til, q_load(lc), lc + 4, s_lidr + 6 * k, nullptr, nullptr);
-        } else {
+                lidar_between_roles<JAC>(roles, s_pose + 7 * k, s_pose + 7 * (k + 1), q_load(b.qil), b.til, q_load(lc), lc + 4, s_lidr + 6 * k, Ji, Jj);
+                if (JAC && (roles & LID_ROLE_JI)) for (int rr = 0; rr < 6; rr++) for (int c = 0; c < 6; c++) s_lidJ[72 * k + 12 * rr + c] = Ji[6 * rr + c];
+                if (JAC && (roles & LID_ROLE_JJ)) for (int rr = 0; rr < 6; rr++) for (int c = 0; c < 6; c++) s_lidJ[72 * k + 12 * rr + 6 + c] = Jj[6 * rr + c];
+            }
+        } else if (wave == 1) {
             if (JAC) for (int e = 0; e < 72; e++) s_lidJ[72 * k + e] = 0;
             for (int e = 0; e < 6; e++) s_lidr[6 * k + e] = 0;
         }
     }
+    WSTAMP(20 + wave);
     lds_barrier();
     LSTAMP(2);
-    if (JAC && do_imu) for (int task = wave; task < 20; task += 4) {
-        const int k = task >> 1, ct = task & 1;
-        double *Xk = s_U + 512 * k;
-        const double *S = b.imu + ((size_t)w * 10 + k) * IMU_REC + IMU_SQRT;
-        double av[4], bv[4];
-#pragma unroll
-        for (int s4 = 0; s4 < 4; s4++) {
-            const int i = lane & 15, kk = 4 * s4 + (lane >> 4);
-            av[s4] = (i < 15 && kk < 15) ? S[15 * i + kk] : 0.0;
-            bv[s4] = Xk[32 * kk + 16 * ct + (lane & 15)];
-        }
-        double4_t acc = {0, 0, 0, 0};
-#pragma unroll
-        for (int s4 = 0; s4 < 4; s4++) acc = __builtin_amdgcn_mfma_f64_16x16x4f64(av[s4], bv[s4], acc, 0, 0, 0);
-#pragma unroll
-        for (int q = 0; q < 4; q++) Xk[32 * ((lane >> 4) + 4 * q) + 16 * ct + (lane & 15)] = acc[q];
+    if (JAC && do_imu) {
+#pragma unroll
+        for (int t5 = 0; t5 < 5; t5++) {
+            const int task = wave + 4 * t5, k = task >> 1, ct = task & 1;
+            double *Xk = s_U + LIN_U_LD * k;
+            double bv[4];
+#pragma unroll
+            for (int s4 = 0; s4 < 4; s4++) bv[s4] = Xk[32 * (4 * s4 + (lane >> 4)) + 16 * ct + (lane & 15)];
+            double4_t acc = {0, 0, 0, 0};
+#pragma unroll
+            for (int s4 = 0; s4 < 4; s4++) acc = __builtin_amdgcn_mfma_f64_16x16x4f64(avS[t5][s4], bv[s4], acc, 0, 0, 0);
+#pragma unroll
+            for (int q = 0; q < 4; q++) Xk[32 * ((lane >> 4) + 4 * q) + 16 * ct + (lane & 15)] = acc[q];
+        }
+    }
+    if (!JAC && do_imu && tid < 150) {
+        const int k = tid / 15, i = tid - 15 * k;
+        if (s_rec[LIN_REC_LD * k + LIN_REC_LD - 1] != 0.0) {
+            double sq = 0;
+#pragma unroll
+            for (int m = 0; m < 15; m++) if (m >= i) sq += Srow[m] * s_U[LIN_U_LD * k + 32 * m + 30];
+            s_U[LIN_U_LD * k + 32 * i + 31] = sq;
+        }
     }
     lds_barrier();
     LSTAMP(3);
+    if (!JAC && do_imu && tid >= 192 && tid < 202 && s_rec[LIN_REC_LD * (tid - 192) + LIN_REC_LD - 1] != 0.0) {
+        double acc = 0;
+        for (int i = 0; i < 15; i++) { const double sq = s_U[LIN_U_LD * (tid - 192) + 32 * i + 31]; acc += sq * sq; }
+        cost_local += 0.5 * acc;
+    }
     if (JAC) {
         double *imuH = b.imuH + ww * 9000, *imug = b.imug + ww * 300;
         if (do_imu)
         for (int task = wave; task < 30; task += 4) {
             const int k = task / 3, tt = task - 3 * k;
             const int ti = (tt == 0) ? 0 : 1, tj = (tt == 2) ? 1 : 0;
-            const double *Xk = s_U + 512 * k;
+            const double *Xk = s_U + LIN_U_LD * k;
             double4_t acc = {0, 0, 0, 0};
 #pragma unroll
             for (int s4 = 0; s4 < 4; s4++) {
@@ -537,7 +592,7 @@
 #pragma unroll
             for (int q = 0; q < 4; q++) {
                 const int p = 16 * ti + (lane >> 4) + 4 * q, c = 16 * tj + (lane & 15);
-                if (p < 30 && c < 30) { imuH[900 * k + 30 * p + c] = acc[q]; if (ti != tj) imuH[900 * k + 30 * c + p] = acc[q]; }
+                if (p < 30 && c <= p) imuH[900 * k + 30 * p + c] = acc[q];
                 if (p == 30 && c < 30) imug[30 * k + c] = acc[q];
                 if (p == 30 && c == 30) cost_local += 0.5 * acc[q];
             }
@@ -1200,7 +1255,7 @@
                 for (int u = 0; u < 5; u++) {
                     const int t = min(t0 + u * SNT, 5 * 900 - 1);
                     const int k2 = t / 900, src = 900 * (2 * k2 + par) + (t - 900 * k2);
-                    o[u] = b.lut_imu[src]; v[u] = imuH[src];
+                    o[u] = b.lut_imu[src]; v[u] = imuH[imu_lower(src)];
                 }
 #pragma unroll
                 for (int u = 0; u < 5; u++) {
@@ -1612,13 +1667,13 @@
             const int q = min(ln + 64 * u, 809), a1 = q / 81, rem = q - 81 * a1, i = rem / 9, j = rem - 9 * i;
             const bool on = ln + 64 * u < 810 && j <= i;
             t[3 * u] = SB_META(SB_OFF_D + q, VB_NPOSE + 9 + 9 * a1 + i, VB_NPOSE + 9 + 9 * a1 + j, on);
-            t[3 * u + 1] = 900 * a1 + 30 * (21 + i) + 21 + j;
-            t[3 * u + 2] = a1 + 1 <= 9 ? 900 * (a1 + 1) + 30 * (6 + i) + 6 + j : -1;
+            t[3 * u + 1] = imu_lower(900 * a1 + 30 * (21 + i) + 21 + j);
+            t[3 * u + 2] = a1 + 1 <= 9 ? imu_lower(900 * (a1 + 1) + 30 * (6 + i) + 6 + j) : -1;
         }
         for (int u = 0; u < 12; u++) {
             const int q = min(ln + 64 * u, 728), a1 = q / 81, rem = q - 81 * a1, i = rem / 9, j = rem - 9 * i;
             t[39 + 2 * u] = SB_META(SB_OFF_E + q, VB_NPOSE + 18 + 9 * a1 + i, VB_NPOSE + 9 + 9 * a1 + j, ln + 64 * u < 729);
-            t[39 + 2 * u + 1] = 900 * (a1 + 1) + 30 * (21 + i) + 6 + j;
+            t[39 + 2 * u + 1] = imu_lower(900 * (a1 + 1) + 30 * (21 + i) + 6 + j);
         }
     } else {
         for (int u = 0; u < 4; u++) {
@@ -1630,7 +1685,7 @@
             const bool h0 = !dg || A >= 1, h1 = dg && A <= 9;
             t[6 * u] = SB_META(SB_OFF_P + sb_prow(r) + c, r, c, td + 192 * u < 756 && c <= r);
             t[6 * u + 1] = 36 * (A * (A + 1) / 2 + Bf) + e;
-            t[6 * u + 2] = h0 ? i0 : -1; t[6 * u + 3] = h1 ? i1i : -1; t[6 * u + 4] = h0 ? j0 : -1; t[6 * u + 5] = h1 ? j1 : -1;
+            t[6 * u + 2] = h0 ? imu_lower(i0) : -1; t[6 * u + 3] = h1 ? imu_lower(i1i) : -1; t[6 * u + 4] = h0 ? j0 : -1; t[6 * u + 5] = h1 ? j1 : -1;
         }
         for (int u = 0; u < 9; u++) {
             const int q = min(td + 192 * u, 1619), fb = q / 36, e = q - 36 * fb, l1 = e / 6, l2 = e - 6 * l1;
@@ -1644,7 +1699,7 @@
             const int src = (c < VB_NPOSE) ? 30 * (6 + i) + (Bf == 0 ? l2 : 15 + l2) : 30 * (6 + i) + 6 + (c - VB_NPOSE);
             const bool hs = c >= VB_NPOSE || Bf <= 1;
             t[44 + 2 * u] = SB_META(SB_OFF_P + sb_prow(r) + c, r, c, td + 192 * u < 675 && c <= r);
-            t[44 + 2 * u + 1] = hs ? src : -1;
+            t[44 + 2 * u + 1] = hs ? imu_lower(src) : -1;
         }
         for (int u = 0; u < 13; u++) {
             const int q = min(td + 192 * u, 2429), a1 = q / 243, rem = q - 243 * a1, i = rem / 27, pos = rem - 27 * i, a = a1 + 1;
@@ -1656,8 +1711,8 @@
             else if (seg == 2) { s0 = 900 * min(a, 9) + 30 * (6 + i) + 15 + m; c165 = 6 * (a + 1) + m; }
             else { s0 = 30 * (21 + i) + 6 + (pos - 18); c165 = VB_NPOSE + (pos - 18); }
             t[52 + 3 * u] = SB_META(SB_OFF_BAND + SB_BOFF(a) + i * SB_BSTR(a) + pos, VB_NPOSE + 9 * a + i, c165, on);
-            t[52 + 3 * u + 1] = on ? s0 : -1;
-            t[52 + 3 * u + 2] = s1;
+            t[52 + 3 * u + 1] = on ? imu_lower(s0) : -1;
+            t[52 + 3 * u + 2] = imu_lower(s1);
         }
     }
     for (int k = 0; k < SB_TAB_ROWS; k++) for (int j = 0; j < 4; j++) tab[((size_t)k * 256 + tid) * 4 + j] = t[4 * k + j];
@@ -2368,6 +2423,57 @@
     if (threadIdx.x) return;
     lidar_between_eval<true>(p0, p1, q_load(qil), til, q_load(lc), lc + 4, out, out + 6, out + 42);
 }
+extern "C" __global__ __launch_bounds__(NT) void k_hook_stage_lanes(int n, int layout, const double *state, const double *rec, const double *lc, const double *G,
+                                                                     const double *qil, const double *til, double *out) {
+    __shared__ double s_r[10 * 16], s_sq[10 * 16];
+    const int tid = threadIdx.x, lane = tid & 63, wave = tid >> 6;
+    for (int f0 = 0; f0 < n; f0 += 10) {
+        int k = -1;
+        unsigned ir = 0, lr = 0;
+        if (layout == 0) {
+            if (tid < 60) { k = tid / 6; ir = 1u << (tid - 6 * k); }
+            else if (tid >= 64 && tid < 94) { k = (tid - 64) / 3; lr = 1u << (tid - 64 - 3 * k); }
+        } else if (lane < 10) { k = lane; ir = imu_wave_roles(wave); lr = lidar_wave_roles(wave); }
+        const int f = f0 + k;
+        if (k >= 0 && f < n) {
+            const double *x = state + 32 * (size_t)f, *rc = rec + (size_t)IMU_REC * f, *c = lc + 7 * (size_t)f;
+            double *o = out + (size_t)HOOK_STAGE_LD * f;
+            if (ir && rc[287] != 0.0) {
+                double r[15];
+                imu_raw_roles<true, 30>(ir, x, x + 7, x + 16, x + 23, rc, G, r, o);
+                if (ir & IMU_ROLE_RES) for (int m = 0; m < 15; m++) { o[450 + m] = r[m]; s_r[16 * k + m] = r[m]; }
+            }
+            if (lr) {
+                double Ji[36], Jj[36];
+                lidar_between_roles<true>(lr, x, x + 16, q_load(qil), til, q_load(c), c + 4, o + 537, Ji, Jj);
+                if (lr & LID_ROLE_JI) for (int e = 0; e < 36; e++) o[465 + e] = Ji[e];
+                if (lr & LID_ROLE_JJ) for (int e = 0; e < 36; e++) o[501 + e] = Jj[e];
+            }
+        }
+        __syncthreads();
+        if (tid < 150 && f0 + tid / 15 < n) {
+            const int kk = tid / 15, i = tid - 15 * kk;
+            const double *rc = rec + (size_t)IMU_REC * (f0 + kk);
+            if (rc[287] != 0.0) {
+                double Srow[15];
+#pragma unroll
+                for (int m = 0; m < 15; m++) Srow[m] = rc[IMU_SQRT + 15 * i + m];
+                double sq = 0;
+#pragma unroll
+                for (int m = 0; m < 15; m++) if (m >= i) sq += Srow[m] * s_r[16 * kk + m];
+                s_sq[16 * kk + i] = sq;
+            }
+        }
+        __syncthreads();
+        if (tid < 10 && f0 + tid < n && rec[(size_t)IMU_REC * (f0 + tid) + 287] != 0.0) {
+            double acc = 0, cost = 0;
+            for (int i = 0; i < 15; i++) { const double sq = s_sq[16 * tid + i]; acc += sq * sq; }
+            cost += 0.5 * acc;
+            out[(size_t)HOOK_STAGE_LD * (f0 + tid) + 543] = cost;
+        }
+        __syncthreads();
+    }
+}
 extern "C" __global__ void k_hook_prior(const int *hdr, const double *x0, const double *x, const double *J0, const double *r0, double *out) {
     __shared__ double s_dx[VB_PRIOR_LD];
     const int tid = threadIdx.x, n = hdr[0], nb = hdr[1];
diff --git a/vil_fusion_amd/csrc/vilf_kernels.hpp b/vil_fusion_amd/csrc/vilf_kernels.hpp
--- a/vil_fusion_amd/csrc/vilf_kernels.hpp
+++ b/vil_fusion_amd/csrc/vilf_kernels.hpp
@@ -14,6 +14,7 @@
 #define QL_NT 64
 #define HOOK_NT 64
 #define HOOK_PRIOR_NT 256
+#define HOOK_STAGE_LD 544
 #define PREINT_NT 64
 
 static_assert(VB_LIN_LDS_DOUBLES >= 10 * 512, "the IMU staging area precedes the chunk loop in the same region");
@@ -87,6 +88,8 @@
 __global__ void k_hook_projection_td(const double *in, double *out);
 __global__ void k_hook_imu(const double *p0, const double *p1, const double *p2, const double *p3, const double *rec, const double *G, double *out, double *scratch);
 __global__ void k_hook_lidar(const double *p0, const double *p1, const double *qil, const double *til, const double *lc, double *out);
+__global__ __launch_bounds__(VB_NT) void k_hook_stage_lanes(int n, int layout, const double *state, const double *rec, const double *lc, const double *G, const double *qil,
+                                                            const double *til, double *out);
 __global__ void k_hook_prior(const int *hdr, const double *x0, const double *x, const double *J0, const double *r0, double *out);
 __global__ void k_hook_edge(const double *pose, const double *cp, const double *pa, const double *pb, double *out);
 __global__ void k_hook_surf(const double *pose, const double *cp, const double *n, double d, double *out);
diff --git a/vil_fusion_amd/csrc/vilf_marg.hip b/vil_fusion_amd/csrc/vilf_marg.hip
--- a/vil_fusion_amd/csrc/vilf_marg.hip
+++ b/vil_fusion_amd/csrc/vilf_marg.hip
@@ -235,19 +235,22 @@
     __syncthreads();
     if (have_prior && tid < phdr[1] && s_pmap[tid] >= 0) s_pinv[s_pmap[tid]] = tid;
     if (mode == 0) {
-        if (tid == 0) {
+        const int mwave = __builtin_amdgcn_readfirstlane(tid >> 6);
+        if ((tid & 63) == 0) {
+            const unsigned ir = imu_wave_roles(mwave), lr = lidar_wave_roles(mwave);
             const double *rec = b.imu + ((size_t)w * 10) * IMU_REC;
-            if (rec[0] < 10.0) {
+            if (ir && rec[0] < 10.0) {
                 double r[15];
-                imu_raw_eval<true, 32, false>(s_pose, s_sb, s_pose + 7, s_sb + 9, rec, b.G, r, s_J);
-                for (int k = 0; k < 15; k++) s_J[32 * k + 30] = r[k];
-            }
-        }
-        if (tid == 64 && b.use_lidar) {
-            const double *lc = b.lidar + ((size_t)w * 10) * 7;
-            double Ji[36], Jj[36];
-            lidar_between_eval<true>(s_pose, s_pose + 7, q_load(b.qil), b.til, q_load(lc), lc + 4, s_lr, Ji, Jj);
-            for (int rr = 0; rr < 6; rr++) for (int c = 0; c < 6; c++) { s_lJ[12 * rr + c] = Ji[6 * rr + c]; s_lJ[12 * rr + 6 + c] = Jj[6 * rr + c]; }
+                imu_raw_roles<true, 32>(ir, s_pose, s_sb, s_pose + 7, s_sb + 9, rec, b.G, r, s_J);
+                if (ir & IMU_ROLE_RES) for (int k = 0; k < 15; k++) s_J[32 * k + 30] = r[k];
+            }
+            if (lr && b.use_lidar) {
+                const double *lc = b.lidar + ((size_t)w * 10) * 7;
+                double Ji[36], Jj[36];
+                lidar_between_roles<true>(lr, s_pose, s_pose + 7, q_load(b.qil), b.til, q_load(lc), lc + 4, s_lr, Ji, Jj);
+                if (lr & LID_ROLE_JI) for (int rr = 0; rr < 6; rr++) for (int c = 0; c < 6; c++) s_lJ[12 * rr + c] = Ji[6 * rr + c];
+                if (lr & LID_ROLE_JJ) for (int rr = 0; rr < 6; rr++) for (int c = 0; c < 6; c++) s_lJ[12 * rr + 6 + c] = Jj[6 * rr + c];
+            }
         }
     }
     __syncthreads();
```

Result: no change. 1.097 million (median of 6 runs) (+0.8%).
